# PlayVoice/whisper-vits-svc

Hardware: AMD Instinct MI355X
Metric: audio-seconds/sec end-to-end SVC @32kHz, 10s clips (Whisper-PPG -> flow -> NSF-BigVGAN) (higher is better)
Workload: dtype f32; 1 GPU; configs[1]: batch=1 x 10s clip per GPU, whisper-large-v2 dims (24 of 32 encoder blocks) + base.yaml prior/flow/NSF-BigVGAN; Whisper fp32, synthesizer fp32; clips_in_flight=4, gemm_ring2_mask=12, world_size=1, rccl_ranks_seen=1, whisper_weights_wire=f32, weights=packed on this rank

## Files before the change

### include/svcmi.h

```cpp
#ifndef SVCMI_H
#define SVCMI_H

#include <stddef.h>
#include <stdint.h>

#ifdef __cplusplus
extern "C" {
#endif

#define SVCMI_ABI_VERSION 22

enum svcmi_status { SVCMI_OK = 0, SVCMI_EINVAL = -1, SVCMI_EUNSUPPORTED = -2, SVCMI_EALIGN = -3 };

enum svcmi_act { SVCMI_ACT_NONE = 0, SVCMI_ACT_RELU = 1, SVCMI_ACT_GELU = 2, SVCMI_ACT_MISH = 3, SVCMI_ACT_TANH = 4, SVCMI_ACT_SIGMOID = 5 };

enum svcmi_conv_flags {
    SVCMI_CONV_ACCUMULATE = 1,
    SVCMI_CONV_MASK_IN = 2,
    SVCMI_CONV_MASK_OUT = 4,
    SVCMI_CONV_PARTIALS = 8,
    SVCMI_CONV_TILE_64x64 = 0x100,
    SVCMI_CONV_TILE_128x64 = 0x200,
    SVCMI_CONV_TILE_128x128 = 0x300,
    SVCMI_CONV_TILE_P16_64x48 = 0x400,
    SVCMI_CONV_TILE_P16_128x48 = 0x500,
    SVCMI_CONV_TILE_P16_64x80 = 0x600,
    SVCMI_CONV_TILE_P16_128x80 = 0x700,
    SVCMI_CONV_TILE_P16_64x160 = 0x800,
    SVCMI_CONV_TILE_64x128 = 0x900,
    SVCMI_CONV_TILE_P16W8_128x80 = 0xA00,
    SVCMI_CONV_TILE_MASK = 0xF00,
    SVCMI_CONV_RING2 = 0x1000
};

int svcmi_abi_version(void);
const char* svcmi_build_info(void);

typedef struct svcmi_conv_desc {
    const float* x;
    const float* w;
    const float* bias;
    const float* res;
    float* y;
    const int32_t* lengths;
    int64_t x_bstride, y_bstride, res_bstride;
    int32_t batch, t_in, t_out, c_in, ldx, n_out, ldw, ldy, ldr;
    int32_t ksize, stride, dilation, pad, x_row_shift;
    int32_t act;
    int32_t flags;
    float alpha;
    int32_t split_k;
    float* workspace;
    int64_t workspace_floats;
    int32_t* counters;
    int64_t counters_len;
    void* y16;
    int64_t y16_bstride;
    int32_t ldy16;
    int32_t y16_format;
} svcmi_conv_desc;

int svcmi_conv_gemm_f32(const svcmi_conv_desc* d, void* stream);

int svcmi_conv_gemm_group_f32(const svcmi_conv_desc* descs, int32_t count, void* stream);

enum svcmi_precision { SVCMI_PREC_F32 = 0, SVCMI_PREC_BF16X3 = 1, SVCMI_PREC_BF16 = 2, SVCMI_PREC_F16 = 3,
                       SVCMI_PREC_BF16_A16 = 4, SVCMI_PREC_F16_A16 = 5, SVCMI_PREC_BF16X3_A16 = 6,
                       SVCMI_PREC_MIXED = 7,
                       SVCMI_PREC_F16W2 = 8, SVCMI_PREC_F16W2_A16 = 9 };
int svcmi_pack_weights_lp(const float* w, int32_t n, int32_t ldw, int32_t precision, void* out, int32_t ldw16, void* stream);
int svcmi_conv_gemm_lp(const svcmi_conv_desc* d, int32_t precision, void* stream);
int svcmi_conv_gemm_group_lp(const svcmi_conv_desc* descs, int32_t count, int32_t precision, void* stream);

int svcmi_layernorm_f32(const float* x, const float* res, const float* gamma, const float* beta, float* y,
                        int32_t batch, int32_t rows_per_batch, int32_t c, int32_t ldx, int32_t ldr, int32_t ldy,
                        int32_t gb_bstride, float eps, void* y16, int32_t ldy16, int32_t y16_format, void* stream);

int svcmi_channel_norm_gelu_f32(const float* x, const float* gamma, const float* beta, float* y, double* scratch,
                                int32_t batch, int32_t t, int32_t c, int32_t ldx, int32_t ldy, float eps, void* stream);

int svcmi_splitk_layernorm_f32(const float* partials, int32_t split, const float* bias, float* x, const float* gamma,
                               const float* beta, float* y, int32_t batch, int32_t rows_per_batch, int32_t c,
                               int32_t ldx, int32_t ldy, float eps, void* y16, int32_t ldy16, int32_t y16_format, void* stream);

int svcmi_attention_f32(const float* q, const float* k, const float* v, float* o,
                        int32_t ldq, int32_t ldk, int32_t ldv, int32_t ldo,
                        int64_t q_bstride, int64_t k_bstride, int64_t v_bstride, int64_t o_bstride,
                        int32_t batch, int32_t t, int32_t heads, int32_t head_dim, float scale,
                        const float* rel_k, const float* rel_v, int32_t window,
                        const int32_t* lengths, void* o16, int32_t ldo16, int64_t o16_bstride, int32_t o16_format, void* stream);

int svcmi_attention16(const void* q, const void* k, const void* v, int32_t ld16, int64_t bstride16, float* o, int32_t ldo,
                      int64_t o_bstride, void* o16, int32_t ldo16, int64_t o16_bstride, int32_t batch, int32_t t, int32_t heads,
                      int32_t head_dim, float scale, const float* rel_k, const float* rel_v, int32_t window,
                      const int32_t* lengths, int32_t format, void* stream);

int svcmi_snake_alias_f32(const float* x, float* y, const float* alpha_log, const float* beta_log,
                          const float* filt, int32_t batch, int32_t len, int32_t c, int32_t ld, void* stream);
int svcmi_snake_alias_group_f32(const float* const* x, float* const* y, const float* const* alpha_log,
                                const float* const* beta_log, const float* filt, int32_t count, int32_t batch,
                                int32_t len, int32_t c, int32_t ld, void* const* y16, int32_t y16_format, void* stream);
int svcmi_block_mean_f32(const float* const* xs, int32_t count, float* y, int64_t n, void* stream);

int svcmi_snake_conv_supported(int32_t c, int32_t ld, int32_t ksize, int32_t dilation);
int svcmi_snake_conv_preferred(int32_t c, int32_t ld, int32_t ksize, int32_t dilation);
int svcmi_snake_conv_f32(const float* x, const float* w, const float* bias, const float* res, float* y,
                         const float* alpha_log, const float* beta_log, const float* filt,
                         int32_t batch, int32_t len, int32_t c, int32_t ld, int32_t ldw, int32_t ksize,
                         int32_t dilation, float alpha, int32_t accumulate, void* stream);

typedef struct svcmi_snake_conv_desc {
    const float* x; const float* w; const float* bias; const float* res; float* y;
    const float* alpha_log; const float* beta_log;
    int32_t ldw, ksize, dilation, accumulate;
    float alpha;
} svcmi_snake_conv_desc;
int svcmi_snake_conv_group_f32(const svcmi_snake_conv_desc* descs, int32_t count, const float* filt, int32_t batch,
                               int32_t len, int32_t c, int32_t ld, void* stream);

int svcmi_snake_conv_lp_supported(int32_t c, int32_t ld, int32_t ksize, int32_t dilation, int32_t precision);
int svcmi_snake_conv_group_lp(const svcmi_snake_conv_desc* descs, int32_t count, const float* filt, int32_t batch,
                              int32_t len, int32_t c, int32_t ld, int32_t precision, void* stream);

int svcmi_upsample_noise_supported(int32_t u, int32_t cp, int32_t c_in);
int svcmi_upsample_noise_f32(const float* x, const float* w_up, const float* b_up, const float* src, const float* w_nz,
                             const float* b_nz, float* y, int32_t batch, int32_t t_in, int32_t c_in, int32_t ldw_up,
                             int32_t taps, int32_t pad, int32_t u, int32_t cp, int64_t src_len, int32_t nz_k,
                             int32_t nz_stride, int32_t nz_pad, int32_t ldw_nz, void* stream);

int svcmi_snake_post_supported(int32_t c, int32_t ld, int32_t ksize);
int svcmi_snake_post_f32(const float* x, const float* w, float* y, const float* alpha_log, const float* beta_log,
                         const float* filt, int32_t batch, int32_t len, int32_t c, int32_t ld, int32_t ksize, void* stream);

int svcmi_tune_set(const char* name, int32_t value);
int svcmi_tune_get(const char* name, int32_t* value);

int svcmi_wn_gate_f32(const float* a, const float* bias, float* out, int32_t batch, int32_t t, int32_t h, int32_t lda,
                      int32_t ldo, int32_t splits, void* stream);

int svcmi_wn_update_f32(const float* rs, float* x, float* skip, const int32_t* lengths,
                        int32_t batch, int32_t t, int32_t h, int32_t ldrs, int32_t first, int32_t last, void* stream);

int svcmi_coupling_pre_f32(const float* x, int32_t ldx, int32_t x0_off, const float* ms_vs, float* out, int32_t ldo,
                           const int32_t* lengths, int32_t batch, int32_t t, int32_t half, void* stream);
int svcmi_coupling_post_f32(float* x, int32_t ldx, int32_t x1_off, const float* m, int32_t ldm, const float* ms_vs,
                            const int32_t* lengths, int32_t batch, int32_t t, int32_t half, void* stream);

int svcmi_embed_pitch_f32(float* x, int32_t ldx, const float* pit, const float* emb, const int32_t* lengths,
                          int32_t batch, int32_t t, int32_t c, void* stream);

int svcmi_sample_prior_f32(const float* stats, int32_t lds, const float* noise_ncl, const int32_t* lengths,
                           float* z, int32_t ldz, int32_t batch, int32_t t, int32_t i, void* stream);

int svcmi_ncl_to_nlc_f32(const float* x, const float* add, float add_scale, float* y,
                         int32_t batch, int32_t c, int32_t t, int32_t ldy, void* stream);
int svcmi_nlc_to_ncl_f32(const float* x, int32_t ldx, float* y, int32_t batch, int32_t c, int32_t t, void* stream);

int svcmi_pitch_prefix_f64(const float* f0, const float* rand_ini, double* prefix,
                           int32_t batch, int32_t t, int32_t hop, float sr, void* stream);
int svcmi_pitch_source_f32(const float* f0, const double* prefix, const float* noise, const float* merge_w,
                           float merge_b, float* out, int32_t batch, int32_t t, int32_t hop, float sr, void* stream);

int svcmi_reflect_pad_f32(const float* x, float* y, int32_t batch, int64_t n, int32_t pad, void* stream);
int svcmi_power_spectrum_f32(const float* ri, float* p, int64_t rows, int32_t nbins, int32_t half, int32_t ldri, int32_t ldp, void* stream);
int svcmi_logmel_finish_f32(float* mel_power, float* scratch, float* out, int32_t batch, int32_t t, int32_t c, void* stream);

int svcmi_pcm_resample_f32(const void* pcm, int32_t fmt, int32_t channels, int64_t frames, const float* taps, int32_t up, int32_t down,
                           int32_t taps_per_phase, int32_t half, float* out, int64_t n_out, void* stream);

int svcmi_lstm_step_f32(const float* gx, int64_t gx_bstride, const float* whh, float* hseq, int64_t h_bstride, int32_t ldh,
                        float* c, int32_t ldc, int32_t batch, int32_t hidden, int32_t t, int32_t t_total, void* stream);
int svcmi_preemph_pad_f32(const float* x, float* y, int32_t batch, int64_t n, int32_t pad, float coef, void* stream);
int svcmi_magnitude_spectrum_f32(const float* ri, float* p, int64_t rows, int32_t nbins, int32_t half, int32_t ldri, int32_t ldp, void* stream);
int svcmi_speaker_mel_finish_f32(float* mel, int64_t total, float ref_level_db, float min_level_db, float max_norm, void* stream);
int svcmi_l2norm_rows_f32(const float* x, int64_t ldx, int32_t rows, int32_t d, float* y, int64_t ldy, void* stream);
int svcmi_group_mean_f32(const float* x, int32_t rows_per_group, int32_t groups, int32_t d, float* y, void* stream);

int svcmi_linear_spectrogram_f32(const float* x, int64_t x_bstride, int32_t batch, int64_t n, const float* basis, int32_t n_fft, int32_t hop,
                                 int32_t pad, float eps, float* out, int64_t frames, void* stream);

int64_t svcmi_stft_distance_workspace_bytes(int32_t batch, int64_t n, int32_t n_fft, int32_t hop, int32_t pad);
int svcmi_stft_distance_f32(const float* x, int64_t x_bstride, const float* y, int64_t y_bstride, int32_t batch, int64_t n, const float* basis,
                            int32_t n_fft, int32_t hop, int32_t pad, float floor_, int64_t frames, float* partials, int64_t partials_bytes,
                            double* out, void* stream);
int svcmi_log_mel_f32(const float* spec, int32_t batch, int32_t bins, int64_t frames, const float* melT, int32_t ldm, int32_t n_mel, float clip,
                      float* out, void* stream);
int64_t svcmi_abs_diff_sum_workspace_bytes(int32_t batch, int64_t count);
int svcmi_abs_diff_sum_f32(const float* a, int64_t a_bstride, const float* b, int64_t b_bstride, int32_t batch, int64_t count, float* partials,
                           int64_t partials_bytes, double* out, void* stream);

int svcmi_crepe_frames_f32(const float* audio, int64_t n, int32_t hop, int32_t frame0, int32_t frames, float* out, int32_t ld, void* stream);
int svcmi_bn_maxpool2_f32(const float* x, const float* scale, const float* shift, float* y, int64_t rows_out, int32_t c,
                          int32_t ldx, int32_t ldy, void* y16, int32_t ldy16, int32_t y16_format, void* stream);
int svcmi_viterbi_decode(const float* prob, const double* log_trans, float* lp_scratch, int16_t* ptr_scratch, int32_t* path,
                         int32_t frames, int32_t batch_frames, int32_t minidx, int32_t maxidx, int32_t band, void* stream);

int svcmi_row_sqnorm_f32(const float* x, int32_t ldx, int64_t rows, int32_t d, float* out, void* stream);
int svcmi_knn_blend_f32(const float* x, int32_t ldx, const float* bank, int32_t ldb, const float* dots, int64_t ldd,
                        const float* bank_sq, float* out, int32_t ldo, int32_t t, int32_t n, int32_t d, int32_t k,
                        float ratio, void* stream);

int svcmi_ivf_assign_f32(const float* x, int32_t ldx, const float* dots, int64_t ldd, const float* cent_sq, int32_t t,
                         int32_t nlist, int32_t d, int32_t* assign, float* dist, void* stream);
int svcmi_ivf_blend_f32(const float* x, int32_t ldx, const int32_t* assign, const int32_t* list_off, const float* bank,
                        int32_t ldb, float* out, int32_t ldo, int32_t t, int32_t d, int32_t k, float ratio,
                        int32_t* out_idx, float* out_dist, void* stream);
int svcmi_segment_mean_f32(const float* x, int32_t ldx, const int32_t* order, const int32_t* seg_off, float* out, int32_t ldo,
                           int32_t segments, int32_t d, void* stream);

int svcmi_source2wav_i16(const float* x, int16_t* y, int64_t n, void* stream);


#define SVCMI_MAX_WHISPER_BLOCKS 32
#define SVCMI_MAX_ENC_LAYERS 8
#define SVCMI_MAX_FLOWS 8
#define SVCMI_MAX_WN_LAYERS 8
#define SVCMI_MAX_STAGES 6
#define SVCMI_MAX_AMP_BLOCKS 3
#define SVCMI_MAX_AMP_DILATIONS 3

typedef struct svcmi_weight {
    const float* w;
    const float* bias;
    const void* w16;
    const void* w16a;
    int32_t n, ldw, ldw16;
    int32_t prec16;
} svcmi_weight;

typedef struct svcmi_whisper_block {
    const float *ln1_g, *ln1_b, *ln2_g, *ln2_b;
    svcmi_weight qkv, o, m1, m2;
} svcmi_whisper_block;

typedef struct svcmi_whisper_model {
    int32_t n_state, n_heads, n_layers, n_mels, n_ctx;
    int32_t precision;
    svcmi_weight conv1, conv2;
    const float* pos;
    const float *lnp_g, *lnp_b;
    svcmi_whisper_block blocks[SVCMI_MAX_WHISPER_BLOCKS];
    int32_t split_o, split_mlp, tile_qkv, tile_o, tile_mlp1, tile_mlp2, small_m_rows, reserved;
    float lp_min_flops;
    int32_t reserved2;
} svcmi_whisper_model;

int64_t svcmi_whisper_workspace_bytes(const svcmi_whisper_model* m, int32_t batch, int32_t n_frames);
int svcmi_whisper_encoder_fwd(const svcmi_whisper_model* m, const float* mel, const float* noise, float noise_scale,
                              int32_t batch, int32_t n_frames, float* out, void* workspace, int64_t workspace_bytes, void* stream);

#define SVCMI_MAX_LSTM_LAYERS 8
typedef struct svcmi_lstm_layer {
    svcmi_weight ih;
    svcmi_weight lin;
    const float* whh;
    const void* reserved;
} svcmi_lstm_layer;
typedef struct svcmi_speaker_model {
    int32_t input_dim, lstm_dim, proj_dim, n_layers;
    svcmi_lstm_layer layers[SVCMI_MAX_LSTM_LAYERS];
} svcmi_speaker_model;

int64_t svcmi_speaker_encoder_workspace_bytes(const svcmi_speaker_model* m, int32_t batch, int32_t t);
int svcmi_speaker_encoder_fwd(const svcmi_speaker_model* m, const float* mel, int32_t batch, int32_t t, float* emb, void* workspace,
                              int64_t workspace_bytes, void* stream);

typedef struct svcmi_vad_conv_block {
    const float *dw_w, *dw_b;
    const float *pw_w, *pw_b;
    const float *proj_w, *proj_b;
    int32_t c_in, c_out;
// ... 247 lines not shown
```

### whisper-vits-svc_amd/csrc/amp_fused.hip

```cpp
#include "svcmi_rt.h"
#include "../../include/svcmi.h"

namespace {

constexpr int TPB = 256;
constexpr int RT = 8;
constexpr int CO = 10;
constexpr int DMAX = 5;

#include "snake_math.h"

template <int CP>
__device__ __forceinline__ int tile_row_offset(int t) {
    static_assert(CP == 12 || CP == 20 || CP == 40, "widths of the fused kernels");
    return CP == 12 ? (t << 3) + (t << 2) : CP == 20 ? (t << 4) + (t << 2) : (t << 5) + (t << 3);
}
__device__ __forceinline__ const float* tile_column(const float* xc) {
#ifndef SVCMI_EMU
    asm("" : "+v"(xc));
#endif
    return xc;
}
template <int CP>
__device__ __forceinline__ float tile_x(const float* xc, int t, int n, int ld) {
    (void)ld;
#ifndef SVCMI_EMU
    return ((const __attribute__((address_space(1))) float*)xc)[tile_row_offset<CP>(clampi(t, 0, n - 1))];
#else
    return xc[tile_row_offset<CP>(clampi(t, 0, n - 1))];
#endif
}
static inline bool tile_len_ok(int len, int ld) { return (long long)len * ld < (1LL << 31); }

struct AmpArgs {
    const float* x; const float* w; const float* bias; const float* res; float* y;
    const float* alpha_log; const float* beta_log; const float* filt;
    int n, ld, ldw, dil, accumulate, ks;
    float alpha;
};

template <bool H16, int LS>
__device__ __forceinline__ void tile_store(float* S, int row, int ch, float v) {
    if constexpr (H16) reinterpret_cast<unsigned short*>(S)[row * LS + ch] = (unsigned short)svcmi_cvt_pk_f16(v, 0.f);
    else S[row * LS + ch] = v;
}

template <int CP, int CR, int LS, bool H16 = false>
__device__ __forceinline__ void snake_tile(float* S, const float* xb, const float* alpha_log, const float* beta_log,
                                           const float* filt, int n, int ld, int t_blk, int halo, int rows, int tid) {
    struct { const float* alpha_log; const float* beta_log; const float* filt; } p = {alpha_log, beta_log, filt};
        float f[12];
#pragma unroll
        for (int k = 0; k < 12; ++k) f[k] = p.filt[k];
        const int runs = (rows + RT - 1) / RT;
        for (int item = tid; item < runs * CP; item += TPB) {
            const int ch = item % CP, run = item / CP;
            const int r0 = run * RT;
            const int t0 = t_blk - halo + r0;
            float out[RT];
            if (ch >= CR || t0 + RT <= 0 || t0 >= n) {
#pragma unroll
                for (int r = 0; r < RT; ++r) out[r] = 0.f;
            } else {
                const float a = expf(p.alpha_log[ch]);
                const float inv_b = 1.0f / (expf(p.beta_log[ch]) + 1e-9f);
                const float* xc = tile_column(xb + ch);
                SnakeWindow<RT + 10> xw;
#pragma unroll
                for (int i = 0; i < RT + 10; ++i) xw.set(i, tile_x<CP>(xc, t0 - 5 + i, n, ld));
                snake_run<RT>(xw, f, a, inv_b, xc, ld, n, t0, out);
#pragma unroll
                for (int r = 0; r < RT; ++r) {
                    const int t = t0 + r;
                    if (t < 0 || t >= n) out[r] = 0.f;
                }
            }
#pragma unroll
            for (int r = 0; r < RT; ++r)
                if (r0 + r < rows) tile_store<H16, LS>(S, r0 + r, ch, out[r]);
        }
}

template <int CP>
struct UTile {
    static constexpr int LU = 2 * CP + 2;
    __device__ __forceinline__ static int pos(int m) { return m * LU; }
    static constexpr int floats(int pair_rows) { return (pair_rows + 7) * LU; }
};

template <int CP, int CR, int LS, int MAXI, bool H16 = false>
__device__ __forceinline__ void snake_tile_u(float* smem, const float* xb, const float* alpha_log, const float* beta_log,
                                             const float* filt, int n, int ld, int t_blk, int halo, int rows, int tid) {
    constexpr int LU = UTile<CP>::LU;
    float f[12];
#pragma unroll
    for (int k = 0; k < 12; ++k) f[k] = filt[k];
    const int t_lo = t_blk - halo;
    const int pairs = rows + 5;
    const int mruns = (pairs + RT - 1) / RT;
    for (int item = tid; item < mruns * CP; item += TPB) {
        const int ch = item % CP, run = item / CP;
        if (ch >= CR) continue;
        const int m0 = run * RT, tq0 = t_lo + m0;
        svcmi_f32x2 s2[RT];
        if (2 * tq0 - 5 + 2 * RT - 1 < -12 || 2 * tq0 - 5 > 2 * n - 1 + 12) {
#pragma unroll
            for (int m = 0; m < RT; ++m) s2[m] = svcmi_splat2(0.f);
        } else {
            const float a = expf(alpha_log[ch]);
            const float inv_b = 1.0f / (expf(beta_log[ch]) + 1e-9f);
            const float* xc = tile_column(xb + ch);
            SnakeWindow<RT + 5> xw;
#pragma unroll
            for (int i = 0; i < RT + 5; ++i) xw.set(i, tile_x<CP>(xc, tq0 - 5 + i, n, ld));
            snake_pairs<RT>(xw, f, a, inv_b, xc, ld, n, tq0, s2);
        }
#pragma unroll
        for (int m = 0; m < RT; ++m)
            if (m0 + m < pairs) *reinterpret_cast<float2*>(smem + UTile<CP>::pos(m0 + m) + 2 * ch) = make_float2(s2[m][0], s2[m][1]);
    }
    __syncthreads();
    const int runs = (rows + RT - 1) / RT;
    float outs[MAXI][RT];
#pragma unroll
    for (int q = 0; q < MAXI; ++q) {
        const int item = tid + q * TPB;
        if (item < runs * CP) {
            const int ch = item % CP, run = item / CP, r0 = run * RT, t0 = t_lo + r0;
            if (ch >= CR || t0 + RT <= 0 || t0 >= n) {
#pragma unroll
                for (int r = 0; r < RT; ++r) outs[q][r] = 0.f;
            } else {
                svcmi_f32x2 P[RT + 5];
                const float* ub = smem + UTile<CP>::pos(r0) + 2 * ch;
#pragma unroll
                for (int i = 0; i < RT + 5; ++i) {
                    const float2 v = *reinterpret_cast<const float2*>(ub + i * LU);
                    P[i] = svcmi_f32x2{v.x, v.y};
                }
                snake_fir<RT>(P, f, outs[q]);
#pragma unroll
                for (int r = 0; r < RT; ++r) {
                    const int t = t0 + r;
                    if (t < 0 || t >= n) outs[q][r] = 0.f;
                }
            }
        }
    }
    __syncthreads();
#pragma unroll
    for (int q = 0; q < MAXI; ++q) {
        const int item = tid + q * TPB;
        if (item < runs * CP) {
            const int ch = item % CP, r0 = (item / CP) * RT;
#pragma unroll
            for (int r = 0; r < RT; ++r)
                if (r0 + r < rows) tile_store<H16, LS>(smem, r0 + r, ch, outs[q][r]);
        }
    }
}

template <int CP, int G, int TT, int KS>
struct AmpTile {
    static constexpr int TSUB = 4 / G;
    static constexpr int TB = TSUB * 64 * TT;
    static constexpr int LS = (CP / 4) % 2 ? CP : CP + 4;
    static constexpr int ROWS = TB + (KS - 1) * DMAX;
};

template <int CP, int CR, int KS_T, int G, int TT, bool UT = false>
__device__ __forceinline__ void snake_conv_body(const AmpArgs& p, float* S) {
    using TL = AmpTile<CP, G, TT, KS_T ? KS_T : 11>;
    const int KS = KS_T ? KS_T : p.ks;
    constexpr int TSUB = TL::TSUB, TB = TL::TB, LS = TL::LS;
    static_assert(G * CO >= CR && CP % 4 == 0 && CP >= CR, "channel split");

    const int tid = threadIdx.x, lane = tid & 63;
    const int wave = SVCMI_UNIFORM((int)(tid >> 6));
    const int b = blockIdx.y;
    const int n = p.n, ld = p.ld, d = p.dil;
    const int halo = (KS - 1) * d / 2;
    const int t_blk = blockIdx.x * TB;
    const int rows = TB + 2 * halo;
    const float* xb = p.x + (long long)b * n * ld;

    if constexpr (UT) snake_tile_u<CP, CR, LS, (((TL::ROWS + RT - 1) / RT) * CP + TPB - 1) / TPB>(S, xb, p.alpha_log, p.beta_log, p.filt, n, ld, t_blk, halo, rows, tid);
    else snake_tile<CP, CR, LS>(S, xb, p.alpha_log, p.beta_log, p.filt, n, ld, t_blk, halo, rows, tid);
    __syncthreads();

    const int g = wave % G, tsub = wave / G;
    const int co0 = g * CO;
    constexpr int NCO = CO;
    static_assert(NCO % 2 == 0 && CR % 2 == 0, "channel pairs");
    svcmi_f32x2 acc[TT][NCO / 2];
#pragma unroll
    for (int c = 0; c < NCO; c += 2) {
        const float b0 = (co0 + c < CR && p.bias) ? p.bias[co0 + c] : 0.f, b1 = (co0 + c < CR && p.bias) ? p.bias[co0 + c + 1] : 0.f;
#pragma unroll
        for (int j = 0; j < TT; ++j) acc[j][c / 2] = svcmi_f32x2{b0, b1};
    }
    const int tl0 = tsub * 64 * TT + lane;
    constexpr bool PRE = TT == 1;
    const float* rb = p.res ? p.res + (long long)b * n * ld : nullptr;
    float2 rpre[PRE ? TT : 1][NCO / 2];
    if constexpr (PRE) {
#pragma unroll
        for (int j = 0; j < TT; ++j) {
            const int t = t_blk + tl0 + 64 * j;
#pragma unroll
            for (int c = 0; c < NCO; c += 2) {
                rpre[j][c / 2] = make_float2(0.f, 0.f);
                if (rb && t < n && co0 + c < CR) rpre[j][c / 2] = *reinterpret_cast<const float2*>(rb + (long long)t * ld + co0 + c);
            }
        }
    }
    const float* wg = p.w + (long long)co0 * p.ldw;
    for (int tap = 0; tap < KS; ++tap) {
        const float* srow = S + (tl0 + tap * d) * LS;
        const float* wt = wg + tap * CP;
#pragma unroll
        for (int c4 = 0; c4 < (CR + 3) / 4; ++c4) {
            svcmi_f32x2 x01[TT], x23[TT];
#pragma unroll
            for (int j = 0; j < TT; ++j) {
                const float4 xin = *reinterpret_cast<const float4*>(srow + j * 64 * LS + 4 * c4);
                x01[j] = svcmi_f32x2{xin.x, xin.y}; x23[j] = svcmi_f32x2{xin.z, xin.w};
            }
#pragma unroll
            for (int c = 0; c < NCO; c += 2) {
                if (co0 + c < CR) {
                    const float* wr = wt + (long long)c * p.ldw + 4 * c4;
                    const float4 w0 = *reinterpret_cast<const float4*>(wr), w1 = *reinterpret_cast<const float4*>(wr + p.ldw);
#pragma unroll
                    for (int j = 0; j < TT; ++j) {
                        acc[j][c / 2] = svcmi_fma2(svcmi_splat_lo(x01[j]), svcmi_f32x2{w0.x, w1.x}, acc[j][c / 2]);
                        if (4 * c4 + 1 < CR) acc[j][c / 2] = svcmi_fma2(svcmi_splat_hi(x01[j]), svcmi_f32x2{w0.y, w1.y}, acc[j][c / 2]);
                        if (4 * c4 + 2 < CR) acc[j][c / 2] = svcmi_fma2(svcmi_splat_lo(x23[j]), svcmi_f32x2{w0.z, w1.z}, acc[j][c / 2]);
                        if (4 * c4 + 3 < CR) acc[j][c / 2] = svcmi_fma2(svcmi_splat_hi(x23[j]), svcmi_f32x2{w0.w, w1.w}, acc[j][c / 2]);
                    }
                }
            }
        }
    }

    float* yb = p.y + (long long)b * n * ld;
#pragma unroll
    for (int j = 0; j < TT; ++j) {
        const int t = t_blk + tl0 + 64 * j;
        if (t >= n) continue;
        float* yr = yb + (long long)t * ld + co0;
#pragma unroll
        for (int c = 0; c < NCO; c += 2) {
            float v0 = acc[j][c / 2][0], v1 = acc[j][c / 2][1];
            if (co0 + c >= CR) { v0 = 0.f; v1 = 0.f; }
            else {
                if (rb) {
                    float2 r2;
                    if constexpr (PRE) r2 = rpre[j][c / 2];
                    else r2 = *reinterpret_cast<const float2*>(rb + (long long)t * ld + co0 + c);
                    v0 += r2.x; v1 += r2.y;
                }
                v0 *= p.alpha; v1 *= p.alpha;
                if (p.accumulate) { const float2 o2 = *reinterpret_cast<const float2*>(yr + c); v0 += o2.x; v1 += o2.y; }
            }
            *reinterpret_cast<float2*>(yr + c) = make_float2(v0, v1);
        }
        if (g == G - 1) {
#pragma unroll
            for (int c = G * CO; c < CP; c += 2) *reinterpret_cast<float2*>(yb + (long long)t * ld + c) = make_float2(0.f, 0.f);
        }
    }
}

template <int CP, int CR, int KS, int G, int TT>
__global__ __launch_bounds__(TPB) void snake_conv_kernel(AmpArgs p) {
    using TL = AmpTile<CP, G, TT, KS>;
    __shared__ __attribute__((aligned(16))) float S[TL::ROWS * TL::LS];
    snake_conv_body<CP, CR, KS, G, TT>(p, S);
}

constexpr int AMP_GROUP = 3;
struct AmpGroupArgs {
    AmpArgs p[AMP_GROUP];
};

template <int CP, int CR, int G, int TT>
__global__ __launch_bounds__(TPB) void snake_conv_group_kernel(AmpGroupArgs g) {
    using TL = AmpTile<CP, G, TT, 11>;
    __shared__ __attribute__((aligned(16))) float S[TL::ROWS * TL::LS];
    snake_conv_body<CP, CR, 0, G, TT>(g.p[blockIdx.z], S);
}

template <int CP, int CR, int G, int TT>
__global__ __launch_bounds__(TPB) void snake_conv_group_u_kernel(AmpGroupArgs g) {
    using TL = AmpTile<CP, G, TT, 11>;
    constexpr int NU = UTile<CP>::floats(TL::ROWS + 5), NS = TL::ROWS * TL::LS;
    static_assert(((TL::ROWS + RT - 1) / RT) * CP <= 4 * TPB, "snake_tile_u keeps at most 4 work items per thread in registers");
    __shared__ __attribute__((aligned(16))) float S[NU > NS ? NU : NS];
    snake_conv_body<CP, CR, 0, G, TT, true>(g.p[blockIdx.z], S);
}

template <int CP, int CR, int TERMS>
struct Amp16 {
    static constexpr int CK = (CR + 7) / 8;
    static constexpr int LSH = 24;
    static constexpr int NCT = (CR + 15) / 16;
    static constexpr int TB = 256;
    static constexpr int ROWS = TB + 10 * DMAX;
    static constexpr int MAXSTEPS = (11 * CK + 3) / 4;
    static constexpr int S_FLOATS = (ROWS * LSH / 2 + 3) / 4 * 4;
    static constexpr int U_FLOATS = (UTile<CP>::floats(ROWS + 5) + 3) / 4 * 4;
    static constexpr int W_FLOATS = MAXSTEPS * NCT * TERMS * 64 * 4;
    static_assert(CK * 8 <= LSH && CP <= CK * 8 && CP + 4 >= CK * 8, "pad columns [CP, 8 CK) are one 8-byte store per row");
};

template <int CP, int CR, int TERMS, bool UT>
__device__ __forceinline__ void snake_conv16_body(const AmpArgs& p, float* smem, float* wl) {
    using TL = Amp16<CP, CR, TERMS>;
    constexpr int CK = TL::CK, LSH = TL::LSH, NCT = TL::NCT, TB = TL::TB;
    const int KS = p.ks;
    const int tid = threadIdx.x, lane = tid & 63;
    const int wave = SVCMI_UNIFORM((int)(tid >> 6));
    const int b = blockIdx.y;
    const int n = p.n, ld = p.ld, d = p.dil;
    const int halo = (KS - 1) * d / 2;
    const int t_blk = blockIdx.x * TB;
    const int rows = TB + 2 * halo;
    const float* xb = p.x + (long long)b * n * ld;
    const int nsteps = (KS * CK + 3) / 4;

    svcmi_u32x4* wf = reinterpret_cast<svcmi_u32x4*>(wl);
    auto pack_weights = [&] {
    for (int u = tid; u < nsteps * NCT * 64; u += TPB) {
        const int l = u & 63, f = u >> 6;
        const int ct = f % NCT, step = f / NCT;
        const int co = ct * 16 + (l & 15), s = 4 * step + (l >> 4);
        const int tap = s / CK, cb = s - tap * CK;
        float v[8];
#pragma unroll
        for (int h = 0; h < 2; ++h) {
            const int ci0 = cb * 8 + 4 * h;
            float4 q = make_float4(0.f, 0.f, 0.f, 0.f);
            if (co < CR && tap < KS && ci0 < CR) q = *reinterpret_cast<const float4*>(p.w + (long long)co * p.ldw + tap * CP + ci0);
            v[4 * h] = q.x;
            v[4 * h + 1] = ci0 + 1 < CR ? q.y : 0.f;
            v[4 * h + 2] = ci0 + 2 < CR ? q.z : 0.f;
            v[4 * h + 3] = ci0 + 3 < CR ? q.w : 0.f;
        }
        svcmi_u32x4 hi;
#pragma unroll
        for (int e = 0; e < 4; ++e) hi[e] = svcmi_cvt_pk_f16(v[2 * e], v[2 * e + 1]);
        wf[(f * TERMS) * 64 + l] = hi;
        if constexpr (TERMS == 2) {
            svcmi_u32x4 lo;
#pragma unroll
            for (int e = 0; e < 4; ++e)
                lo[e] = svcmi_cvt_pk_f16(v[2 * e] - svcmi_f16_bits_f32(hi[e]), v[2 * e + 1] - svcmi_f16_bits_f32(hi[e] >> 16));
            wf[(f * TERMS + 1) * 64 + l] = lo;
        }
    }
    };
    if constexpr (!UT) pack_weights();

    if constexpr (UT) snake_tile_u<CP, CR, LSH, (((TL::ROWS + RT - 1) / RT) * CP + TPB - 1) / TPB, true>(smem, xb, p.alpha_log, p.beta_log, p.filt, n, ld, t_blk, halo, rows, tid);
    else snake_tile<CP, CR, LSH, true>(smem, xb, p.alpha_log, p.beta_log, p.filt, n, ld, t_blk, halo, rows, tid);
    if constexpr (UT) pack_weights();
    unsigned short* S16 = reinterpret_cast<unsigned short*>(smem);
    if constexpr (CP < CK * 8)
        for (int r = tid; r < rows; r += TPB) *reinterpret_cast<svcmi_u32x2*>(S16 + r * LSH + CP) = svcmi_u32x2{0u, 0u};
    __syncthreads();

    constexpr int NT = 4;
    const int tq = lane & 15, kq = lane >> 4;
    svcmi_f32x4 acc[NT][NCT];
#pragma unroll
    for (int tt = 0; tt < NT; ++tt)
#pragma unroll
        for (int ct = 0; ct < NCT; ++ct) acc[tt][ct] = svcmi_f32x4{0.f, 0.f, 0.f, 0.f};
    const int row0 = wave * (16 * NT) + tq;
    const float* rb = p.res ? p.res + (long long)b * n * ld : nullptr;
    float4 rpre[NT][NCT];
#pragma unroll
    for (int tt = 0; tt < NT; ++tt) {
        const int t = t_blk + wave * (16 * NT) + tt * 16 + tq;
#pragma unroll
        for (int ct = 0; ct < NCT; ++ct) {
            const int co4 = ct * 16 + 4 * kq;
            rpre[tt][ct] = make_float4(0.f, 0.f, 0.f, 0.f);
            if (rb && t < n && co4 < CP) rpre[tt][ct] = *reinterpret_cast<const float4*>(rb + (long long)t * ld + co4);
        }
    }
    for (int step = 0; step < nsteps; ++step) {
        const int s = 4 * step + kq;
        int tap = s / CK;
        const int cb = s - tap * CK;
        tap = tap < KS ? tap : KS - 1;
        const unsigned short* sp = S16 + (row0 + tap * d) * LSH + cb * 8;
        svcmi_u32x4 bf[NT], af[NCT][TERMS];
#pragma unroll
        for (int ct = 0; ct < NCT; ++ct)
#pragma unroll
            for (int tm = 0; tm < TERMS; ++tm) af[ct][tm] = wf[((step * NCT + ct) * TERMS + tm) * 64 + lane];
#pragma unroll
        for (int tt = 0; tt < NT; ++tt) bf[tt] = *reinterpret_cast<const svcmi_u32x4*>(sp + tt * 16 * LSH);
#pragma unroll
        for (int tm = 0; tm < TERMS; ++tm)
#pragma unroll
            for (int ct = 0; ct < NCT; ++ct)
#pragma unroll
                for (int tt = 0; tt < NT; ++tt) acc[tt][ct] = svcmi_mfma16_16x16x32<true>(af[ct][tm], bf[tt], acc[tt][ct]);
    }

    float* yb = p.y + (long long)b * n * ld;
#pragma unroll
    for (int tt = 0; tt < NT; ++tt) {
        const int t = t_blk + wave * (16 * NT) + tt * 16 + tq;
        asm volatile("" ::: "memory");
        if (t >= n) continue;
#pragma unroll
        for (int ct = 0; ct < NCT; ++ct) {
            const int co4 = ct * 16 + 4 * kq;
            if (co4 >= CP) continue;
            float v[4] = {acc[tt][ct][0], acc[tt][ct][1], acc[tt][ct][2], acc[tt][ct][3]};
            float* yr = yb + (long long)t * ld + co4;
            float4 bq = make_float4(0.f, 0.f, 0.f, 0.f), oq = bq;
            const float4 rq = rpre[tt][ct];
            if (p.bias) bq = *reinterpret_cast<const float4*>(p.bias + co4);
            if (p.accumulate) oq = *reinterpret_cast<const float4*>(yr);
            const float bv[4] = {bq.x, bq.y, bq.z, bq.w}, rv[4] = {rq.x, rq.y, rq.z, rq.w}, ov[4] = {oq.x, oq.y, oq.z, oq.w};
#pragma unroll
            for (int e = 0; e < 4; ++e) v[e] = co4 + e < CR ? (v[e] + bv[e] + rv[e]) * p.alpha + ov[e] : 0.f;
            *reinterpret_cast<float4*>(yr) = make_float4(v[0], v[1], v[2], v[3]);
        }
    }
}

template <int CP, int CR, int TERMS, bool UT>
__global__ __launch_bounds__(TPB) void snake_conv16_group_kernel(AmpGroupArgs g) {
    using TL = Amp16<CP, CR, TERMS>;
    constexpr int NSW = TL::S_FLOATS + TL::W_FLOATS;
    __shared__ __attribute__((aligned(16))) float smem[UT && TL::U_FLOATS > NSW ? TL::U_FLOATS : NSW];
    snake_conv16_body<CP, CR, TERMS, UT>(g.p[blockIdx.z], smem, smem + TL::S_FLOATS);
}

template <int CP, int CR>
struct AmpM {
    static constexpr int NC4 = CP / 4;
    static constexpr int NCT = (CR + 15) / 16;
    static constexpr int TB = 256;
    static constexpr int ROWS = TB + 10 * DMAX;
    static constexpr int MAXQ = (11 * NC4 + 3) / 4;
    static constexpr int S_FLOATS = ROWS * CP;
// ... 99 lines not shown
}

template <int CP, int CR, bool UT>
__global__ __launch_bounds__(TPB) void snake_convm_group_kernel(AmpGroupArgs g) {
    using TL = AmpM<CP, CR>;
    constexpr int NSW = TL::S_FLOATS + TL::W_FLOATS;
    __shared__ __attribute__((aligned(16))) float smem[UT && TL::U_FLOATS > NSW ? TL::U_FLOATS : NSW];
    snake_convm_body<CP, CR, UT>(g.p[blockIdx.z], smem, smem + TL::S_FLOATS);
}

struct UpArgs {
    const float* x; const float* wu; const float* bu; const float* src; const float* wn; const float* bn; float* y;
    int t_in, cin, ldwu, taps, pad, u, cp, nz_k, nz_stride, nz_pad, ldwn;
    long long src_len;
};

template <int N>
__global__ __launch_bounds__(TPB) void upsample_noise_kernel(UpArgs p) {
    const int b = blockIdx.y;
    const int q = blockIdx.x * TPB + threadIdx.x;
    if (q >= p.t_in) return;
    const float* xb = p.x + (long long)b * p.t_in * p.cin;
    float acc[N];
    float* yr = p.y + ((long long)b * p.t_in + q) * N;
    if (!p.x) {
#pragma unroll
        for (int n = 0; n < N; n += 4) {
            const float4 v = *reinterpret_cast<const float4*>(yr + n);
            acc[n] = v.x; acc[n + 1] = v.y; acc[n + 2] = v.z; acc[n + 3] = v.w;
        }
    } else {
#pragma unroll
        for (int n = 0; n < N; ++n) acc[n] = p.bu[n];
    }
    for (int k = 0; p.x && k < p.taps; ++k) {
        const int row = q + k - p.pad;
        if (row < 0 || row >= p.t_in) continue;
        const float* xr = xb + (long long)row * p.cin;
        const float* wk = p.wu + k * p.cin;
        for (int c4 = 0; c4 < p.cin; c4 += 4) {
            const float4 xv = *reinterpret_cast<const float4*>(xr + c4);
            const svcmi_f32x2 x01 = {xv.x, xv.y}, x23 = {xv.z, xv.w};
#pragma unroll
            for (int n = 0; n < N; n += 2) {
                const float4 w0 = *reinterpret_cast<const float4*>(wk + (long long)n * p.ldwu + c4);
                const float4 w1 = *reinterpret_cast<const float4*>(wk + (long long)(n + 1) * p.ldwu + c4);
                svcmi_f32x2 a2 = {acc[n], acc[n + 1]};
                a2 = svcmi_fma2(svcmi_splat_lo(x01), svcmi_f32x2{w0.x, w1.x}, a2);
                a2 = svcmi_fma2(svcmi_splat_hi(x01), svcmi_f32x2{w0.y, w1.y}, a2);
                a2 = svcmi_fma2(svcmi_splat_lo(x23), svcmi_f32x2{w0.z, w1.z}, a2);
                a2 = svcmi_fma2(svcmi_splat_hi(x23), svcmi_f32x2{w0.w, w1.w}, a2);
                acc[n] = a2[0]; acc[n + 1] = a2[1];
            }
        }
    }
    const float* sb = p.src + (long long)b * p.src_len;
    const int cp = N / 2;
#pragma unroll
    for (int r = 0; r < 2; ++r) {
        const long long t = 2LL * q + r;
        for (int k = 0; k < p.nz_k; ++k) {
            const long long si = t * p.nz_stride - p.nz_pad + k;
            const float sv = (si >= 0 && si < p.src_len) ? sb[si] : 0.f;
#pragma unroll
            for (int co = 0; co < cp; ++co) acc[r * cp + co] = fmaf(p.wn[co * p.ldwn + k], sv, acc[r * cp + co]);
        }
#pragma unroll
        for (int co = 0; co < cp; ++co) acc[r * cp + co] += p.bn[co];
    }
#pragma unroll
    for (int n = 0; n < N; n += 4) *reinterpret_cast<float4*>(yr + n) = make_float4(acc[n], acc[n + 1], acc[n + 2], acc[n + 3]);
}

struct PostArgs {
    const float* x; const float* w; float* y; const float* alpha_log; const float* beta_log; const float* filt;
    int n, ld;
};

template <int CP, int CR, int KS, int TT>
__global__ __launch_bounds__(TPB) void snake_post_kernel(PostArgs p) {
    constexpr int TB = TPB * TT;
    constexpr int LS = (CP / 4) % 2 ? CP : CP + 4;
    constexpr int ROWS = TB + KS - 1;
    __shared__ __attribute__((aligned(16))) float S[ROWS * LS];
    const int tid = threadIdx.x, b = blockIdx.y;
    const int t_blk = blockIdx.x * TB;
    snake_tile<CP, CR, LS>(S, p.x + (long long)b * p.n * p.ld, p.alpha_log, p.beta_log, p.filt, p.n, p.ld, t_blk, (KS - 1) / 2,
                           ROWS, tid);
    __syncthreads();
    float acc[TT];
#pragma unroll
    for (int j = 0; j < TT; ++j) acc[j] = 0.f;
#pragma unroll
    for (int tap = 0; tap < KS; ++tap) {
#pragma unroll
        for (int c4 = 0; c4 < (CR + 3) / 4; ++c4) {
            const float4 wv = *reinterpret_cast<const float4*>(p.w + tap * CP + 4 * c4);
#pragma unroll
            for (int j = 0; j < TT; ++j) {
                const float4 xin = *reinterpret_cast<const float4*>(S + (tid + TPB * j + tap) * LS + 4 * c4);
                acc[j] = fmaf(wv.x, xin.x, acc[j]);
                if (4 * c4 + 1 < CR) acc[j] = fmaf(wv.y, xin.y, acc[j]);
                if (4 * c4 + 2 < CR) acc[j] = fmaf(wv.z, xin.z, acc[j]);
                if (4 * c4 + 3 < CR) acc[j] = fmaf(wv.w, xin.w, acc[j]);
            }
        }
    }
    float* yb = p.y + (long long)b * p.n;
#pragma unroll
    for (int j = 0; j < TT; ++j) {
        const int t = t_blk + tid + TPB * j;
        if (t < p.n) yb[t] = tanhf(acc[j]);
    }
}

template <int CP, int CR, int G, int TT>
int launch_amp(const AmpArgs& a, int batch, int ksize, void* stream) {
    constexpr int TB = (4 / G) * 64 * TT;
    dim3 grid((unsigned)((a.n + TB - 1) / TB), (unsigned)batch);
    switch (ksize) {
        case 3: SVCMI_LAUNCH((snake_conv_kernel<CP, CR, 3, G, TT>), grid, dim3(TPB), 0, stream, a); break;
        case 7: SVCMI_LAUNCH((snake_conv_kernel<CP, CR, 7, G, TT>), grid, dim3(TPB), 0, stream, a); break;
        case 11: SVCMI_LAUNCH((snake_conv_kernel<CP, CR, 11, G, TT>), grid, dim3(TPB), 0, stream, a); break;
        default: return SVCMI_EUNSUPPORTED;
    }
    return SVCMI_LAST_ERROR();
}

int g_amp_tt = 0;

}

extern "C" int svcmi_snake_conv_supported(int32_t c, int32_t ld, int32_t ksize, int32_t dilation) {
    const bool shape = (c == 10 && ld == 12) || (c == 20 && ld == 20) || (c == 40 && ld == 40);
    return shape && (ksize == 3 || ksize == 7 || ksize == 11) && dilation >= 1 && dilation <= DMAX;
}

extern "C" int svcmi_snake_conv_preferred(int32_t c, int32_t ld, int32_t ksize, int32_t dilation) {
    return svcmi_snake_conv_supported(c, ld, ksize, dilation) && c <= 20;
}

extern "C" int svcmi_snake_conv_f32(const float* x, const float* w, const float* bias, const float* res, float* y,
                                    const float* alpha_log, const float* beta_log, const float* filt,
                                    int32_t batch, int32_t len, int32_t c, int32_t ld, int32_t ldw, int32_t ksize,
                                    int32_t dilation, float alpha, int32_t accumulate, void* stream) {
    if (!x || !w || !y || !alpha_log || !beta_log || !filt || batch <= 0 || len <= 0) return SVCMI_EINVAL;
    if (x == y) return SVCMI_EINVAL;
    if (!svcmi_snake_conv_supported(c, ld, ksize, dilation)) return SVCMI_EUNSUPPORTED;
    if (ldw < ksize * ld || ldw % 4 != 0) return SVCMI_EINVAL;
    if (((uintptr_t)w & 15) || ((uintptr_t)x & 7) || ((uintptr_t)y & 7) || ((uintptr_t)res & 7)) return SVCMI_EALIGN;
    if (batch > 65535 || !tile_len_ok(len, ld)) return SVCMI_EUNSUPPORTED;
    AmpArgs a;
    a.x = x; a.w = w; a.bias = bias; a.res = res; a.y = y; a.alpha_log = alpha_log; a.beta_log = beta_log; a.filt = filt;
    a.n = len; a.ld = ld; a.ldw = ldw; a.dil = dilation; a.accumulate = accumulate; a.alpha = alpha; a.ks = ksize;
    const int tt = g_amp_tt ? g_amp_tt : 2;
    if (c == 10) return tt == 1 ? launch_amp<12, 10, 1, 1>(a, batch, ksize, stream) : tt == 2 ? launch_amp<12, 10, 1, 2>(a, batch, ksize, stream) : launch_amp<12, 10, 1, 4>(a, batch, ksize, stream);
    if (c == 20) return tt == 1 ? launch_amp<20, 20, 2, 1>(a, batch, ksize, stream) : tt == 2 ? launch_amp<20, 20, 2, 2>(a, batch, ksize, stream) : launch_amp<20, 20, 2, 4>(a, batch, ksize, stream);
    return tt == 1 ? launch_amp<40, 40, 4, 1>(a, batch, ksize, stream) : tt == 2 ? launch_amp<40, 40, 4, 2>(a, batch, ksize, stream) : launch_amp<40, 40, 4, 4>(a, batch, ksize, stream);
}

int g_amp_u = 0;
int g_amp_mfma = 1;

template <int TT>
static void launch_amp_group(const AmpGroupArgs& g, int count, int batch, int len, int c, void* stream) {
    if constexpr (TT == 1) {
        if (g_amp_u >= 0 && c == 10) {
            constexpr int TB = AmpTile<12, 1, 1, 3>::TB;
            SVCMI_LAUNCH((snake_conv_group_u_kernel<12, 10, 1, 1>), dim3((unsigned)((len + TB - 1) / TB), (unsigned)batch, (unsigned)count),
                         dim3(TPB), 0, stream, g);
            return;
        }
    }
    if constexpr (TT == 2) {
        if ((g_amp_u > 0 || (g_amp_u == 0 && (long long)batch * len >= 500000)) && c == 20) {
            constexpr int TB = AmpTile<20, 2, 2, 3>::TB;
            SVCMI_LAUNCH((snake_conv_group_u_kernel<20, 20, 2, 2>), dim3((unsigned)((len + TB - 1) / TB), (unsigned)batch, (unsigned)count),
                         dim3(TPB), 0, stream, g);
            return;
        }
    }
    if (c == 10) {
        constexpr int TB = AmpTile<12, 1, TT, 3>::TB;
        SVCMI_LAUNCH((snake_conv_group_kernel<12, 10, 1, TT>), dim3((unsigned)((len + TB - 1) / TB), (unsigned)batch, (unsigned)count),
                     dim3(TPB), 0, stream, g);
    } else if (c == 20) {
        constexpr int TB = AmpTile<20, 2, TT, 3>::TB;
        SVCMI_LAUNCH((snake_conv_group_kernel<20, 20, 2, TT>), dim3((unsigned)((len + TB - 1) / TB), (unsigned)batch, (unsigned)count),
                     dim3(TPB), 0, stream, g);
    } else {
        constexpr int TB = AmpTile<40, 4, TT, 3>::TB;
        SVCMI_LAUNCH((snake_conv_group_kernel<40, 40, 4, TT>), dim3((unsigned)((len + TB - 1) / TB), (unsigned)batch, (unsigned)count),
                     dim3(TPB), 0, stream, g);
    }
}

extern "C" int svcmi_snake_conv_group_f32(const svcmi_snake_conv_desc* descs, int32_t count, const float* filt, int32_t batch,
                                          int32_t len, int32_t c, int32_t ld, void* stream) {
    if (!descs || !filt || count < 1 || count > AMP_GROUP || batch <= 0 || len <= 0) return SVCMI_EINVAL;
    if (batch > 65535 || !tile_len_ok(len, ld)) return SVCMI_EUNSUPPORTED;
    int order[AMP_GROUP] = {0, 1, 2};
    for (int i = 0; i < count; ++i)
        for (int j = i + 1; j < count; ++j)
            if (descs[order[j]].ksize > descs[order[i]].ksize) { const int t = order[i]; order[i] = order[j]; order[j] = t; }
    AmpGroupArgs g;
    for (int i = 0; i < count; ++i) {
        const svcmi_snake_conv_desc& d = descs[order[i]];
        if (!d.x || !d.w || !d.y || !d.alpha_log || !d.beta_log || d.x == d.y) return SVCMI_EINVAL;
        if (!svcmi_snake_conv_supported(c, ld, d.ksize, d.dilation)) return SVCMI_EUNSUPPORTED;
        if (d.ldw < d.ksize * ld || d.ldw % 4 != 0) return SVCMI_EINVAL;
        if (((uintptr_t)d.w & 15) || ((uintptr_t)d.x & 7) || ((uintptr_t)d.y & 7) || ((uintptr_t)d.res & 7)) return SVCMI_EALIGN;
        AmpArgs& a = g.p[i];
        a.x = d.x; a.w = d.w; a.bias = d.bias; a.res = d.res; a.y = d.y; a.alpha_log = d.alpha_log; a.beta_log = d.beta_log;
        a.filt = filt; a.n = len; a.ld = ld; a.ldw = d.ldw; a.dil = d.dilation; a.accumulate = d.accumulate; a.alpha = d.alpha;
        a.ks = d.ksize;
    }
    for (int i = count; i < AMP_GROUP; ++i) g.p[i] = g.p[0];
    const bool mfma_auto = g_amp_mfma == 1 && c == 20 && batch <= 2;
    if ((mfma_auto || g_amp_mfma >= 2) && c <= 20 && !g_amp_tt) {
        bool al = true;
        for (int i = 0; i < count; ++i) al = al && !(((uintptr_t)g.p[i].y | (uintptr_t)g.p[i].res | (uintptr_t)g.p[i].bias) & 15);
        if (al) {
            const dim3 grid((unsigned)((len + 255) / 256), (unsigned)batch, (unsigned)count);
            const bool ut = g_amp_mfma == 3 ? false : g_amp_mfma == 2 ? true : g_amp_u >= 0;
            if (c == 10) { if (ut) SVCMI_LAUNCH((snake_convm_group_kernel<12, 10, true>), grid, dim3(TPB), 0, stream, g); else SVCMI_LAUNCH((snake_convm_group_kernel<12, 10, false>), grid, dim3(TPB), 0, stream, g); }
            else { if (ut) SVCMI_LAUNCH((snake_convm_group_kernel<20, 20, true>), grid, dim3(TPB), 0, stream, g); else SVCMI_LAUNCH((snake_convm_group_kernel<20, 20, false>), grid, dim3(TPB), 0, stream, g); }
            return SVCMI_LAST_ERROR();
        }
    }
    const int tt = g_amp_tt ? g_amp_tt : (c == 10 ? 1 : 2);
    if (tt == 4) launch_amp_group<4>(g, count, batch, len, c, stream);
    else if (tt == 1) launch_amp_group<1>(g, count, batch, len, c, stream);
    else launch_amp_group<2>(g, count, batch, len, c, stream);
    return SVCMI_LAST_ERROR();
}

extern "C" int svcmi_snake_conv_lp_supported(int32_t c, int32_t ld, int32_t ksize, int32_t dilation, int32_t precision) {
    return svcmi_snake_conv_supported(c, ld, ksize, dilation) && c <= 20 && (precision == SVCMI_PREC_F16 || precision == SVCMI_PREC_F16W2);
}

template <int CP, int CR, int TERMS>
static void launch_amp16_group(const AmpGroupArgs& g, int count, int batch, int len, bool ut, void* stream) {
    constexpr int TB = Amp16<CP, CR, TERMS>::TB;
    const dim3 grid((unsigned)((len + TB - 1) / TB), (unsigned)batch, (unsigned)count);
    if (ut) SVCMI_LAUNCH((snake_conv16_group_kernel<CP, CR, TERMS, true>), grid, dim3(TPB), 0, stream, g);
    else SVCMI_LAUNCH((snake_conv16_group_kernel<CP, CR, TERMS, false>), grid, dim3(TPB), 0, stream, g);
}

extern "C" int svcmi_snake_conv_group_lp(const svcmi_snake_conv_desc* descs, int32_t count, const float* filt, int32_t batch,
                                         int32_t len, int32_t c, int32_t ld, int32_t precision, void* stream) {
    if (!descs || !filt || count < 1 || count > AMP_GROUP || batch <= 0 || len <= 0) return SVCMI_EINVAL;
    if (batch > 65535 || !tile_len_ok(len, ld)) return SVCMI_EUNSUPPORTED;
    int order[AMP_GROUP] = {0, 1, 2};
    for (int i = 0; i < count; ++i)
        for (int j = i + 1; j < count; ++j)
            if (descs[order[j]].ksize > descs[order[i]].ksize) { const int t = order[i]; order[i] = order[j]; order[j] = t; }
    AmpGroupArgs g;
    for (int i = 0; i < count; ++i) {
        const svcmi_snake_conv_desc& d = descs[order[i]];
        if (!d.x || !d.w || !d.y || !d.alpha_log || !d.beta_log || d.x == d.y) return SVCMI_EINVAL;
        if (!svcmi_snake_conv_lp_supported(c, ld, d.ksize, d.dilation, precision)) return SVCMI_EUNSUPPORTED;
        if (d.ldw < d.ksize * ld || d.ldw % 4 != 0) return SVCMI_EINVAL;
        if (((uintptr_t)d.w & 15) || ((uintptr_t)d.x & 7) || ((uintptr_t)d.y & 15) || ((uintptr_t)d.res & 15) || ((uintptr_t)d.bias & 15)) return SVCMI_EALIGN;
        AmpArgs& a = g.p[i];
        a.x = d.x; a.w = d.w; a.bias = d.bias; a.res = d.res; a.y = d.y; a.alpha_log = d.alpha_log; a.beta_log = d.beta_log;
        a.filt = filt; a.n = len; a.ld = ld; a.ldw = d.ldw; a.dil = d.dilation; a.accumulate = d.accumulate; a.alpha = d.alpha;
        a.ks = d.ksize;
    }
    for (int i = count; i < AMP_GROUP; ++i) g.p[i] = g.p[0];
    const bool ut = g_amp_u >= 0;
    const bool w2 = precision == SVCMI_PREC_F16W2;
    if (c == 10) { if (w2) launch_amp16_group<12, 10, 2>(g, count, batch, len, ut, stream); else launch_amp16_group<12, 10, 1>(g, count, batch, len, ut, stream); }
    else { if (w2) launch_amp16_group<20, 20, 2>(g, count, batch, len, ut, stream); else launch_amp16_group<20, 20, 1>(g, count, batch, len, ut, stream); }
    return SVCMI_LAST_ERROR();
}

extern "C" int svcmi_snake_post_supported(int32_t c, int32_t ld, int32_t ksize) { return c == 10 && ld == 12 && ksize == 7; }

extern "C" int svcmi_snake_post_f32(const float* x, const float* w, float* y, const float* alpha_log, const float* beta_log,
                                    const float* filt, int32_t batch, int32_t len, int32_t c, int32_t ld, int32_t ksize, void* stream) {
    if (!x || !w || !y || !alpha_log || !beta_log || !filt || batch <= 0 || len <= 0) return SVCMI_EINVAL;
    if (!svcmi_snake_post_supported(c, ld, ksize)) return SVCMI_EUNSUPPORTED;
    if (((uintptr_t)w & 15) || ((uintptr_t)x & 7)) return SVCMI_EALIGN;
    if (batch > 65535 || !tile_len_ok(len, ld)) return SVCMI_EUNSUPPORTED;
    PostArgs a;
    a.x = x; a.w = w; a.y = y; a.alpha_log = alpha_log; a.beta_log = beta_log; a.filt = filt; a.n = len; a.ld = ld;
    constexpr int TT = 2;
    SVCMI_LAUNCH((snake_post_kernel<12, 10, 7, TT>), dim3((unsigned)((len + TPB * TT - 1) / (TPB * TT)), (unsigned)batch), dim3(TPB), 0,
                 stream, a);
    return SVCMI_LAST_ERROR();
}

extern "C" int svcmi_upsample_noise_supported(int32_t u, int32_t cp, int32_t cin) {
    return u == 2 && (cp == 12 || cp == 20) && cin % 4 == 0 && cin > 0;
}

extern "C" int svcmi_upsample_noise_f32(const float* x, const float* w_up, const float* b_up, const float* src, const float* w_nz,
                                        const float* b_nz, float* y, int32_t batch, int32_t t_in, int32_t c_in, int32_t ldw_up,
                                        int32_t taps, int32_t pad, int32_t u, int32_t cp, int64_t src_len, int32_t nz_k,
                                        int32_t nz_stride, int32_t nz_pad, int32_t ldw_nz, void* stream) {
    if (!src || !w_nz || !b_nz || !y || batch <= 0 || t_in <= 0 || nz_k <= 0) return SVCMI_EINVAL;
    if (x && (!w_up || !b_up || taps <= 0)) return SVCMI_EINVAL;
    if (!svcmi_upsample_noise_supported(u, cp, c_in)) return SVCMI_EUNSUPPORTED;
    if ((x && (ldw_up < taps * c_in || ldw_up % 4)) || ldw_nz < nz_k) return SVCMI_EINVAL;
    if (((uintptr_t)x & 15) || ((uintptr_t)w_up & 15) || ((uintptr_t)y & 15)) return SVCMI_EALIGN;
    if (batch > 65535) return SVCMI_EUNSUPPORTED;
    UpArgs a;
    a.x = x; a.wu = w_up; a.bu = b_up; a.src = src; a.wn = w_nz; a.bn = b_nz; a.y = y;
    a.t_in = t_in; a.cin = c_in; a.ldwu = ldw_up; a.taps = taps; a.pad = pad; a.u = u; a.cp = cp;
    a.nz_k = nz_k; a.nz_stride = nz_stride; a.nz_pad = nz_pad; a.ldwn = ldw_nz; a.src_len = src_len;
    dim3 grid((unsigned)((t_in + TPB - 1) / TPB), (unsigned)batch);
    if (cp == 12) SVCMI_LAUNCH((upsample_noise_kernel<24>), grid, dim3(TPB), 0, stream, a);
    else SVCMI_LAUNCH((upsample_noise_kernel<40>), grid, dim3(TPB), 0, stream, a);
    return SVCMI_LAST_ERROR();
}

extern "C" int svcmi_conv_tune_set(const char* name, int32_t value);
extern "C" int svcmi_attn_tune_set(const char* name, int32_t value);
extern "C" int svcmi_host_tune_set(const char* name, int32_t value);
extern "C" int svcmi_snake_tune_set(const char* name, int32_t value);

extern "C" int svcmi_tune_set(const char* name, int32_t value) {
    if (!name) return SVCMI_EINVAL;
    if (svcmi_conv_tune_set(name, value) == 0 || svcmi_attn_tune_set(name, value) == 0 || svcmi_host_tune_set(name, value) == 0 ||
        svcmi_snake_tune_set(name, value) == 0) return 0;
    const char* k = "amp_tt";
    int i = 0;
    while (k[i] && name[i] == k[i]) ++i;
    if (k[i] == 0 && name[i] == 0 && (value == 0 || value == 1 || value == 2 || value == 4)) { g_amp_tt = value; return 0; }
    const char* km = "amp_mfma";
    i = 0;
    while (km[i] && name[i] == km[i]) ++i;
    if (km[i] == 0 && name[i] == 0 && value >= 0 && value <= 3) { g_amp_mfma = value; return 0; }
    const char* ku = "amp_u";
    i = 0;
    while (ku[i] && name[i] == ku[i]) ++i;
    if (ku[i] == 0 && name[i] == 0 && value >= -1 && value <= 1) { g_amp_u = value; return 0; }
    return SVCMI_EINVAL;
}
```

### whisper-vits-svc_amd/csrc/host_stages.hip

```cpp
#include <math.h>
#include <string.h>

#include <vector>

#include "svcmi_rt.h"
#include "../../include/svcmi.h"

extern "C" int svcmi_pyin_plan_check_(const svcmi_pyin_plan* p);
extern "C" int svcmi_yin_plan_check_(const svcmi_yin_plan* p);

namespace {

int g_amp_grouped = 1;
int g_amp_lp = 1;

enum Op {
    OP_CONV_F32, OP_CONV_LP, OP_CONV_GROUP_F32, OP_CONV_GROUP_LP, OP_LAYERNORM, OP_SPLITK_LN, OP_ATTENTION, OP_SNAKE_ALIAS,
    OP_SNAKE_ALIAS_GROUP, OP_BLOCK_MEAN, OP_SNAKE_CONV, OP_SNAKE_CONV_GROUP, OP_UPSAMPLE_NOISE, OP_SNAKE_POST, OP_WN_GATE,
    OP_COUPLING_PRE, OP_COUPLING_POST, OP_EMBED_PITCH, OP_SAMPLE_PRIOR, OP_NCL_TO_NLC, OP_COPY2D, OP_PITCH_PREFIX, OP_PITCH_SOURCE,
    OP_ATTENTION16, OP_SNAKE_CONV_GROUP_LP, OP_LSTM_STEP, OP_L2NORM_ROWS, OP_VAD_FRONTEND, OP_VAD_LSTM_SCAN,
    OP_SALIENCE_STFT, OP_SALIENCE_MAP, OP_SALIENCE_DP, OP_PYIN_CMNDF, OP_PYIN_OBSERVE, OP_PYIN_VITERBI, OP_PYIN_FINISH,
    OP_YIN_CMNDF, OP_YIN_PICK, OP_YIN_APERIODICITY, OP_SWEEP_PITCH, OP_SWEEP_EMBED,
    OP_COUNT
};
// ... 421 lines not shown
    float* stats = qkv;
    {
        CV v; v.x = x; v.x_bs = (int64_t)T * H; v.B = B; v.t_in = T; v.c_in = v.ldx = H; v.w = &m.proj; v.lengths = io.lengths;
        v.mask_in = v.mask_out = true; v.y = stats; v.y_bs = (int64_t)T * 2 * I; v.ldy = 2 * I;
        conv(c, v);
    }
    run(c, OP_SAMPLE_PRIOR, 0.0, 16.0 * B * T * I,
        [&] { return svcmi_sample_prior_f32(stats, 2 * I, io.noise, io.lengths, z_p, I, B, T, I, c.stream); });
}

void prior_fwd(Ctx& c, const svcmi_synth_model& m, const svcmi_synth_io& io, float* z_p) {
    const int B = io.batch, T = io.t, H = m.hidden;
    const int64_t mark = c.ar.mark();
    c.prec = class_prec(m, SVCMI_CLASS_ENC);
    float* xa = c.ar.f((int64_t)B * T * H);
    float* xb = c.ar.f((int64_t)B * T * H);
    prior_front(c, m, io, xa);
    run(c, OP_EMBED_PITCH, 0.0, 8.0 * B * T * H,
        [&] { return svcmi_embed_pitch_f32(xa, H, io.pit, m.pit_emb, io.lengths, B, T, H, c.stream); });
    prior_tail(c, m, io, xa, xb, z_p);
    c.ar.release(mark);
}

void flow_fwd(Ctx& c, const svcmi_synth_model& m, const svcmi_synth_io& io, float* x) {
    const int B = io.batch, T = io.t, H = m.hidden, I = m.inter, half = I / 2, kf = m.flow_kernel;
    const int64_t mark = c.ar.mark();
    c.prec = class_prec(m, SVCMI_CLASS_FLOW);
    float* hs = c.ar.f((int64_t)B * T * 2 * H);
    float* skip = hs + H;
    const int nk = (kf * H + 31) / 32;
    const int blocks = B * ((T + 63) / 64) * ((2 * H + 63) / 64);
    int split = 1;
    if (blocks < 256) {
        const int a = nk / 8, b = (288 + blocks / 2) / blocks;
        split = a < b ? a : b;
        if (split < 1) split = 1;
    }
    float* msvs = c.ar.f((int64_t)B * 2 * half);
    float* x0n = c.ar.f((int64_t)B * T * half);
    float* acts = c.ar.f((int64_t)B * T * H);
    float* mpost = c.ar.f((int64_t)B * T * half);
    float* slabs = c.ar.f((int64_t)B * split * T * 2 * H);
    for (int fl = 0; fl < m.n_flow; ++fl) {
        const svcmi_flow_layer& L = m.flow[fl];
        {
            CV v; v.x = io.spk; v.x_bs = m.spk_dim; v.B = B; v.t_in = 1; v.c_in = v.ldx = m.spk_dim; v.w = &L.snac;
            v.y = msvs; v.y_bs = 2 * half; v.ldy = 2 * half;
            conv(c, v);
        }
        run(c, OP_COUPLING_PRE, 0.0, 8.0 * B * T * half,
            [&] { return svcmi_coupling_pre_f32(x, I, L.x0_off, msvs, x0n, half, io.lengths, B, T, half, c.stream); });
        {
            CV v; v.x = x0n; v.x_bs = (int64_t)T * half; v.B = B; v.t_in = T; v.c_in = v.ldx = half; v.w = &L.pre; v.lengths = io.lengths;
            v.mask_out = true; v.y = hs; v.y_bs = (int64_t)T * 2 * H; v.ldy = 2 * H;
            conv(c, v);
        }
        for (int l = 0; l < L.n_wn; ++l) {
            const svcmi_wn_layer& W = L.wn[l];
            {
                CV v; v.x = hs; v.x_bs = (int64_t)T * 2 * H; v.B = B; v.t_in = T; v.c_in = H; v.ldx = 2 * H; v.w = &W.in; v.bias = false;
                v.ksize = kf; v.pad = (kf - 1) / 2; v.slabs = slabs; v.split_k = split;
                conv(c, v);
            }
            run(c, OP_WN_GATE, 0.0, 4.0 * B * T * H * (2 * split + 1),
                [&] { return svcmi_wn_gate_f32(slabs, W.in.bias, acts, B, T, H, 2 * H, H, split, c.stream); });
            {
                CV v; v.x = acts; v.x_bs = (int64_t)T * H; v.B = B; v.t_in = T; v.c_in = v.ldx = H; v.w = &W.rs; v.lengths = io.lengths;
                v.mask_out = true; v.accumulate = true; v.y = l == L.n_wn - 1 ? skip : hs; v.y_bs = (int64_t)T * 2 * H; v.ldy = 2 * H;
                conv(c, v);
            }
        }
        {
            CV v; v.x = skip; v.x_bs = (int64_t)T * 2 * H; v.B = B; v.t_in = T; v.c_in = H; v.ldx = 2 * H; v.w = &L.post;
            v.lengths = io.lengths; v.mask_out = true; v.y = mpost; v.y_bs = (int64_t)T * half; v.ldy = half;
            conv(c, v);
        }
        run(c, OP_COUPLING_POST, 0.0, 12.0 * B * T * half,
            [&] { return svcmi_coupling_post_f32(x, I, L.x1_off, mpost, half, msvs, io.lengths, B, T, half, c.stream); });
    }
    c.ar.release(mark);
}

struct Snk { const float* a; const float* b; };

void snake_alias(Ctx& c, const svcmi_synth_model& m, const float* x, float* y, Snk s, int B, int64_t L, int C, int ld) {
    run(c, OP_SNAKE_ALIAS, 0.0, 8.0 * B * L * ld,
        [&] { return svcmi_snake_alias_f32(x, y, s.a, s.b, m.filt, B, (int32_t)L, C, ld, c.stream); });
}

void amp_block_seq(Ctx& c, const svcmi_synth_model& m, const svcmi_gen_stage& st, const svcmi_amp_block& blk, const float* y, float* acc,
                   float* xj, float* tmp, float* tmp2, int j, int nb, int B, int64_t L) {
    const int cp = st.cp, k = blk.k;
    const int64_t bs = L * cp;
    bool fused = true;
    for (int q = 0; q < blk.n_dil; ++q) fused = fused && svcmi_snake_conv_preferred(st.c, cp, k, blk.dil[q]);
    const float* xc = y;
    for (int q = 0; q < blk.n_dil; ++q) {
        const bool last = q == blk.n_dil - 1;
        const int d = blk.dil[q];
        float* outp = last ? acc : xj;
        const float alpha = last ? 1.0f / nb : 1.0f;
        const bool accum = last && j > 0;
        if (fused) {
            run(c, OP_SNAKE_CONV, 2.0 * B * L * st.c * st.c * k, 8.0 * B * L * st.c, [&] {
                return svcmi_snake_conv_f32(xc, blk.c1[q].w, blk.c1[q].bias, nullptr, tmp, blk.a1_alpha[q], blk.a1_beta[q], m.filt, B,
                                            (int32_t)L, st.c, cp, blk.c1[q].ldw, k, d, 1.0f, 0, c.stream);
            });
            run(c, OP_SNAKE_CONV, 2.0 * B * L * st.c * st.c * k, 8.0 * B * L * st.c, [&] {
                return svcmi_snake_conv_f32(tmp, blk.c2[q].w, blk.c2[q].bias, xc, outp, blk.a2_alpha[q], blk.a2_beta[q], m.filt, B,
                                            (int32_t)L, st.c, cp, blk.c2[q].ldw, k, 1, alpha, accum ? 1 : 0, c.stream);
            });
        } else {
            snake_alias(c, m, xc, tmp, Snk{blk.a1_alpha[q], blk.a1_beta[q]}, B, L, cp, cp);
            CV v; v.B = B; v.t_in = (int)L; v.c_in = v.ldx = cp; v.x_bs = bs; v.y_bs = bs; v.ldy = cp; v.ksize = k; v.tile = amp_tile(cp);
            { CV a = v; a.x = tmp; a.w = &blk.c1[q]; a.dil = d; a.pad = (k * d - d) / 2; a.y = tmp2; conv(c, a); }
            snake_alias(c, m, tmp2, tmp, Snk{blk.a2_alpha[q], blk.a2_beta[q]}, B, L, cp, cp);
            {
                CV a = v; a.x = tmp; a.w = &blk.c2[q]; a.pad = (k - 1) / 2; a.res = xc; a.res_bs = bs; a.ldr = cp; a.alpha = alpha;
                a.accumulate = accum; a.y = outp;
                conv(c, a);
            }
        }
        xc = xj;
    }
}

bool amp_stage_grouped(Ctx& c, const svcmi_synth_model& m, const svcmi_gen_stage& st, const float* y, float* acc, int B, int64_t L) {
    const int nb = st.n_blocks, cp = st.cp;
    if (!g_amp_grouped || nb < 2 || nb > 3 || cp % 4) return false;
    const int nd = st.blocks[0].n_dil;
    int nf = 0, nall = 0;
    for (int j = 0; j < nb; ++j) {
        if (st.blocks[j].n_dil != nd) return false;
        for (int q = 0; q < nd; ++q) { nf += svcmi_snake_conv_preferred(st.c, cp, st.blocks[j].k, st.blocks[j].dil[q]) ? 1 : 0; ++nall; }
    }
    if (nf != 0 && nf != nall) return false;
    const bool fused = nf == nall;
    const int64_t n = (int64_t)B * L * cp, bs = L * cp;
    float *xj[3], *t1[3], *t2[3];
    void* t1h[3] = {nullptr, nullptr, nullptr};
    for (int j = 0; j < nb; ++j) xj[j] = c.ar.f(n);
    for (int j = 0; j < nb; ++j) t1[j] = c.ar.f(n);
    for (int j = 0; j < nb; ++j) t2[j] = c.ar.f(n);
    if (!fused && mode16(c.prec) && cp % 8 == 0)
        for (int j = 0; j < nb; ++j) t1h[j] = c.ar.take(n * 2);
    const float* xc[3] = {y, y, y};
    bool lp = fused && g_amp_lp && (c.prec == SVCMI_PREC_F16 || c.prec == SVCMI_PREC_F16W2);
    for (int j = 0; lp && j < nb; ++j)
        for (int q = 0; q < nd; ++q) lp = lp && svcmi_snake_conv_lp_supported(st.c, cp, st.blocks[j].k, st.blocks[j].dil[q], SVCMI_PREC_F16W2);
    for (int q = 0; q < nd; ++q) {
        float** outs = q == nd - 1 ? t2 : xj;
        if (fused) {
            svcmi_snake_conv_desc d[3];
            double fl = 0.0;
            for (int j = 0; j < nb; ++j) {
                const svcmi_amp_block& b = st.blocks[j];
                d[j] = svcmi_snake_conv_desc{xc[j], b.c1[q].w, b.c1[q].bias, nullptr, t1[j], b.a1_alpha[q], b.a1_beta[q], b.c1[q].ldw, b.k,
                                             b.dil[q], 0, 1.0f};
                fl += 2.0 * B * L * st.c * st.c * b.k;
            }
            auto half_step = [&] {
                if (lp) run(c, OP_SNAKE_CONV_GROUP_LP, fl, 8.0 * nb * B * L * st.c,
                            [&] { return svcmi_snake_conv_group_lp(d, nb, m.filt, B, (int32_t)L, st.c, cp, SVCMI_PREC_F16W2, c.stream); });
                else run(c, OP_SNAKE_CONV_GROUP, fl, 8.0 * nb * B * L * st.c,
                         [&] { return svcmi_snake_conv_group_f32(d, nb, m.filt, B, (int32_t)L, st.c, cp, c.stream); });
            };
            half_step();
            for (int j = 0; j < nb; ++j) {
                const svcmi_amp_block& b = st.blocks[j];
                d[j] = svcmi_snake_conv_desc{t1[j], b.c2[q].w, b.c2[q].bias, xc[j], outs[j], b.a2_alpha[q], b.a2_beta[q], b.c2[q].ldw, b.k,
                                             1, 0, 1.0f};
            }
            half_step();
        } else {
            const float* px[3]; float* py[3]; const float *pa[3], *pb[3];
            CV vs[3];
            auto snake = [&](bool second) {
                const bool h16 = t1h[0] && conv_group(c, vs, nb, true) >= SVCMI_PREC_BF16_A16;
                for (int j = 0; j < nb; ++j) {
                    px[j] = second ? t2[j] : xc[j]; py[j] = t1[j];
                    pa[j] = second ? st.blocks[j].a2_alpha[q] : st.blocks[j].a1_alpha[q];
                    pb[j] = second ? st.blocks[j].a2_beta[q] : st.blocks[j].a1_beta[q];
                    if (!h16) vs[j].x16 = nullptr;
                }
                run(c, OP_SNAKE_ALIAS_GROUP, 0.0, (h16 ? 4.0 + 2.0 * w16(c.prec, 1) : 8.0) * nb * B * L * cp, [&] {
                    return svcmi_snake_alias_group_f32(px, h16 ? nullptr : py, pa, pb, m.filt, nb, B, (int32_t)L, cp, cp, h16 ? t1h : nullptr, fmt16_of(c.prec),
                                                       c.stream);
                });
            };
            for (int j = 0; j < nb; ++j) {
                const svcmi_amp_block& b = st.blocks[j];
                CV& v = vs[j]; v = CV();
                v.x = t1[j]; v.x16 = t1h[j]; v.x_bs = bs; v.B = B; v.t_in = (int)L; v.c_in = v.ldx = cp; v.w = &b.c1[q]; v.ksize = b.k; v.dil = b.dil[q];
                v.tile = amp_tile(cp);
                v.pad = (b.k * b.dil[q] - b.dil[q]) / 2; v.y = t2[j]; v.y_bs = bs; v.ldy = cp;
            }
            snake(false);
            conv_group(c, vs, nb);
            for (int j = 0; j < nb; ++j) {
                const svcmi_amp_block& b = st.blocks[j];
                CV& v = vs[j]; v = CV();
                v.x = t1[j]; v.x16 = t1h[j]; v.x_bs = bs; v.B = B; v.t_in = (int)L; v.c_in = v.ldx = cp; v.w = &b.c2[q]; v.ksize = b.k; v.pad = (b.k - 1) / 2;
                v.tile = amp_tile(cp);
                v.res = xc[j]; v.res_bs = bs; v.ldr = cp; v.y = outs[j]; v.y_bs = bs; v.ldy = cp;
            }
            snake(true);
            conv_group(c, vs, nb);
        }
        for (int j = 0; j < nb; ++j) xc[j] = outs[j];
    }
    run(c, OP_BLOCK_MEAN, 0.0, 4.0 * (nb + 1) * n, [&] { return svcmi_block_mean_f32(xc, nb, acc, n, c.stream); });
    return true;
}

void generator_tile(Ctx& c, const svcmi_synth_model& m, const float* z, const float* spk, const float* source, float* wave, int B, int T,
                    int split_k, int stop_after) {
    const int U = m.upsample_input;
    const int64_t mark = c.ar.mark();
    c.prec = class_prec(m, SVCMI_CLASS_UPS);
    float* sb = c.ar.f((int64_t)B * 2 * U);
    {
        CV v; v.x = spk; v.x_bs = m.spk_dim; v.B = B; v.t_in = 1; v.c_in = v.ldx = m.spk_dim; v.w = &m.adapter; v.y = sb; v.y_bs = 2 * U; v.ldy = 2 * U;
        conv(c, v);
    }
    float* xn = c.ar.f((int64_t)B * T * U);
    layernorm(c, z, nullptr, sb, sb + U, xn, B, T, U, U, 0, U, 2 * U);
    int cin = m.conv_pre.n;
    float* x = c.ar.f((int64_t)B * T * cin);
    {
        CV v; v.x = xn; v.x_bs = (int64_t)T * U; v.B = B; v.t_in = T; v.c_in = v.ldx = U; v.w = &m.conv_pre; v.ksize = 7; v.pad = 3;
        v.act = SVCMI_ACT_MISH; v.split_k = split_k; v.y = x; v.y_bs = (int64_t)T * cin; v.ldy = cin;
        conv(c, v);
    }
    const int64_t Lsrc = (int64_t)T * m.hop;
    if (stop_after == SVCMI_STOP_GEN_PRE) { c.ar.release(mark); return; }
    int64_t t_in = T;
    for (int i = 0; i < m.n_stages; ++i) {
        const svcmi_gen_stage& st = m.stages[i];
        const int cp = st.cp, u = st.u;
        const int64_t L = t_in * u;
        float* y = c.ar.f((int64_t)B * L * cp);
        float* acc = c.ar.f((int64_t)B * L * cp);
        const int64_t smark = c.ar.mark();
        c.prec = class_prec(m, SVCMI_CLASS_UPS);
        CV up; up.x = x; up.x_bs = t_in * cin; up.B = B; up.t_in = (int)t_in; up.t_out = (int)t_in; up.c_in = up.ldx = cin; up.w = &st.up;
        up.ksize = st.up_taps; up.pad = st.up_pad; up.split_k = split_k; up.y = y; up.y_bs = L * cp; up.ldy = u * cp;
        if (svcmi_upsample_noise_supported(u, cp, cin)) {
            const bool fuse_up = cp <= 12;
            if (!fuse_up) conv(c, up);
            run(c, OP_UPSAMPLE_NOISE, 0.0, 4.0 * B * t_in * (cin + u * cp), [&] {
                return svcmi_upsample_noise_f32(fuse_up ? x : nullptr, st.up.w, st.up.bias, source, st.nz.w, st.nz.bias, y, B, (int32_t)t_in,
                                                fuse_up ? cin : 4, st.up.ldw, st.up_taps, st.up_pad, u, cp, Lsrc, st.nz_k, st.nz_stride,
                                                st.nz_pad, st.nz.ldw, c.stream);
            });
        } else {
            conv(c, up);
            CV nz; nz.x = source; nz.x_bs = Lsrc; nz.B = B; nz.t_in = (int)Lsrc; nz.t_out = (int)L; nz.c_in = 1; nz.ldx = 1; nz.w = &st.nz;
            nz.ksize = st.nz_k; nz.stride = st.nz_stride; nz.pad = st.nz_pad; nz.accumulate = true; nz.split_k = split_k;
            nz.y = y; nz.y_bs = L * cp; nz.ldy = cp;
            conv(c, nz);
        }
        c.prec = class_prec(m, SVCMI_CLASS_AMP0 + (i < SVCMI_AMP_CLASSES ? i : SVCMI_AMP_CLASSES - 1));
        if (!amp_stage_grouped(c, m, st, y, acc, B, L)) {
            c.ar.release(smark);
            float* xj = c.ar.f((int64_t)B * L * cp);
            float* tmp = c.ar.f((int64_t)B * L * cp);
            float* tmp2 = c.ar.f((int64_t)B * L * cp);
            for (int j = 0; j < st.n_blocks; ++j) amp_block_seq(c, m, st, st.blocks[j], y, acc, xj, tmp, tmp2, j, st.n_blocks, B, L);
        }
        c.ar.release(smark);
        x = acc; cin = cp; t_in = L;
        if (stop_after == SVCMI_STOP_STAGE0 + i) { c.ar.release(mark); return; }
    }
    const svcmi_gen_stage& last = m.stages[m.n_stages - 1];
    c.prec = class_prec(m, SVCMI_CLASS_UPS);
    if (svcmi_snake_post_supported(last.c, cin, 7) && m.post.ldw >= 7 * cin) {
        run(c, OP_SNAKE_POST, 2.0 * B * t_in * last.c * 7, 4.0 * B * t_in * (last.c + 1), [&] {
            return svcmi_snake_post_f32(x, m.post.w, wave, m.post_alpha, m.post_beta, m.filt, B, (int32_t)t_in, last.c, cin, 7, c.stream);
        });
    } else {
        float* a = c.ar.f((int64_t)B * t_in * cin);
        snake_alias(c, m, x, a, Snk{m.post_alpha, m.post_beta}, B, t_in, cin, cin);
        CV v; v.x = a; v.x_bs = t_in * cin; v.B = B; v.t_in = (int)t_in; v.c_in = v.ldx = cin; v.w = &m.post; v.bias = false; v.n_out = 1;
        v.ksize = 7; v.pad = 3; v.act = SVCMI_ACT_TANH; v.y = wave; v.y_bs = t_in; v.ldy = 1;
        conv(c, v);
    }
    c.ar.release(mark);
}

constexpr int STREAM_HALO = 32;

void generator_fwd(Ctx& c, const svcmi_synth_model& m, const svcmi_synth_io& io, const float* z) {
    const int B = io.batch, T = io.t, S = io.stream_frames, U = m.upsample_input, hop = m.hop;
    if (S <= 0) { generator_tile(c, m, z, io.spk, io.source, io.wave, B, T, 0, io.stop_after); return; }
    const int64_t mark = c.ar.mark();
    const int tmax = S + 2 * STREAM_HALO < T ? S + 2 * STREAM_HALO : T;
    float* zt = c.ar.f((int64_t)B * tmax * U);
    float* st = c.ar.f((int64_t)B * tmax * hop);
    float* ot = c.ar.f((int64_t)B * tmax * hop);
    for (int t0 = 0; t0 < T; t0 += S) {
        const int a = t0 - STREAM_HALO > 0 ? t0 - STREAM_HALO : 0, b = t0 + S + STREAM_HALO < T ? t0 + S + STREAM_HALO : T;
        const int n = S < T - t0 ? S : T - t0, tt = b - a;
        copy2d(c, z + (int64_t)a * U, (int64_t)T * U, zt, (int64_t)tt * U, B, (int64_t)tt * U);
        copy2d(c, io.source + (int64_t)a * hop, (int64_t)T * hop, st, (int64_t)tt * hop, B, (int64_t)tt * hop);
        generator_tile(c, m, zt, io.spk, st, ot, B, tt, 1, SVCMI_STOP_NONE);
        copy2d(c, ot + (int64_t)(t0 - a) * hop, (int64_t)tt * hop, io.wave + (int64_t)t0 * hop, (int64_t)T * hop, B, (int64_t)n * hop);
    }
    c.ar.release(mark);
}

bool synth_shapes_ok(const svcmi_synth_model& m, const svcmi_synth_io& io) {
    if (m.precision < SVCMI_PREC_F32 || (m.precision > SVCMI_PREC_F16 && m.precision != SVCMI_PREC_MIXED && m.precision != SVCMI_PREC_F16W2)) return false;
    if (m.precision == SVCMI_PREC_MIXED)
        for (int i = 0; i < SVCMI_PREC_CLASSES; ++i)
            if ((m.class_prec[i] < SVCMI_PREC_F32 || m.class_prec[i] > SVCMI_PREC_F16) && m.class_prec[i] != SVCMI_PREC_F16W2) return false;
    return io.batch > 0 && io.t > 0 && m.n_enc >= 1 && m.n_enc <= SVCMI_MAX_ENC_LAYERS && m.n_flow >= 0 && m.n_flow <= SVCMI_MAX_FLOWS &&
           m.n_stages >= 1 && m.n_stages <= SVCMI_MAX_STAGES && m.hidden % 4 == 0 && m.inter % 8 == 0 && 2 * m.inter <= 3 * m.hidden &&
           m.upsample_input % 4 == 0 && (io.ppg_row_shift == 0 || io.ppg_row_shift == 1) && io.ppg_bstride % 4 == 0;
}

void synth_fwd(Ctx& c, const svcmi_synth_model& m, const svcmi_synth_io& io) {
    if (!synth_shapes_ok(m, io)) { c.rc = SVCMI_EINVAL; return; }
    const int B = io.batch, T = io.t, I = m.inter;
    c.lp_min_flops = m.lp_min_flops > 0.f ? m.lp_min_flops : 1.5e9f;
// ... 514 lines not shown
```

### whisper-vits-svc_amd/svcmi/_lib.py

```python
import ctypes
import os
from ctypes import POINTER, Structure, c_char_p, c_double, c_float, c_int, c_int32, c_int64, c_void_p

HERE = os.path.dirname(os.path.abspath(__file__))
DEFAULT_LIB = os.path.join(HERE, "libsvcmi.so")

ACT_NONE, ACT_RELU, ACT_GELU, ACT_MISH, ACT_TANH, ACT_SIGMOID = 0, 1, 2, 3, 4, 5
CONV_ACCUMULATE, CONV_MASK_IN, CONV_MASK_OUT, CONV_PARTIALS = 1, 2, 4, 8
ABI_VERSION = 22
PREC_F32, PREC_BF16X3, PREC_BF16, PREC_F16, PREC_BF16_A16, PREC_F16_A16, PREC_BF16X3_A16 = 0, 1, 2, 3, 4, 5, 6
PRECISIONS = {None: 0, "f32": 0, "fp32": 0, "bf16x3": 1, "bf16": 2, "f16": 3, "fp16": 3, "f16w2": 8}
PREC_F16W2, PREC_F16W2_A16 = 8, 9
PREC_MIXED = 7
PREC_CLASSES = 12
CLASS_ENC, CLASS_FLOW, CLASS_UPS, CLASS_AMP0 = 0, 1, 2, 3
AMP_CLASSES = 5
CLASS_NAMES = {"enc": 0, "flow": 1, "ups": 2, "amp0": 3, "amp1": 4, "amp2": 5, "amp3": 6, "amp4": 7, "encattn": 8}
MIXED_DEFAULT = {"enc": "bf16x3", "encattn": "f32", "ups": "bf16x3", "flow": "f16", "amp0": "bf16x3", "amp1": "f16", "amp2": "f16", "amp3": "f16w2", "amp4": "f16w2"}


def parse_precision(p):
    if isinstance(p, tuple):
        return p
    if isinstance(p, int) and not isinstance(p, bool):
        if p == PREC_MIXED:
            raise SvcmiError("precision code SVCMI_PREC_MIXED needs its per-class modes: pass \"mixed\", \"mixed:...\" or a dict")
        if p not in set(PRECISIONS.values()):
            raise SvcmiError(f"unknown precision code {p}")
        return (p, None)
    if (p is None or isinstance(p, str)) and p in PRECISIONS:
        return (PRECISIONS[p], None)
    pol = dict(MIXED_DEFAULT)
    if isinstance(p, dict):
        pol.update(p)
    elif isinstance(p, str) and (p == "mixed" or p.startswith("mixed:")):
        for item in filter(None, p[6:].split(",")):
            k, _, v = item.partition("=")
            pol[k.strip()] = v.strip()
    else:
        raise SvcmiError(f"unknown precision {p!r}")
    bad = [k for k in pol if k not in CLASS_NAMES] + [v for v in pol.values() if v not in PRECISIONS]
    if bad:
        raise SvcmiError(f"mixed precision policy: unknown class / mode {bad}; classes {sorted(CLASS_NAMES)}, modes f32 / bf16x3 / bf16 / f16 / f16w2")
    cls = [0] * PREC_CLASSES
    for k, v in pol.items():
        cls[CLASS_NAMES[k]] = PRECISIONS[v]
    return (PREC_MIXED, tuple(cls))
CONV_TILE_64x128 = 9


class SnakeConvDesc(Structure):
    _fields_ = [("x", c_void_p), ("w", c_void_p), ("bias", c_void_p), ("res", c_void_p), ("y", c_void_p),
                ("alpha_log", c_void_p), ("beta_log", c_void_p),
                ("ldw", c_int32), ("ksize", c_int32), ("dilation", c_int32), ("accumulate", c_int32), ("alpha", c_float)]


class ConvDesc(Structure):
    _fields_ = [
        ("x", c_void_p), ("w", c_void_p), ("bias", c_void_p), ("res", c_void_p), ("y", c_void_p), ("lengths", c_void_p),
        ("x_bstride", c_int64), ("y_bstride", c_int64), ("res_bstride", c_int64),
        ("batch", c_int32), ("t_in", c_int32), ("t_out", c_int32), ("c_in", c_int32), ("ldx", c_int32),
        ("n_out", c_int32), ("ldw", c_int32), ("ldy", c_int32), ("ldr", c_int32),
        ("ksize", c_int32), ("stride", c_int32), ("dilation", c_int32), ("pad", c_int32), ("x_row_shift", c_int32),
        ("act", c_int32), ("flags", c_int32), ("alpha", c_float), ("split_k", c_int32),
        ("workspace", c_void_p), ("workspace_floats", c_int64),
        ("counters", c_void_p), ("counters_len", c_int64),
        ("y16", c_void_p), ("y16_bstride", c_int64), ("ldy16", c_int32), ("y16_format", c_int32),
    ]


MAX_WHISPER_BLOCKS, MAX_ENC_LAYERS, MAX_FLOWS, MAX_WN_LAYERS, MAX_STAGES, MAX_AMP_BLOCKS, MAX_AMP_DILATIONS = 32, 8, 8, 8, 6, 3, 3
STOP_NONE, STOP_PRIOR, STOP_FLOW, STOP_GEN_PRE, STOP_STAGE0 = 0, 1, 2, 3, 4


class Weight(Structure):
    _fields_ = [("w", c_void_p), ("bias", c_void_p), ("w16", c_void_p), ("w16a", c_void_p), ("n", c_int32), ("ldw", c_int32),
                ("ldw16", c_int32), ("prec16", c_int32)]


class WhisperBlock(Structure):
    _fields_ = [("ln1_g", c_void_p), ("ln1_b", c_void_p), ("ln2_g", c_void_p), ("ln2_b", c_void_p),
                ("qkv", Weight), ("o", Weight), ("m1", Weight), ("m2", Weight)]


class WhisperModel(Structure):
    _fields_ = [("n_state", c_int32), ("n_heads", c_int32), ("n_layers", c_int32), ("n_mels", c_int32), ("n_ctx", c_int32),
                ("precision", c_int32), ("conv1", Weight), ("conv2", Weight), ("pos", c_void_p), ("lnp_g", c_void_p), ("lnp_b", c_void_p),
                ("blocks", WhisperBlock * MAX_WHISPER_BLOCKS),
                ("split_o", c_int32), ("split_mlp", c_int32), ("tile_qkv", c_int32), ("tile_o", c_int32), ("tile_mlp1", c_int32),
                ("tile_mlp2", c_int32), ("small_m_rows", c_int32), ("reserved", c_int32), ("lp_min_flops", c_float), ("reserved2", c_int32)]


class EncLayer(Structure):
    _fields_ = [("qkv", Weight), ("o", Weight), ("f1", Weight), ("f2", Weight), ("rel_k", c_void_p), ("rel_v", c_void_p),
                ("g1", c_void_p), ("b1", c_void_p), ("g2", c_void_p), ("b2", c_void_p)]


class WnLayer(Structure):
    _fields_ = [("in_", Weight), ("rs", Weight)]


class FlowLayer(Structure):
    _fields_ = [("x0_off", c_int32), ("x1_off", c_int32), ("n_wn", c_int32), ("reserved", c_int32),
                ("pre", Weight), ("post", Weight), ("snac", Weight), ("wn", WnLayer * MAX_WN_LAYERS)]


class AmpBlock(Structure):
    _fields_ = [("k", c_int32), ("n_dil", c_int32), ("dil", c_int32 * MAX_AMP_DILATIONS), ("reserved", c_int32),
                ("c1", Weight * MAX_AMP_DILATIONS), ("c2", Weight * MAX_AMP_DILATIONS),
                ("a1_alpha", c_void_p * MAX_AMP_DILATIONS), ("a1_beta", c_void_p * MAX_AMP_DILATIONS),
                ("a2_alpha", c_void_p * MAX_AMP_DILATIONS), ("a2_beta", c_void_p * MAX_AMP_DILATIONS)]


class GenStage(Structure):
    _fields_ = [("u", c_int32), ("c", c_int32), ("cp", c_int32), ("up_taps", c_int32), ("up_pad", c_int32), ("nz_k", c_int32),
                ("nz_stride", c_int32), ("nz_pad", c_int32), ("n_blocks", c_int32), ("reserved", c_int32),
                ("up", Weight), ("nz", Weight), ("blocks", AmpBlock * MAX_AMP_BLOCKS)]


class SynthModel(Structure):
    _fields_ = [("hidden", c_int32), ("inter", c_int32), ("n_heads", c_int32), ("enc_window", c_int32), ("enc_ffn_kernel", c_int32),
                ("flow_kernel", c_int32), ("n_enc", c_int32), ("n_flow", c_int32), ("n_stages", c_int32),
                ("ppg_dim", c_int32), ("vec_dim", c_int32), ("spk_dim", c_int32), ("upsample_input", c_int32), ("hop", c_int32),
                ("precision", c_int32), ("lp_min_flops", c_float), ("sampling_rate", c_float), ("merge_b", c_float),
                ("class_prec", c_int32 * PREC_CLASSES),
                ("pre", Weight), ("hub", Weight), ("proj", Weight), ("pit_emb", c_void_p),
                ("enc", EncLayer * MAX_ENC_LAYERS), ("flow", FlowLayer * MAX_FLOWS),
                ("adapter", Weight), ("conv_pre", Weight), ("post", Weight),
                ("merge_w", c_void_p), ("filt", c_void_p), ("post_alpha", c_void_p), ("post_beta", c_void_p),
                ("stages", GenStage * MAX_STAGES)]


class SynthIO(Structure):
    _fields_ = [("ppg", c_void_p), ("vec", c_void_p), ("pit", c_void_p), ("spk", c_void_p), ("lengths", c_void_p), ("source", c_void_p),
                ("noise", c_void_p), ("ppg_bstride", c_int64), ("ppg_row_shift", c_int32), ("batch", c_int32), ("t", c_int32),
                ("stream_frames", c_int32), ("stop_after", c_int32), ("reserved", c_int32),
                ("wave", c_void_p), ("z_p", c_void_p), ("z", c_void_p)]


SWEEP_MAX_KEYS = 32


class SweepIO(Structure):
    _fields_ = [("ppg", c_void_p), ("vec", c_void_p), ("pit", c_void_p), ("spk", c_void_p), ("length", c_void_p), ("source", c_void_p),
                ("noise", c_void_p), ("factors", c_double * SWEEP_MAX_KEYS), ("ppg_row_shift", c_int32), ("t", c_int32), ("n_keys", c_int32),
                ("stream_frames", c_int32), ("wave", c_void_p), ("pit_k", c_void_p)]


class LstmLayer(Structure):
    _fields_ = [("ih", Weight), ("lin", Weight), ("whh", c_void_p), ("reserved", c_void_p)]


MAX_LSTM_LAYERS = 8


class SpeakerModel(Structure):
    _fields_ = [("input_dim", c_int32), ("lstm_dim", c_int32), ("proj_dim", c_int32), ("n_layers", c_int32),
                ("layers", LstmLayer * MAX_LSTM_LAYERS)]


class VadConvBlock(Structure):
    _fields_ = [("dw_w", c_void_p), ("dw_b", c_void_p), ("pw_w", c_void_p), ("pw_b", c_void_p), ("proj_w", c_void_p), ("proj_b", c_void_p),
                ("c_in", c_int32), ("c_out", c_int32)]


class VadDown(Structure):
    _fields_ = [("w", c_void_p), ("b", c_void_p), ("scale", c_void_p), ("shift", c_void_p), ("c", c_int32), ("stride", c_int32)]


class VadModel(Structure):
    _fields_ = [("basis_t", c_void_p), ("filt", c_void_p), ("block", VadConvBlock * 4), ("down", VadDown * 4),
                ("gate0_w", c_void_p), ("gate0_b", c_void_p), ("whh0_t", c_void_p), ("wih1_t", c_void_p), ("whh1_t", c_void_p),
                ("gate1_b", c_void_p), ("dec_w", c_void_p), ("dec_b", c_float), ("reserved", c_int32)]


class SaliencePlan(Structure):
    _fields_ = [("basis", c_void_p), ("smooth", c_void_p), ("harm_off", c_void_p), ("harm_w", c_void_p),
                ("n_fft", c_int32), ("hop", c_int32), ("k_lo", c_int32), ("n_bins", c_int32),
                ("n_pitch", c_int32), ("smooth_len", c_int32), ("n_harm", c_int32), ("tol", c_int32),
                ("fs", c_float), ("f_min", c_float), ("f_max", c_float), ("bins_per_octave", c_float),
                ("thresh", c_double), ("log_hi", c_double), ("log_lo", c_double)]


SALIENCE_MAX_BINS = 1024


class PyinPlan(Structure):
    _fields_ = [("thresholds", c_void_p), ("beta", c_void_p), ("f_axis", c_void_p), ("band", c_void_p),
                ("n_fft", c_int32), ("hop", c_int32), ("p_min", c_int32), ("p_max", c_int32),
                ("n_pitch", c_int32), ("n_thr", c_int32), ("max_step", c_int32), ("reserved", c_int32),
                ("fs", c_double), ("tol_cents", c_double), ("absolute_min_prob", c_double), ("voicing_prob", c_double),
                ("log_tiny", c_double), ("log_cross", c_double), ("log_c", c_double), ("tiny", c_double)]


PYIN_MAX_BINS, PYIN_MAX_THRESHOLDS, PYIN_MAX_NFFT, PYIN_MAX_BAND = 1024, 128, 4096, 33


class YinPlan(Structure):
    _fields_ = [("n_fft", c_int32), ("hop", c_int32), ("lag_min", c_int32), ("lag_max", c_int32),
                ("fs", c_double), ("threshold", c_double), ("ratio_up", c_double), ("ratio_down", c_double)]


YIN_MAX_NFFT = 4096


class SwipeWindow(Structure):
    _fields_ = [("basis", c_void_p), ("resample", c_void_p), ("kernels", c_void_p), ("cand", c_void_p), ("mu", c_void_p),
                ("n_fft", c_int32), ("n_cand", c_int32)]


SWIPE_MAX_WINDOWS, SWIPE_MAX_NFFT, SWIPE_MAX_LOGBINS, SWIPE_MAX_CANDIDATES = 8, 4096, 1024, 1024


class SwipePlan(Structure):
    _fields_ = [("win", SwipeWindow * SWIPE_MAX_WINDOWS),
                ("n_win", c_int32), ("hop", c_int32), ("n_log", c_int32), ("n_pitch", c_int32),
                ("f_min", c_double), ("step", c_double), ("threshold", c_double)]


class TraceRecord(Structure):
    _fields_ = [("op", c_int32), ("ms", c_float), ("flops", c_double), ("bytes", c_double)]


_P, _I, _L, _F = c_void_p, c_int32, c_int64, c_float
SIGNATURES = {
    "svcmi_abi_version": (c_int, []),
    "svcmi_build_info": (c_char_p, []),
    "svcmi_conv_gemm_f32": (c_int, [POINTER(ConvDesc), _P]),
    "svcmi_pack_weights_lp": (c_int, [_P, _I, _I, _I, _P, _I, _P]),
    "svcmi_conv_gemm_lp": (c_int, [POINTER(ConvDesc), _I, _P]),
    "svcmi_conv_gemm_group_lp": (c_int, [_P, _I, _I, _P]),
    "svcmi_layernorm_f32": (c_int, [_P, _P, _P, _P, _P, _I, _I, _I, _I, _I, _I, _I, _F, _P, _I, _I, _P]),
    "svcmi_channel_norm_gelu_f32": (c_int, [_P, _P, _P, _P, _P, _I, _I, _I, _I, _I, _F, _P]),
    "svcmi_splitk_layernorm_f32": (c_int, [_P, _I, _P, _P, _P, _P, _P, _I, _I, _I, _I, _I, _F, _P, _I, _I, _P]),
    "svcmi_attention_f32": (c_int, [_P, _P, _P, _P, _I, _I, _I, _I, _L, _L, _L, _L, _I, _I, _I, _I, _F, _P, _P, _I, _P, _P, _I, _L, _I, _P]),
    "svcmi_attention16": (c_int, [_P, _P, _P, _I, _L, _P, _I, _L, _P, _I, _L, _I, _I, _I, _I, _F, _P, _P, _I, _P, _I, _P]),
    "svcmi_snake_alias_f32": (c_int, [_P, _P, _P, _P, _P, _I, _I, _I, _I, _P]),
    "svcmi_snake_conv_supported": (c_int, [_I, _I, _I, _I]),
    "svcmi_snake_conv_preferred": (c_int, [_I, _I, _I, _I]),
    "svcmi_snake_conv_f32": (c_int, [_P, _P, _P, _P, _P, _P, _P, _P, _I, _I, _I, _I, _I, _I, _I, _F, _I, _P]),
    "svcmi_upsample_noise_supported": (c_int, [_I, _I, _I]),
    "svcmi_upsample_noise_f32": (c_int, [_P, _P, _P, _P, _P, _P, _P, _I, _I, _I, _I, _I, _I, _I, _I, _L, _I, _I, _I, _I, _P]),
    "svcmi_tune_set": (c_int, [c_char_p, _I]),
    "svcmi_tune_get": (c_int, [c_char_p, POINTER(c_int32)]),
    "svcmi_wn_gate_f32": (c_int, [_P, _P, _P, _I, _I, _I, _I, _I, _I, _P]),
    "svcmi_wn_update_f32": (c_int, [_P, _P, _P, _P, _I, _I, _I, _I, _I, _I, _P]),
    "svcmi_coupling_pre_f32": (c_int, [_P, _I, _I, _P, _P, _I, _P, _I, _I, _I, _P]),
    "svcmi_coupling_post_f32": (c_int, [_P, _I, _I, _P, _I, _P, _P, _I, _I, _I, _P]),
    "svcmi_embed_pitch_f32": (c_int, [_P, _I, _P, _P, _P, _I, _I, _I, _P]),
    "svcmi_sample_prior_f32": (c_int, [_P, _I, _P, _P, _P, _I, _I, _I, _I, _P]),
    "svcmi_ncl_to_nlc_f32": (c_int, [_P, _P, _F, _P, _I, _I, _I, _I, _P]),
    "svcmi_nlc_to_ncl_f32": (c_int, [_P, _I, _P, _I, _I, _I, _P]),
    "svcmi_pitch_prefix_f64": (c_int, [_P, _P, _P, _I, _I, _I, _F, _P]),
    "svcmi_pitch_source_f32": (c_int, [_P, _P, _P, _P, _F, _P, _I, _I, _I, _F, _P]),
    "svcmi_reflect_pad_f32": (c_int, [_P, _P, _I, _L, _I, _P]),
    "svcmi_power_spectrum_f32": (c_int, [_P, _P, _L, _I, _I, _I, _I, _P]),
    "svcmi_logmel_finish_f32": (c_int, [_P, _P, _P, _I, _I, _I, _P]),
    "svcmi_pcm_resample_f32": (c_int, [_P, _I, _I, _L, _P, _I, _I, _I, _I, _P, _L, _P]),
    "svcmi_linear_spectrogram_f32": (c_int, [_P, _L, _I, _L, _P, _I, _I, _I, _F, _P, _L, _P]),
    "svcmi_stft_distance_workspace_bytes": (c_int64, [_I, _L, _I, _I, _I]),
    "svcmi_stft_distance_f32": (c_int, [_P, _L, _P, _L, _I, _L, _P, _I, _I, _I, _F, _L, _P, _L, _P, _P]),
    "svcmi_log_mel_f32": (c_int, [_P, _I, _I, _L, _P, _I, _I, _F, _P, _P]),
    "svcmi_abs_diff_sum_workspace_bytes": (c_int64, [_I, _L]),
    "svcmi_abs_diff_sum_f32": (c_int, [_P, _L, _P, _L, _I, _L, _P, _L, _P, _P]),
    "svcmi_lstm_step_f32": (c_int, [_P, _L, _P, _P, _L, _I, _P, _I, _I, _I, _I, _I, _P]),
    "svcmi_preemph_pad_f32": (c_int, [_P, _P, _I, _L, _I, _F, _P]),
    "svcmi_magnitude_spectrum_f32": (c_int, [_P, _P, _L, _I, _I, _I, _I, _P]),
    "svcmi_speaker_mel_finish_f32": (c_int, [_P, _L, _F, _F, _F, _P]),
    "svcmi_l2norm_rows_f32": (c_int, [_P, _L, _I, _I, _P, _L, _P]),
    "svcmi_group_mean_f32": (c_int, [_P, _I, _I, _I, _P, _P]),
    "svcmi_speaker_encoder_workspace_bytes": (c_int64, [POINTER(SpeakerModel), _I, _I]),
    "svcmi_speaker_encoder_fwd": (c_int, [POINTER(SpeakerModel), _P, _I, _I, _P, _P, _L, _P]),
    "svcmi_vad_model_bytes": (c_int64, []),
    "svcmi_vad_frontend_f32": (c_int, [POINTER(VadModel), _P, _P, _P, _I, _I, _P, _P, _P]),
    "svcmi_vad_lstm_scan_f32": (c_int, [POINTER(VadModel), _P, _P, _I, _I, _P, _P, _P]),
    "svcmi_mask_spans_f32": (c_int, [_P, _L, _P, _I, _L, _I, _P, _L, _P]),
    "svcmi_vad_workspace_bytes": (c_int64, [_I, _I]),
    "svcmi_vad_probs_fwd": (c_int, [POINTER(VadModel), _P, _P, _P, _I, _I, _P, _P, _P, _L, _P]),
    "svcmi_salience_plan_bytes": (c_int64, []),
    "svcmi_salience_stft_f32": (c_int, [POINTER(SaliencePlan), _P, _L, _P, _L, _P]),
    "svcmi_salience_map_f32": (c_int, [POINTER(SaliencePlan), _P, _L, _P, _P, _P, _P]),
    "svcmi_salience_dp_f64": (c_int, [_P, _L, _I, _I, c_double, c_double, _P, _P, _P]),
    "svcmi_salience_workspace_bytes": (c_int64, [POINTER(SaliencePlan), _L]),
    "svcmi_salience_f0_fwd": (c_int, [POINTER(SaliencePlan), _P, _L, _P, _P, _P, _L, _P]),
    "svcmi_pyin_plan_bytes": (c_int64, []),
    "svcmi_pyin_cmndf_f64": (c_int, [POINTER(PyinPlan), _P, _L, _P, _P, _L, _P]),
    "svcmi_pyin_observe_f64": (c_int, [POINTER(PyinPlan), _P, _L, _P, _P, _P, _P, _P]),
    "svcmi_pyin_viterbi_f64": (c_int, [_P, _L, _I, _I, _P, c_double, c_double, c_double, _P, _P, _P]),
    "svcmi_pyin_finish_f64": (c_int, [POINTER(PyinPlan), _P, _P, _P, _P, _P, _L, _P, _P, _P]),
    "svcmi_pyin_workspace_bytes": (c_int64, [POINTER(PyinPlan), _L]),
    "svcmi_pyin_f0_fwd": (c_int, [POINTER(PyinPlan), _P, _L, _P, _P, _P, _P, _P, _P, _P, _P, _L, _P]),
    "svcmi_yin_plan_bytes": (c_int64, []),
    "svcmi_yin_cmndf_f64": (c_int, [POINTER(YinPlan), _P, _L, _P, _P, _L, _P]),
    "svcmi_yin_pick_f64": (c_int, [POINTER(YinPlan), _P, _L, _P, _P, _P, _P, _P]),
    "svcmi_yin_aperiodicity_f64": (c_int, [POINTER(YinPlan), _P, _L, _P, _L, _P, _P]),
    "svcmi_yin_workspace_bytes": (c_int64, [POINTER(YinPlan), _L]),
    "svcmi_yin_f0_fwd": (c_int, [POINTER(YinPlan), _P, _L, _P, _P, _P, _P, _P, _P, _L, _P]),
    "svcmi_swipe_plan_bytes": (c_int64, []),
    "svcmi_swipe_frames": (c_int64, [POINTER(SwipePlan), _I, _L]),
    "svcmi_swipe_mag_f32": (c_int, [POINTER(SwipePlan), _I, _P, _L, _P, _P]),
    "svcmi_swipe_resample_f32": (c_int, [POINTER(SwipePlan), _I, _P, _L, _P, _P]),
    "svcmi_swipe_strength_f32": (c_int, [POINTER(SwipePlan), _I, _P, _L, _P, _P]),
    "svcmi_swipe_accum_f32": (c_int, [POINTER(SwipePlan), _P, _L, _P, _P]),
    "svcmi_swipe_finish_f64": (c_int, [_P, _L, _I, _I, c_double, c_double, c_double, _P, _P, _P, _P, _P]),
    "svcmi_swipe_workspace_bytes": (c_int64, [POINTER(SwipePlan), _L]),
    "svcmi_swipe_f0_fwd": (c_int, [POINTER(SwipePlan), _P, _L, _P, _P, _P, _P, _P, _L, _P]),
    "svcmi_crepe_frames_f32": (c_int, [_P, _L, _I, _I, _I, _P, _I, _P]),
    "svcmi_bn_maxpool2_f32": (c_int, [_P, _P, _P, _P, _L, _I, _I, _I, _P, _I, _I, _P]),
    "svcmi_viterbi_decode": (c_int, [_P, _P, _P, _P, _P, _I, _I, _I, _I, _I, _P]),
    "svcmi_row_sqnorm_f32": (c_int, [_P, _I, _L, _I, _P, _P]),
    "svcmi_knn_blend_f32": (c_int, [_P, _I, _P, _I, _P, _L, _P, _P, _I, _I, _I, _I, _I, _F, _P]),
    "svcmi_ivf_assign_f32": (c_int, [_P, _I, _P, _L, _P, _I, _I, _I, _P, _P, _P]),
    "svcmi_ivf_blend_f32": (c_int, [_P, _I, _P, _P, _P, _I, _P, _I, _I, _I, _I, _F, _P, _P, _P]),
    "svcmi_segment_mean_f32": (c_int, [_P, _I, _P, _P, _P, _I, _I, _I, _P]),
    "svcmi_snake_post_supported": (c_int, [_I, _I, _I]),
    "svcmi_snake_post_f32": (c_int, [_P, _P, _P, _P, _P, _P, _I, _I, _I, _I, _I, _P]),
    "svcmi_conv_gemm_group_f32": (c_int, [_P, _I, _P]),
    "svcmi_snake_conv_group_f32": (c_int, [_P, _I, _P, _I, _I, _I, _I, _P]),
    "svcmi_snake_conv_lp_supported": (c_int, [_I, _I, _I, _I, _I]),
    "svcmi_snake_conv_group_lp": (c_int, [_P, _I, _P, _I, _I, _I, _I, _I, _P]),
    "svcmi_snake_alias_group_f32": (c_int, [_P, _P, _P, _P, _P, _I, _I, _I, _I, _I, _P, _I, _P]),
    "svcmi_block_mean_f32": (c_int, [_P, _I, _P, _L, _P]),
    "svcmi_source2wav_i16": (c_int, [_P, _P, _L, _P]),
    "svcmi_whisper_workspace_bytes": (c_int64, [POINTER(WhisperModel), _I, _I]),
    "svcmi_whisper_encoder_fwd": (c_int, [POINTER(WhisperModel), _P, _P, _F, _I, _I, _P, _P, _L, _P]),
    "svcmi_synth_workspace_bytes": (c_int64, [POINTER(SynthModel), _I, _I, _I]),
    "svcmi_pitch2source_fwd": (c_int, [POINTER(SynthModel), _P, _P, _P, _I, _I, _P, _P, _L, _P]),
    "svcmi_text_encoder_fwd": (c_int, [POINTER(SynthModel), POINTER(SynthIO), _P, _P, _L, _P]),
    "svcmi_flow_reverse_fwd": (c_int, [POINTER(SynthModel), POINTER(SynthIO), _P, _P, _L, _P]),
    "svcmi_generator_fwd": (c_int, [POINTER(SynthModel), POINTER(SynthIO), _P, _P, _L, _P]),
    "svcmi_synth_infer_fwd": (c_int, [POINTER(SynthModel), POINTER(SynthIO), _P, _L, _P]),
    "svcmi_copy2d_f32": (c_int, [_P, _L, _P, _L, _L, _L, _P]),
    "svcmi_sweep_pitch_f32": (c_int, [_P, _P, _P, _I, _I, _P]),
    "svcmi_sweep_embed_f32": (c_int, [_P, _I, _P, _P, _P, _P, _I, _I, _I, _I, _P]),
    "svcmi_sweep_io_bytes": (c_int64, []),
    "svcmi_synth_sweep_workspace_bytes": (c_int64, [POINTER(SynthModel), _I, _I, _I]),
    "svcmi_synth_sweep_fwd": (c_int, [POINTER(SynthModel), POINTER(SweepIO), _P, _L, _P]),
    "svcmi_trace_begin": (c_int, [_I]),
    "svcmi_trace_end": (c_int, [POINTER(TraceRecord), _I]),
    "svcmi_trace_op_name": (c_char_p, [_I]),
    "svcmi_struct_sizes": (c_int, [POINTER(c_int64), _I]),
    "svcmi_packed_model_info": (c_int, [_P, _L, POINTER(c_int32), POINTER(c_int64), POINTER(c_int64)]),
    "svcmi_packed_model_bind": (c_int, [_P, _L, _P, _P, _L]),
}


class SvcmiError(RuntimeError):
    pass


def load_library(path=None):
    path = path or os.environ.get("SVCMI_LIB", DEFAULT_LIB)
    if not os.path.exists(path):
        raise SvcmiError(
            f"{path} not found: the HIP kernels are not built. Run `python whisper-vits-svc_amd/build.py` "
            "(hipcc --offload-arch=gfx950). svcmi has no CPU fallback.")
    lib = ctypes.CDLL(path)
    for name, (res, args) in SIGNATURES.items():
        try:
            fn = getattr(lib, name)
        except AttributeError as e:
            raise SvcmiError(f"{path} does not export {name}") from e
        fn.restype, fn.argtypes = res, args
    if lib.svcmi_abi_version() != ABI_VERSION:
        raise SvcmiError(f"ABI mismatch: library {lib.svcmi_abi_version()} vs binding {ABI_VERSION}")
    import ctypes as _c
    sizes = (c_int64 * 8)()
    n = lib.svcmi_struct_sizes(sizes, 8)
    mine = [_c.sizeof(t) for t in (Weight, WhisperModel, SynthModel, SynthIO, TraceRecord, ConvDesc, SnakeConvDesc)]
    if list(sizes[:n]) != mine:
        raise SvcmiError(f"struct layout mismatch: library {list(sizes[:n])} vs binding {mine}")
    if lib.svcmi_vad_model_bytes() != _c.sizeof(VadModel):
        raise SvcmiError(f"struct layout mismatch: svcmi_vad_model is {lib.svcmi_vad_model_bytes()} bytes in the library, {_c.sizeof(VadModel)} in the binding")
    if lib.svcmi_salience_plan_bytes() != _c.sizeof(SaliencePlan):
        raise SvcmiError(f"struct layout mismatch: svcmi_salience_plan is {lib.svcmi_salience_plan_bytes()} bytes in the library, {_c.sizeof(SaliencePlan)} in the binding")
    if lib.svcmi_pyin_plan_bytes() != _c.sizeof(PyinPlan):
        raise SvcmiError(f"struct layout mismatch: svcmi_pyin_plan is {lib.svcmi_pyin_plan_bytes()} bytes in the library, {_c.sizeof(PyinPlan)} in the binding")
    if lib.svcmi_yin_plan_bytes() != _c.sizeof(YinPlan):
        raise SvcmiError(f"struct layout mismatch: svcmi_yin_plan is {lib.svcmi_yin_plan_bytes()} bytes in the library, {_c.sizeof(YinPlan)} in the binding")
    if lib.svcmi_sweep_io_bytes() != _c.sizeof(SweepIO):
        raise SvcmiError(f"struct layout mismatch: svcmi_sweep_io is {lib.svcmi_sweep_io_bytes()} bytes in the library, {_c.sizeof(SweepIO)} in the binding")
    if lib.svcmi_swipe_plan_bytes() != _c.sizeof(SwipePlan):
        raise SvcmiError(f"struct layout mismatch: svcmi_swipe_plan is {lib.svcmi_swipe_plan_bytes()} bytes in the library, {_c.sizeof(SwipePlan)} in the binding")
    return lib
```

### whisper-vits-svc_amd/svcmi/cmodel.py

```python
from . import _lib
from ._lib import PREC_BF16, PREC_BF16X3, PREC_F16, PREC_F32
from .vits import consts as K


class CModel:

    def __init__(self, struct, keep):
        self.struct, self.keep = struct, keep


def _weight(cw, ops, w, bias, prec, keep, a16=False):
    cw.w, cw.bias = w.data_ptr(), (0 if bias is None else bias.data_ptr())
    cw.n, cw.ldw = int(w.shape[0]), int(w.shape[1])
    cw.w16, cw.w16a, cw.ldw16, cw.prec16 = 0, 0, 0, 0
    if prec != PREC_F32 and w.dim() == 2 and w.is_contiguous():
        base = PREC_F16 if prec == _lib.PREC_F16W2 else prec
        img = ops.lp_weight(w, base)
        cw.w16, cw.ldw16, cw.prec16 = img.data_ptr(), img.shape[1] // (2 if prec == PREC_BF16X3 else 1), prec
        keep.append(img)
        if a16:
            a16_code = {PREC_BF16X3: _lib.PREC_BF16X3_A16, _lib.PREC_F16W2: _lib.PREC_F16W2_A16}.get(prec, prec + 2)
            img_a = ops.lp_weight(w, a16_code)
            cw.w16a = img_a.data_ptr()
            keep.append(img_a)
    keep.append(w)
    keep.append(bias)


def whisper_cmodel(w, ops, prec=PREC_F32):
    m, keep = _lib.WhisperModel(), [w]
    if w.n_layers > _lib.MAX_WHISPER_BLOCKS:
        raise _lib.SvcmiError(f"{w.n_layers} encoder blocks > {_lib.MAX_WHISPER_BLOCKS}")
    m.n_state, m.n_heads, m.n_layers, m.n_mels = w.S, w.heads, w.n_layers, w.n_mels
    m.n_ctx, m.precision = int(w.pos.shape[0]), prec
    x3 = prec == PREC_BF16X3
    _weight(m.conv1, ops, w.conv1_w, w.conv1_b, prec, keep)
    _weight(m.conv2, ops, w.conv2_w, w.conv2_b, prec, keep)
    m.pos, m.lnp_g, m.lnp_b = w.pos.data_ptr(), w.lnp_g.data_ptr(), w.lnp_b.data_ptr()
    for i, b in enumerate(w.blocks):
        cb = m.blocks[i]
        cb.ln1_g, cb.ln1_b, cb.ln2_g, cb.ln2_b = (b[k].data_ptr() for k in ("ln1_g", "ln1_b", "ln2_g", "ln2_b"))
        _weight(cb.qkv, ops, b["qkv_w"], b["qkv_b"], prec, keep, a16=True)
        _weight(cb.o, ops, b["o_w"], b["o_b"], prec, keep, a16=not x3)
        _weight(cb.m1, ops, b["m1_w"], b["m1_b"], prec, keep, a16=not x3)
        _weight(cb.m2, ops, b["m2_w"], b["m2_b"], prec, keep, a16=not x3)
    return CModel(m, keep)


def speaker_cmodel(w, ops):
    m, keep = _lib.SpeakerModel(), [w]
    if len(w.layers) > _lib.MAX_LSTM_LAYERS:
        raise _lib.SvcmiError(f"{len(w.layers)} LSTM layers > {_lib.MAX_LSTM_LAYERS}")
    m.input_dim, m.lstm_dim, m.proj_dim, m.n_layers = w.input_dim, w.lstm_dim, w.proj_dim, len(w.layers)
    for i, ly in enumerate(w.layers):
        _weight(m.layers[i].ih, ops, ly["ih_w"], ly["bias"], PREC_F32, keep)
        _weight(m.layers[i].lin, ops, ly["lin_w"], None, PREC_F32, keep)
        m.layers[i].whh = ly["whh"].data_ptr()
        keep.append(ly["whh"])
    return CModel(m, keep)


def synth_cmodel(w, ops, prec=PREC_F32):
    code, classes = prec if isinstance(prec, tuple) else (prec, None)
    m, keep = _lib.SynthModel(), [w]
    hp = w.hp
    if len(w.enc) > _lib.MAX_ENC_LAYERS or len(w.flow) > _lib.MAX_FLOWS or len(w.stages) > _lib.MAX_STAGES:
        raise _lib.SvcmiError("model exceeds the fixed capacities of svcmi_synth_model")
    m.hidden, m.inter, m.n_heads = w.H, w.I, w.n_heads
    m.enc_window, m.enc_ffn_kernel, m.flow_kernel = K.ENC_WINDOW, K.ENC_FFN_KERNEL, K.FLOW_KERNEL
    m.n_enc, m.n_flow, m.n_stages = len(w.enc), len(w.flow), len(w.stages)
    m.ppg_dim, m.vec_dim, m.spk_dim = hp.vits.ppg_dim, hp.vits.vec_dim, hp.vits.spk_dim
    m.upsample_input, m.hop = w.U, w.hop
    m.precision, m.lp_min_flops = code, 0.0
    for i in range(_lib.PREC_CLASSES):
        m.class_prec[i] = classes[i] if classes else 0
    m.sampling_rate, m.merge_b = float(hp.data.sampling_rate), float(w.merge_b)
    state = {"cls": _lib.CLASS_ENC}

    def W(cw, wt, b=None, a16=False):
        p = classes[state["cls"]] if classes else code
        _weight(cw, ops, wt, b, p, keep, a16=a16 and p != PREC_BF16X3)
    W(m.pre, w.pre_w, w.pre_b)
    W(m.hub, w.hub_w, w.hub_b)
    W(m.proj, w.proj_w, w.proj_b)
    m.pit_emb = w.pit_emb.data_ptr()
    for i, L in enumerate(w.enc):
        e = m.enc[i]
        W(e.qkv, L["qkv_w"], L["qkv_b"], a16=True)
        W(e.o, L["o_w"], L["o_b"], a16=True)
        W(e.f1, L["f1_w"], L["f1_b"], a16=True)
        W(e.f2, L["f2_w"], L["f2_b"], a16=True)
        e.rel_k, e.rel_v = L["rel_k"].data_ptr(), L["rel_v"].data_ptr()
        e.g1, e.b1, e.g2, e.b2 = (L[k].data_ptr() for k in ("g1", "b1", "g2", "b2"))
    state["cls"] = _lib.CLASS_FLOW
    for i, L in enumerate(w.flow):
        f = m.flow[i]
        if len(L["wn"]) > _lib.MAX_WN_LAYERS:
            raise _lib.SvcmiError("too many WN layers")
        f.x0_off, f.x1_off, f.n_wn = L["x0_off"], L["x1_off"], len(L["wn"])
        W(f.pre, L["pre_w"], L["pre_b"])
        W(f.post, L["post_w"], L["post_b"])
        W(f.snac, L["snac_w"], L["snac_b"])
        for l, Wl in enumerate(L["wn"]):
            W(f.wn[l].in_, Wl["in_w"], Wl["in_b"])
            W(f.wn[l].rs, Wl["rs_w"], Wl["rs_b"])
    state["cls"] = _lib.CLASS_UPS
    W(m.adapter, w.ad_w, w.ad_b)
    W(m.conv_pre, w.pre_conv_w, w.pre_conv_b)
    W(m.post, w.post_w, None)
    m.merge_w, m.filt = w.merge_w.data_ptr(), w.filt.data_ptr()
    m.post_alpha, m.post_beta = w.post_a[0].data_ptr(), w.post_a[1].data_ptr()
    for i, st in enumerate(w.stages):
        s = m.stages[i]
        if len(st["blocks"]) > _lib.MAX_AMP_BLOCKS:
            raise _lib.SvcmiError("more AMP blocks per stage than svcmi_gen_stage holds")
        s.u, s.c, s.cp, s.up_taps, s.up_pad = st["u"], st["c"], st["cp"], st["up_taps"], st["up_pad"]
        s.nz_k, s.nz_stride, s.nz_pad, s.n_blocks = st["nz_k"], st["nz_stride"], st["nz_pad"], len(st["blocks"])
        state["cls"] = _lib.CLASS_UPS
        W(s.up, st["up_w"], st["up_b"])
        W(s.nz, st["nz_w"], st["nz_b"])
        state["cls"] = _lib.CLASS_AMP0 + min(i, _lib.AMP_CLASSES - 1)
        for j, blk in enumerate(st["blocks"]):
            b = s.blocks[j]
            if len(blk["d"]) > _lib.MAX_AMP_DILATIONS:
                raise _lib.SvcmiError("more dilations per AMP block than svcmi_amp_block holds")
            b.k, b.n_dil = blk["k"], len(blk["d"])
            for q, d in enumerate(blk["d"]):
                b.dil[q] = d
                W(b.c1[q], blk["c1"][q][0], blk["c1"][q][1], a16=st["cp"] % 8 == 0)
                W(b.c2[q], blk["c2"][q][0], blk["c2"][q][1], a16=st["cp"] % 8 == 0)
                b.a1_alpha[q], b.a1_beta[q] = blk["a1"][q][0].data_ptr(), blk["a1"][q][1].data_ptr()
                b.a2_alpha[q], b.a2_beta[q] = blk["a2"][q][0].data_ptr(), blk["a2"][q][1].data_ptr()
    return CModel(m, keep)


def vad_cmodel(w):
    m, keep = _lib.VadModel(), [w]
    m.basis_t, m.filt = w.basis_t.data_ptr(), w.filt.data_ptr()
    for i, blk in enumerate(w.blocks):
        b = m.block[i]
        b.c_in, b.c_out = blk["c_in"], blk["c_out"]
        for k in ("dw_w", "dw_b", "pw_w", "pw_b", "proj_w", "proj_b"):
            setattr(b, k, 0 if blk[k] is None else blk[k].data_ptr())
    for i, dn in enumerate(w.downs):
        d = m.down[i]
        d.c, d.stride = dn["c"], dn["stride"]
        for k in ("w", "b", "scale", "shift"):
            setattr(d, k, dn[k].data_ptr())
    for k in ("gate0_w", "gate0_b", "whh0_t", "wih1_t", "whh1_t", "gate1_b", "dec_w"):
        setattr(m, k, getattr(w, k).data_ptr())
    m.dec_b = w.dec_b
    return CModel(m, keep)
```

### whisper-vits-svc_amd/svcmi/ops.py

```python
import contextlib
import ctypes
import os
import threading

import torch

from . import _lib
from ._lib import (ACT_GELU, ACT_MISH, ACT_NONE, ACT_RELU, ACT_SIGMOID, ACT_TANH, CONV_ACCUMULATE, CONV_MASK_IN,
                   CONV_MASK_OUT, CONV_PARTIALS, PREC_BF16, PREC_BF16X3, PREC_F16, PREC_F32, PRECISIONS, ConvDesc, SnakeConvDesc, SvcmiError,
                   SynthIO, TraceRecord)


SPLIT16 = "bf16x3"


def _fmt16(dtype):
    return {torch.bfloat16: PREC_BF16, torch.float16: PREC_F16, SPLIT16: PREC_BF16X3}[dtype]


def _alloc16(lead, c, out16, device):
    if out16 == SPLIT16:
        cp = (c + 7) // 8 * 8
        return (torch.zeros if cp != c else torch.empty)(*lead, 2 * cp, dtype=torch.bfloat16, device=device)
    return torch.empty(*lead, c, dtype=out16, device=device)
# ... 399 lines not shown
    def layernorm(self, x, gamma=None, beta=None, *, res=None, eps=1e-5, per_batch_affine=False, out=None, out16=None):
        self._chk(x, gamma, beta, res, out)
        B, T, Cc = x.shape
        if out is None:
            out = torch.empty_like(x)
        y16 = _alloc16((B, T), Cc, out16, x.device) if out16 is not None else None
        self._call("svcmi_layernorm_f32", _ptr(x), _ptr(res), _ptr(gamma), _ptr(beta), _ptr(out), B, T, Cc,
                   x.stride(1), res.stride(1) if res is not None else 0, out.stride(1),
                   (gamma.stride(0) if gamma is not None else beta.stride(0)) if per_batch_affine else 0, eps,
                   _ptr(y16), y16.stride(1) if y16 is not None else 0, _fmt16(out16) if out16 is not None else 0, self._stream())
        return out if out16 is None else (out, y16)

    def channel_norm_gelu(self, x, gamma, beta, eps=1e-5, out=None):
        self._chk(x, gamma, beta, out)
        B, T, Cc = x.shape
        if out is None:
            out = torch.empty_like(x)
        scratch = torch.empty(B * 129 * Cc, dtype=torch.float64, device=x.device)
        self._call("svcmi_channel_norm_gelu_f32", _ptr(x), _ptr(gamma), _ptr(beta), _ptr(out), _ptr(scratch), B, T, Cc,
                   x.stride(1), out.stride(1), eps, self._stream())
        return out

    def splitk_layernorm(self, partials, bias, x, gamma, beta, *, eps=1e-5, out=None, out16=None):
        self._chk(partials, bias, x, gamma, beta, out)
        B, S, T, Cc = partials.shape
        if out is None:
            out = torch.empty_like(x)
        y16 = _alloc16((B, T), Cc, out16, x.device) if out16 is not None else None
        self._call("svcmi_splitk_layernorm_f32", _ptr(partials), S, _ptr(bias), _ptr(x), _ptr(gamma), _ptr(beta), _ptr(out),
                   B, T, Cc, x.stride(1), out.stride(1), eps, _ptr(y16), y16.stride(1) if y16 is not None else 0,
                   _fmt16(out16) if out16 is not None else 0, self._stream())
        return out if out16 is None else (out, y16)

    def attention(self, qkv, heads, scale, *, rel_k=None, rel_v=None, window=0, lengths=None, out=None, out16=None):
        self._chk(qkv, rel_k, rel_v, lengths, out)
        B, T, C3 = qkv.shape
        Cc = C3 // 3
        if out is None:
            out = torch.empty(B, T, Cc, dtype=torch.float32, device=qkv.device)
        base = qkv.data_ptr()
        bs = qkv.stride(0)
        o16 = _alloc16((B, T), Cc, out16, qkv.device) if out16 is not None else None
        self._call("svcmi_attention_f32", base, base + 4 * Cc, base + 8 * Cc, _ptr(out), C3, C3, C3, out.stride(1),
                   bs, bs, bs, out.stride(0), B, T, heads, Cc // heads, scale, _ptr(rel_k), _ptr(rel_v), window,
                   _ptr(lengths), _ptr(o16), o16.stride(1) if o16 is not None else 0, o16.stride(0) if o16 is not None else 0,
                   _fmt16(out16) if out16 is not None else 0, self._stream(),
                   work={"flops": 4.0 * B * T * T * Cc})
        return out if out16 is None else (out, o16)

    def attention16(self, qkv16, heads, scale, *, rel_k=None, rel_v=None, window=0, lengths=None, want_f32=True):
        self._chk(qkv16, lengths, rel_k, rel_v)
        B, T, C3 = qkv16.shape
        Cc = C3 // 3
        o = torch.empty(B, T, Cc, dtype=torch.float32, device=qkv16.device) if want_f32 else None
        o16 = torch.empty(B, T, Cc, dtype=qkv16.dtype, device=qkv16.device)
        base, esz = qkv16.data_ptr(), 2
        self._call("svcmi_attention16", base, base + esz * Cc, base + 2 * esz * Cc, C3, qkv16.stride(0), _ptr(o), Cc, T * Cc, _ptr(o16), Cc, T * Cc,
                   B, T, heads, Cc // heads, scale, _ptr(rel_k), _ptr(rel_v), window, _ptr(lengths), _fmt16(qkv16.dtype), self._stream(),
                   work={"flops": 4.0 * B * T * T * Cc})
        return o, o16

    def snake_alias(self, x, alpha_log, beta_log, filt, out=None):
        self._chk(x, alpha_log, beta_log, filt, out)
        B, L, Cc = x.shape
        if out is None:
            out = torch.empty_like(x)
        self._call("svcmi_snake_alias_f32", _ptr(x), _ptr(out), _ptr(alpha_log), _ptr(beta_log), _ptr(filt),
                   B, L, Cc, x.stride(1), self._stream(), work={"bytes": 8.0 * B * L * Cc})
        return out

    def snake_alias_group(self, xs, alpha_logs, beta_logs, filt, outs):
        self._chk(*xs, *alpha_logs, *beta_logs, filt, *outs)
        n = len(xs)
        B, L, Cc = xs[0].shape
        arr = lambda ts: (ctypes.c_void_p * n)(*[t.data_ptr() for t in ts])
        if outs[0].dtype != torch.float32:
            split = outs[0].dtype == torch.bfloat16 and outs[0].shape[-1] == 2 * xs[0].stride(1)
            self._call("svcmi_snake_alias_group_f32", arr(xs), None, arr(alpha_logs), arr(beta_logs), _ptr(filt), n,
                       B, L, Cc, xs[0].stride(1), arr(outs), _fmt16(SPLIT16 if split else outs[0].dtype), self._stream(),
                       work={"bytes": (8.0 if split else 6.0) * n * B * L * Cc})
            return outs
        self._call("svcmi_snake_alias_group_f32", arr(xs), arr(outs), arr(alpha_logs), arr(beta_logs), _ptr(filt), n,
                   B, L, Cc, xs[0].stride(1), None, 0, self._stream(), work={"bytes": 8.0 * n * B * L * Cc})
        return outs

    def block_mean(self, xs, out=None):
        self._chk(*xs, out)
        if out is None:
            out = torch.empty_like(xs[0])
        arr = (ctypes.c_void_p * len(xs))(*[t.data_ptr() for t in xs])
        self._call("svcmi_block_mean_f32", arr, len(xs), _ptr(out), xs[0].numel(), self._stream(),
                   work={"bytes": 4.0 * (len(xs) + 1) * xs[0].numel()})
        return out

    def upsample_noise_supported(self, u, cp, cin):
        return bool(self.lib.svcmi_upsample_noise_supported(u, cp, cin))

    def upsample_noise(self, x, up_w, up_b, taps, pad, u, cp, src, nz_w, nz_b, nz_k, nz_stride, nz_pad, y=None):
        self._chk(x, up_w, up_b, src, nz_w, nz_b, y)
        noise_only = y is not None
        if noise_only:
            B, t_in, cin = y.shape[0], y.shape[1] // u, 4
        else:
            B, t_in, cin = x.shape
            y = torch.empty(B, t_in * u, cp, dtype=torch.float32, device=x.device)
        self._call("svcmi_upsample_noise_f32", 0 if noise_only else _ptr(x), _ptr(up_w), _ptr(up_b), _ptr(src), _ptr(nz_w),
                   _ptr(nz_b), _ptr(y), B, t_in, cin, up_w.shape[1] if up_w is not None else 0, taps, pad, u, cp, src.shape[1],
                   nz_k, nz_stride, nz_pad, nz_w.shape[1], self._stream(), work={"bytes": 4.0 * B * t_in * (cin + u * cp)})
        return y

    def snake_conv_supported(self, c, ld, ksize, dilation):
        return bool(self.lib.svcmi_snake_conv_supported(c, ld, ksize, dilation))

    def snake_conv_preferred(self, c, ld, ksize, dilation):
        return bool(self.lib.svcmi_snake_conv_preferred(c, ld, ksize, dilation))

    def snake_conv(self, x, alpha_log, beta_log, filt, w, bias, *, c, ksize, dilation=1, res=None, alpha=1.0,
                   accumulate=False, out=None):
        self._chk(x, alpha_log, beta_log, filt, w, bias, res, out)
        B, L, ld = x.shape
        if out is None:
            out = torch.empty_like(x)
        self._call("svcmi_snake_conv_f32", _ptr(x), _ptr(w), _ptr(bias), _ptr(res), _ptr(out), _ptr(alpha_log),
                   _ptr(beta_log), _ptr(filt), B, L, c, ld, w.shape[1], ksize, dilation, float(alpha), int(accumulate),
                   self._stream(), work={"flops": 2.0 * B * L * c * c * ksize, "bytes": 8.0 * B * L * c})
        return out

    def snake_post_supported(self, c, ld, ksize):
        return bool(self.lib.svcmi_snake_post_supported(c, ld, ksize))

    def snake_post(self, x, alpha_log, beta_log, filt, w, *, c, ksize):
        self._chk(x, alpha_log, beta_log, filt, w)
        B, L, ld = x.shape
        out = torch.empty(B, L, dtype=torch.float32, device=x.device)
        self._call("svcmi_snake_post_f32", _ptr(x), _ptr(w), _ptr(out), _ptr(alpha_log), _ptr(beta_log), _ptr(filt), B, L, c, ld,
                   ksize, self._stream(), work={"flops": 2.0 * B * L * c * ksize, "bytes": 4.0 * B * L * (c + 1)})
        return out

    def snake_conv_group(self, problems, filt, *, c, precision=None):
        descs = (SnakeConvDesc * len(problems))()
        B, L, ld = problems[0]["x"].shape
        flops = 0.0
        for i, pr in enumerate(problems):
            self._chk(pr["x"], pr["alpha_log"], pr["beta_log"], pr["w"], pr.get("bias"), pr.get("res"), pr["out"])
            d = descs[i]
            d.x, d.w, d.bias, d.res, d.y = _ptr(pr["x"]), _ptr(pr["w"]), _ptr(pr.get("bias")), _ptr(pr.get("res")), _ptr(pr["out"])
            d.alpha_log, d.beta_log = _ptr(pr["alpha_log"]), _ptr(pr["beta_log"])
            d.ldw, d.ksize, d.dilation = pr["w"].shape[1], pr["ksize"], pr.get("dilation", 1)
            d.accumulate, d.alpha = int(pr.get("accumulate", False)), float(pr.get("alpha", 1.0))
            flops += 2.0 * B * L * c * c * pr["ksize"]
        if precision is not None:
            self._call("svcmi_snake_conv_group_lp", descs, len(problems), _ptr(filt), B, L, c, ld, PRECISIONS[precision], self._stream(),
                       work={"flops": flops, "bytes": 8.0 * len(problems) * B * L * c})
        else:
            self._call("svcmi_snake_conv_group_f32", descs, len(problems), _ptr(filt), B, L, c, ld, self._stream(),
                       work={"flops": flops, "bytes": 8.0 * len(problems) * B * L * c})
        return [pr["out"] for pr in problems]

    def pitch2source(self, f0, rand_ini, noise, merge_w, merge_b, hop, sr):
        self._chk(f0, rand_ini, noise, merge_w)
        B, T = f0.shape
        prefix = torch.empty(B, T, 11, dtype=torch.float64, device=f0.device)
        self._call("svcmi_pitch_prefix_f64", _ptr(f0), _ptr(rand_ini), _ptr(prefix), B, T, hop, float(sr), self._stream())
        out = torch.empty(B, T * hop, dtype=torch.float32, device=f0.device)
        self._call("svcmi_pitch_source_f32", _ptr(f0), _ptr(prefix), _ptr(noise), _ptr(merge_w), float(merge_b),
                   _ptr(out), B, T, hop, float(sr), self._stream())
        return out

    def reflect_pad(self, x, pad):
        self._chk(x)
        B, n = x.shape
        y = torch.empty(B, n + 2 * pad, dtype=torch.float32, device=x.device)
        self._call("svcmi_reflect_pad_f32", _ptr(x), _ptr(y), B, n, pad, self._stream())
        return y

    def power_spectrum(self, ri, nbins, half):
        self._chk(ri)
        B, T, ld = ri.shape
        p = torch.empty(B, T, half, dtype=torch.float32, device=ri.device)
        self._call("svcmi_power_spectrum_f32", _ptr(ri), _ptr(p), B * T, nbins, half, ld, half, self._stream())
        return p

    def logmel_finish(self, mel_power):
        self._chk(mel_power)
        B, T, Cc = mel_power.shape
        scratch = torch.empty(B * 64, dtype=torch.float32, device=mel_power.device)
        out = torch.empty(B, Cc, T, dtype=torch.float32, device=mel_power.device)
        self._call("svcmi_logmel_finish_f32", _ptr(mel_power), _ptr(scratch), _ptr(out), B, T, Cc, self._stream())
        return out

    def pcm_resample(self, pcm, fmt, channels, taps, up, down, half):
        self._chk(pcm, taps)
        pcm = pcm.contiguous()
        if 0 <= fmt <= 3 and pcm.element_size() != (4, 2, 4, 1)[fmt]:
            raise SvcmiError(f"pcm_resample: fmt {fmt} does not describe a {pcm.dtype} tensor")
        if taps is not None and not (taps.dtype == torch.float32 and taps.is_contiguous() and taps.dim() == 2 and taps.shape[0] == up):
            raise SvcmiError("pcm_resample: taps must be a contiguous float32 [up, K] image")
        frames = pcm.numel() // max(int(channels), 1)
        n_out = -(-frames * up // down) if up >= 1 and down >= 1 else 0
        out = torch.empty(max(n_out, 0), dtype=torch.float32, device=pcm.device)
        self._call("svcmi_pcm_resample_f32", _ptr(pcm), fmt, channels, frames, _ptr(taps), up, down,
                   taps.shape[1] if taps is not None else 0, half, _ptr(out), n_out, self._stream(),
                   work={"bytes": float(pcm.numel() * pcm.element_size() + 4 * n_out)})
        return out

    def linear_spectrogram(self, x, basis, n_fft, hop, pad, eps=1e-6, out=None):
        self._chk(x, basis, out)
        if not (x.dim() == 2 and x.dtype == torch.float32 and (x.shape[1] <= 1 or x.stride(1) == 1)):
            raise SvcmiError("linear_spectrogram: x must be float32 [B, n] with unit stride along n")
        bins = n_fft // 2 + 1
        if not (basis.dtype == torch.float32 and basis.is_contiguous() and tuple(basis.shape) == (n_fft, 2 * bins)):
            raise SvcmiError("linear_spectrogram: basis must be a contiguous float32 [n_fft, n_fft + 2] table")
        B, n = x.shape
        frames = 1 + (n + 2 * pad - n_fft) // hop if hop >= 1 and n + 2 * pad >= n_fft else 0
        if out is None:
            out = torch.empty(B, bins, max(frames, 0), dtype=torch.float32, device=x.device)
        elif not (out.dtype == torch.float32 and out.is_contiguous() and tuple(out.shape) == (B, bins, frames)):
            raise SvcmiError("linear_spectrogram: out must be a contiguous float32 [B, bins, frames] tensor")
        self._call("svcmi_linear_spectrogram_f32", _ptr(x), x.stride(0), B, n, _ptr(basis), n_fft, hop, pad, float(eps), _ptr(out), frames,
                   self._stream(), work={"flops": 4.0 * B * frames * bins * n_fft, "bytes": 4.0 * (B * n + basis.numel() + out.numel())})
        return out

    def stft_distance(self, x, y, basis, n_fft, hop, pad=None, floor=1e-7, out=None, workspace=None):
        self._chk(x, y, basis, out, workspace)
        for name, t in (("x", x), ("y", y)):
            if not (t.dim() == 2 and t.dtype == torch.float32 and (t.shape[1] <= 1 or t.stride(1) == 1)):
                raise SvcmiError(f"stft_distance: {name} must be float32 [B, n] with unit stride along n")
        if x.shape != y.shape or x.device != y.device:
            raise SvcmiError(f"stft_distance: x {tuple(x.shape)} on {x.device} and y {tuple(y.shape)} on {y.device} differ")
        bins = n_fft // 2 + 1
        if not (basis.dtype == torch.float32 and basis.is_contiguous() and tuple(basis.shape) == (n_fft, 2 * bins)):
            raise SvcmiError("stft_distance: basis must be a contiguous float32 [n_fft, n_fft + 2] table")
        B, n = x.shape
        pad = n_fft // 2 if pad is None else pad
        frames = 1 + (n + 2 * pad - n_fft) // hop if hop >= 1 and n + 2 * pad >= n_fft else 0
        need = self.stft_distance_workspace(B, n, n_fft, hop, pad)
        if workspace is None:
            workspace = torch.empty(max(need, 1), dtype=torch.float32, device=x.device)
        elif not (workspace.dtype == torch.float32 and workspace.is_contiguous() and workspace.numel() >= need):
            raise SvcmiError(f"stft_distance: workspace must be a contiguous float32 tensor of at least {need} elements")
        if out is None:
            out = torch.empty(B, 3, dtype=torch.float64, device=x.device)
        elif not (out.dtype == torch.float64 and out.is_contiguous() and tuple(out.shape) == (B, 3)):
            raise SvcmiError("stft_distance: out must be a contiguous float64 [B, 3] tensor")
        self._call("svcmi_stft_distance_f32", _ptr(x), x.stride(0), _ptr(y), y.stride(0), B, n, _ptr(basis), n_fft, hop, pad, float(floor), frames,
                   _ptr(workspace), 4 * workspace.numel(), _ptr(out), self._stream(),
                   work={"flops": 8.0 * B * frames * bins * n_fft, "bytes": 4.0 * (2 * B * n + basis.numel())})
        return out

    def stft_distance_workspace(self, batch, n, n_fft, hop, pad=None):
        nbytes = self.lib.svcmi_stft_distance_workspace_bytes(batch, n, n_fft, hop, n_fft // 2 if pad is None else pad)
        if nbytes < 0:
            raise SvcmiError(f"stft_distance: batch {batch}, n {n}, n_fft {n_fft}, hop {hop}, pad {pad} is not a valid geometry (code {nbytes})")
        return nbytes // 4

    def log_mel(self, spec, melT, n_mel, clip=1e-5, out=None):
        self._chk(spec, melT, out)
        if not (spec.dim() == 3 and spec.dtype == torch.float32 and spec.is_contiguous()):
            raise SvcmiError("log_mel: spec must be a contiguous float32 [B, bins, frames] tensor")
        B, bins, frames = spec.shape
        if not (melT.dim() == 2 and melT.dtype == torch.float32 and melT.is_contiguous() and melT.shape[0] == bins
                and melT.shape[1] >= (n_mel + 31) // 32 * 32):
            raise SvcmiError("log_mel: melT must be a contiguous float32 [bins, ldm] table, ldm >= n_mel rounded up to 32")
        if out is None:
            out = torch.empty(B, n_mel, frames, dtype=torch.float32, device=spec.device)
        elif not (out.dtype == torch.float32 and out.is_contiguous() and tuple(out.shape) == (B, n_mel, frames)):
            raise SvcmiError("log_mel: out must be a contiguous float32 [B, n_mel, frames] tensor")
        self._call("svcmi_log_mel_f32", _ptr(spec), B, bins, frames, _ptr(melT), melT.shape[1], n_mel, float(clip), _ptr(out), self._stream(),
                   work={"flops": 2.0 * B * frames * bins * n_mel, "bytes": 4.0 * (spec.numel() + melT.numel() + out.numel())})
        return out

    def abs_diff_sum(self, a, b, out=None):
        self._chk(a, b, out)
        if a.shape != b.shape or a.dim() < 2 or a.dtype != torch.float32 or b.dtype != torch.float32 or a.device != b.device:
            raise SvcmiError("abs_diff_sum: a and b must be float32 tensors [B, ...] of one shape on one device")
        if not (a[0].is_contiguous() and b[0].is_contiguous()):
            raise SvcmiError("abs_diff_sum: every batch item must be contiguous")
        B, count = a.shape[0], a[0].numel()
        nbytes = self.lib.svcmi_abs_diff_sum_workspace_bytes(B, count)
        if nbytes < 0:
            raise SvcmiError(f"abs_diff_sum: batch {B} x {count} elements is not a valid shape")
        workspace = torch.empty(nbytes // 4, dtype=torch.float32, device=a.device)
        if out is None:
            out = torch.empty(B, dtype=torch.float64, device=a.device)
        elif not (out.dtype == torch.float64 and out.is_contiguous() and tuple(out.shape) == (B,)):
            raise SvcmiError("abs_diff_sum: out must be a contiguous float64 [B] tensor")
        self._call("svcmi_abs_diff_sum_f32", _ptr(a), a.stride(0), _ptr(b), b.stride(0), B, count, _ptr(workspace), nbytes, _ptr(out), self._stream(),
                   work={"bytes": 8.0 * B * count})
        return out

    def lstm_step(self, gx, whh, hseq, c, t):
        self._chk(gx, whh, hseq, c)
        B, T, H = hseq.shape
        self._call("svcmi_lstm_step_f32", _ptr(gx), gx.stride(0), _ptr(whh), _ptr(hseq), hseq.stride(0), hseq.stride(1), _ptr(c), c.stride(0),
                   B, H, t, T, self._stream(), work={"flops": 8.0 * B * H * H if t else 0.0, "bytes": 16.0 * H * H if t else 0.0})
        return hseq

    def preemph_pad(self, x, pad, coef):
        self._chk(x)
        B, n = x.shape
        y = torch.empty(B, n + 2 * pad, dtype=torch.float32, device=x.device)
        self._call("svcmi_preemph_pad_f32", _ptr(x), _ptr(y), B, n, pad, float(coef), self._stream())
        return y

    def magnitude_spectrum(self, ri, nbins, half):
        self._chk(ri)
# ... 476 lines not shown
```

### whisper-vits-svc_amd/svcmi/weights.py

```python
import math

import torch


def _round4(n):
    return (n + 3) // 4 * 4


def fold_weight_norm(sd, name):
    v, g = sd[name + ".weight_v"].float(), sd[name + ".weight_g"].float()
    n = v.flatten(1).norm(dim=1).view(-1, *([1] * (v.dim() - 1)))
    return g * v / n


def pack_conv(w, cin_pad=None, n_pad=None):
    N, Cin, Kk = w.shape
    cin_pad = cin_pad or Cin
    n_pad = n_pad or N
    p = torch.zeros(n_pad, Kk, cin_pad, dtype=torch.float32, device=w.device)
    p[:N, :, :Cin] = w.float().permute(0, 2, 1)
    p = p.reshape(n_pad, Kk * cin_pad)
    ldw = _round4(p.shape[1])
    if ldw != p.shape[1]:
        p = torch.cat([p, torch.zeros(n_pad, ldw - p.shape[1], dtype=torch.float32, device=w.device)], dim=1)
    return p.contiguous()


def pad_vec(v, n_pad):
    out = torch.zeros(n_pad, dtype=torch.float32, device=v.device)
    out[:v.shape[0]] = v.float()
    return out


def pack_conv_transpose(w, bias, u, p, cin_pad=None, cout_pad=None):
    Cin, Cout, Kk = w.shape
    cin_pad = cin_pad or Cin
    cout_pad = cout_pad or Cout
    js = [j for r in range(u) for j in range(-Kk, Kk + 1) if 0 <= u * j + r + p < Kk]
    jmin, jmax = min(js), max(js)
    taps = jmax - jmin + 1
    W = torch.zeros(u, cout_pad, taps, cin_pad, dtype=torch.float32, device=w.device)
    for r in range(u):
        for j in range(jmin, jmax + 1):
            kk = u * j + r + p
            if 0 <= kk < Kk:
                W[r, :Cout, jmax - j, :Cin] = w[:, :, kk].float().t()
    b = torch.zeros(u, cout_pad, dtype=torch.float32, device=w.device)
    b[:, :Cout] = bias.float()[None, :]
    return W.reshape(u * cout_pad, taps * cin_pad).contiguous(), b.reshape(-1).contiguous(), taps, jmax


class VitsWeights:

    def __init__(self, sd, hp, device):
        from .vits import consts as K
        f = lambda t: t.float().to(device).contiguous()
        H, I = hp.vits.hidden_channels, hp.vits.inter_channels
        self.hp = hp
        self.H, self.I, self.half = H, I, I // 2
        self.n_heads = K.ENC_HEADS
        self.pre_w, self.pre_b = f(pack_conv(sd["enc_p.pre.weight"])), f(sd["enc_p.pre.bias"])
        self.hub_w, self.hub_b = f(pack_conv(sd["enc_p.hub.weight"])), f(sd["enc_p.hub.bias"])
        self.pit_emb = f(sd["enc_p.pit.weight"])
        self.enc = []
        for i in range(K.ENC_LAYERS):
            a = f"enc_p.enc.attn_layers.{i}"
            qkv_w = torch.cat([sd[a + ".conv_q.weight"], sd[a + ".conv_k.weight"], sd[a + ".conv_v.weight"]], 0)
            qkv_b = torch.cat([sd[a + ".conv_q.bias"], sd[a + ".conv_k.bias"], sd[a + ".conv_v.bias"]], 0)
            self.enc.append(dict(
                qkv_w=f(pack_conv(qkv_w)), qkv_b=f(qkv_b),
                o_w=f(pack_conv(sd[a + ".conv_o.weight"])), o_b=f(sd[a + ".conv_o.bias"]),
                rel_k=f(sd[a + ".emb_rel_k"][0]), rel_v=f(sd[a + ".emb_rel_v"][0]),
                g1=f(sd[f"enc_p.enc.norm_layers_1.{i}.gamma"]), b1=f(sd[f"enc_p.enc.norm_layers_1.{i}.beta"]),
                f1_w=f(pack_conv(sd[f"enc_p.enc.ffn_layers.{i}.conv_1.weight"])), f1_b=f(sd[f"enc_p.enc.ffn_layers.{i}.conv_1.bias"]),
                f2_w=f(pack_conv(sd[f"enc_p.enc.ffn_layers.{i}.conv_2.weight"])), f2_b=f(sd[f"enc_p.enc.ffn_layers.{i}.conv_2.bias"]),
                g2=f(sd[f"enc_p.enc.norm_layers_2.{i}.gamma"]), b2=f(sd[f"enc_p.enc.norm_layers_2.{i}.beta"])))
        self.proj_w, self.proj_b = f(pack_conv(sd["enc_p.proj.weight"])), f(sd["enc_p.proj.bias"])
        half = self.half
        self.flow = []
        flipped = False
        for fl in reversed(range(K.FLOW_N)):
            flipped = not flipped
            p = f"flow.flows.{2 * fl}"
            pre_w, post_w, post_b = sd[p + ".pre.weight"].float(), sd[p + ".post.weight"].float(), sd[p + ".post.bias"].float()
            snac_w, snac_b = sd[p + ".snac.weight"].float()[:, :, 0], sd[p + ".snac.bias"].float()
            m_w, v_w, m_b, v_b = snac_w[:half], snac_w[half:], snac_b[:half], snac_b[half:]
            if flipped:
                pre_w = pre_w.flip(1)
                post_w, post_b = post_w.flip(0), post_b.flip(0)
                m_w, v_w, m_b, v_b = m_w.flip(0), v_w.flip(0), m_b.flip(0), v_b.flip(0)
            layer = dict(x0_off=half if flipped else 0, x1_off=0 if flipped else half,
                         pre_w=f(pack_conv(pre_w, n_pad=2 * H)), pre_b=f(pad_vec(sd[p + ".pre.bias"], 2 * H)),
                         post_w=f(pack_conv(post_w)), post_b=f(post_b),
                         snac_w=f(pack_conv(torch.cat([m_w, v_w], 0).unsqueeze(-1))), snac_b=f(torch.cat([m_b, v_b], 0)),
                         wn=[])
            for l in range(K.FLOW_WN_LAYERS):
                layer["wn"].append(dict(
                    in_w=f(pack_conv(fold_weight_norm(sd, f"{p}.enc.in_layers.{l}"))), in_b=f(sd[f"{p}.enc.in_layers.{l}.bias"]),
                    rs_w=f(pack_conv(fold_weight_norm(sd, f"{p}.enc.res_skip_layers.{l}"))), rs_b=f(sd[f"{p}.enc.res_skip_layers.{l}.bias"])))
            self.flow.append(layer)
        assert not flipped, "an even number of Flip modules leaves the tensor un-permuted"
        g = hp.gen
        self.rates, self.up_k = list(g.upsample_rates), list(g.upsample_kernel_sizes)
        self.rk = list(g.resblock_kernel_sizes)
        self.rd = [list(d) for d in g.resblock_dilation_sizes]
        self.hop = int(math.prod(self.rates))
        self.ad_w = f(pack_conv(torch.cat([sd["dec.adapter.W_scale.weight"], sd["dec.adapter.W_bias.weight"]], 0).unsqueeze(-1)))
        self.ad_b = f(torch.cat([sd["dec.adapter.W_scale.bias"], sd["dec.adapter.W_bias.bias"]], 0))
        self.U = g.upsample_input
        self.pre_conv_w, self.pre_conv_b = f(pack_conv(sd["dec.conv_pre.weight"])), f(sd["dec.conv_pre.bias"])
        self.merge_w = f(sd["dec.m_source.merge_w"].view(-1))
        self.merge_b = float(sd["dec.m_source.merge_b"].view(-1)[0])
        self.filt = f(sd["dec.activation_post.upsample.filter"].view(-1))
        C0 = g.upsample_initial_channel
        self.stages = []
        for i, (u, k) in enumerate(zip(self.rates, self.up_k)):
            cin, cout = C0 // (2 ** i), C0 // (2 ** (i + 1))
            cin_p, cout_p = _round4(cin), _round4(cout)
            up_w, up_b, taps, upad = pack_conv_transpose(fold_weight_norm(sd, f"dec.ups.{i}"), sd[f"dec.ups.{i}.bias"],
                                                         u, (k - u) // 2, cin_p, cout_p)
            nw = sd[f"dec.noise_convs.{i}.weight"]
            s = int(math.prod(self.rates[i + 1:])) if i + 1 < len(self.rates) else 1
            st = dict(u=u, c=cout, cp=cout_p, up_w=f(up_w), up_b=f(up_b), up_taps=taps, up_pad=upad,
                      nz_w=f(pack_conv(nw, n_pad=cout_p)), nz_b=f(pad_vec(sd[f"dec.noise_convs.{i}.bias"], cout_p)),
                      nz_k=nw.shape[2], nz_stride=s, nz_pad=(s // 2 if i + 1 < len(self.rates) else 0), blocks=[])
            for j, kk in enumerate(self.rk):
                b = f"dec.resblocks.{i * len(self.rk) + j}"
                blk = dict(k=kk, d=self.rd[j], c1=[], c2=[], a1=[], a2=[])
                for q in range(3):
                    blk["c1"].append((f(pack_conv(fold_weight_norm(sd, f"{b}.convs1.{q}"), cout_p, cout_p)), f(pad_vec(sd[f"{b}.convs1.{q}.bias"], cout_p))))
                    blk["c2"].append((f(pack_conv(fold_weight_norm(sd, f"{b}.convs2.{q}"), cout_p, cout_p)), f(pad_vec(sd[f"{b}.convs2.{q}.bias"], cout_p))))
                    blk["a1"].append((f(pad_vec(sd[f"{b}.activations.{2 * q}.act.alpha"], cout_p)), f(pad_vec(sd[f"{b}.activations.{2 * q}.act.beta"], cout_p))))
                    blk["a2"].append((f(pad_vec(sd[f"{b}.activations.{2 * q + 1}.act.alpha"], cout_p)), f(pad_vec(sd[f"{b}.activations.{2 * q + 1}.act.beta"], cout_p))))
                st["blocks"].append(blk)
            self.stages.append(st)
        cl = self.stages[-1]["cp"]
        self.post_a = (f(pad_vec(sd["dec.activation_post.act.alpha"], cl)), f(pad_vec(sd["dec.activation_post.act.beta"], cl)))
        self.post_w = f(pack_conv(sd["dec.conv_post.weight"], cin_pad=cl))


class WhisperWeights:

    def __init__(self, ckpt, device):
        dims, sd = ckpt["dims"], ckpt["model_state_dict"]
        f = lambda t: t.float().to(device).contiguous()
        self.dims = dict(dims) if isinstance(dims, dict) else dict(vars(dims))
        S, L = self.dims["n_audio_state"], self.dims["n_audio_layer"]
        self.S, self.heads = S, self.dims["n_audio_head"]
        self.n_layers = L - L // 4
        self.n_mels = self.dims["n_mels"]
        self.conv1_w, self.conv1_b = f(pack_conv(sd["encoder.conv1.weight"])), f(sd["encoder.conv1.bias"])
        self.conv2_w, self.conv2_b = f(pack_conv(sd["encoder.conv2.weight"])), f(sd["encoder.conv2.bias"])
        self.pos = f(sd["encoder.positional_embedding"]) if "encoder.positional_embedding" in sd else None
        self.blocks = []
        zeros = torch.zeros(S)
        for i in range(self.n_layers):
            b = f"encoder.blocks.{i}"
            qkv_w = torch.cat([sd[b + ".attn.query.weight"], sd[b + ".attn.key.weight"], sd[b + ".attn.value.weight"]], 0)
            qkv_b = torch.cat([sd[b + ".attn.query.bias"].float().cpu(), zeros, sd[b + ".attn.value.bias"].float().cpu()], 0)
            self.blocks.append(dict(
                ln1_g=f(sd[b + ".attn_ln.weight"]), ln1_b=f(sd[b + ".attn_ln.bias"]),
                qkv_w=f(qkv_w), qkv_b=f(qkv_b),
                o_w=f(sd[b + ".attn.out.weight"]), o_b=f(sd[b + ".attn.out.bias"]),
                ln2_g=f(sd[b + ".mlp_ln.weight"]), ln2_b=f(sd[b + ".mlp_ln.bias"]),
                m1_w=f(sd[b + ".mlp.0.weight"]), m1_b=f(sd[b + ".mlp.0.bias"]),
                m2_w=f(sd[b + ".mlp.2.weight"]), m2_b=f(sd[b + ".mlp.2.bias"])))
        self.lnp_g, self.lnp_b = f(sd["encoder.ln_post.weight"]), f(sd["encoder.ln_post.bias"])


class HubertWeights:

    def __init__(self, sd, device):
        f = lambda t: t.float().to(device).contiguous()
        self.conv0_w = f(pack_conv(sd["feature_extractor.conv0.weight"]))
        self.norm0_g, self.norm0_b = f(sd["feature_extractor.norm0.weight"]), f(sd["feature_extractor.norm0.bias"])
        self.convs = []
        i = 1
        while f"feature_extractor.conv{i}.weight" in sd:
            w = sd[f"feature_extractor.conv{i}.weight"]
            self.convs.append((f(pack_conv(w)), int(w.shape[2])))
            i += 1
        self.fp_g, self.fp_b = f(sd["feature_projection.norm.weight"]), f(sd["feature_projection.norm.bias"])
        self.fp_w = f(pack_conv(sd["feature_projection.projection.weight"].unsqueeze(-1)))
        self.fp_b2 = f(sd["feature_projection.projection.bias"])
        v, g = sd["positional_embedding.conv.weight_v"].float(), sd["positional_embedding.conv.weight_g"].float()
        w = g * v / v.pow(2).sum(dim=(0, 1), keepdim=True).sqrt()
        self.E, self.pos_k = int(v.shape[0]), int(v.shape[2])
        self.G = self.E // int(v.shape[1])
        cg = self.E // self.G
        pb = sd["positional_embedding.conv.bias"].float()
        self.pos_w = [f(pack_conv(w[gi * cg:(gi + 1) * cg])) for gi in range(self.G)]
        self.pos_b = [f(pb[gi * cg:(gi + 1) * cg]) for gi in range(self.G)]
        self.norm_g, self.norm_b = f(sd["norm.weight"]), f(sd["norm.bias"])
        self.layers = []
        i = 0
        while f"encoder.layers.{i}.norm1.weight" in sd:
            p = f"encoder.layers.{i}."
            self.layers.append(dict(
                in_w=f(pack_conv(sd[p + "self_attn.in_proj_weight"].unsqueeze(-1))), in_b=f(sd[p + "self_attn.in_proj_bias"]),
                out_w=f(pack_conv(sd[p + "self_attn.out_proj.weight"].unsqueeze(-1))), out_b=f(sd[p + "self_attn.out_proj.bias"]),
                l1_w=f(pack_conv(sd[p + "linear1.weight"].unsqueeze(-1))), l1_b=f(sd[p + "linear1.bias"]),
                l2_w=f(pack_conv(sd[p + "linear2.weight"].unsqueeze(-1))), l2_b=f(sd[p + "linear2.bias"]),
                n1_g=f(sd[p + "norm1.weight"]), n1_b=f(sd[p + "norm1.bias"]),
                n2_g=f(sd[p + "norm2.weight"]), n2_b=f(sd[p + "norm2.bias"])))
            i += 1
        self.heads = 12 if self.E == 768 else self.E // 16
        self.proj_w, self.proj_b = f(pack_conv(sd["proj.weight"].unsqueeze(-1))), f(sd["proj.bias"])


CREPE_FRAME_ROWS = 256
CREPE_DENSE_MAX_ROWS = 32


class CrepeWeights:

    def __init__(self, sd, device, eps=0.0010000000474974513):
        f = lambda t: t.float().to(device).contiguous()
        self.layers = []
        i = 1
        while f"conv{i}.weight" in sd:
            w = sd[f"conv{i}.weight"].float()[:, :, :, 0]
            if i == 1:
                packed = w[:, 0, :].contiguous()
            else:
                packed = pack_conv(w)
            g, b = sd[f"conv{i}_BN.weight"].float(), sd[f"conv{i}_BN.bias"].float()
            mu, var = sd[f"conv{i}_BN.running_mean"].float(), sd[f"conv{i}_BN.running_var"].float()
            scale = g / torch.sqrt(var + eps)
            layer = dict(w=f(packed), b=f(sd[f"conv{i}.bias"]), scale=f(scale), shift=f(b - mu * scale))
            t_in = CREPE_FRAME_ROWS >> (i - 1)
            if i > 1 and t_in <= CREPE_DENSE_MAX_ROWS:
                n_out, c_in, taps = w.shape
                ti = torch.arange(t_in)
                k = ti[None, :] - ti[:, None] + (taps // 2 - 1)
                assert int(k.min()) >= 0 and int(k.max()) < taps
                dense = w[:, :, k].permute(2, 0, 3, 1).reshape(t_in * n_out, t_in * c_in)
                layer.update(dense_w=f(dense), dense_b=f(sd[f"conv{i}.bias"].float().repeat(t_in)), t_in=t_in)
            self.layers.append(layer)
            i += 1
        self.fc_w = f(pack_conv(sd["classifier.weight"].float().unsqueeze(-1)))
        self.fc_b = f(sd["classifier.bias"])


LSTM_UNIT_TILE = 4


def lstm_tile_order(hidden, unit_tile=LSTM_UNIT_TILE):
    if hidden % unit_tile:
        raise ValueError(f"lstm_dim {hidden} is not a multiple of the kernel's unit tile {unit_tile}")
    j = torch.arange(hidden).view(hidden // unit_tile, 1, unit_tile)
    q = torch.arange(4).view(1, 4, 1)
    return (q * hidden + j).reshape(-1)


class SpeakerWeights:

    def __init__(self, sd, device):
        f = lambda t: t.detach().float().to(device).contiguous()
        n = 0
        while f"layers.{n}.lstm.weight_ih_l0" in sd:
            n += 1
        if n == 0:
            raise KeyError("no layers.N.lstm.weight_ih_l0 in the state dict: not an LSTMSpeakerEncoder with projection layers")
        self.layers = []
        for i in range(n):
            p = f"layers.{i}"
            w_ih, w_hh = sd[p + ".lstm.weight_ih_l0"].float(), sd[p + ".lstm.weight_hh_l0"].float()
            H = w_hh.shape[1]
            perm = lstm_tile_order(H).to(w_ih.device)
            bias = sd[p + ".lstm.bias_ih_l0"].float() + sd[p + ".lstm.bias_hh_l0"].float()
            self.layers.append(dict(ih_w=f(pack_conv(w_ih[perm].unsqueeze(-1))), whh=f(w_hh[perm]), bias=f(bias[perm]),
                                    lin_w=f(pack_conv(sd[p + ".linear.weight"].float().unsqueeze(-1)))))
        self.input_dim = int(sd["layers.0.lstm.weight_ih_l0"].shape[1])
        self.lstm_dim = int(sd["layers.0.lstm.weight_hh_l0"].shape[1])
        self.proj_dim = int(sd["layers.0.linear.weight"].shape[0])
        for d in (self.input_dim, self.lstm_dim, self.proj_dim):
            if d % 4:
                raise ValueError(f"speaker encoder dimension {d} is not a multiple of 4")


VAD_BLOCKS = (("first_layer.0", 258, 16), ("encoder.3.0", 16, 32), ("encoder.7.0", 32, 32), ("encoder.11.0", 32, 64))
VAD_DOWNS = (("encoder.0", "encoder.1", 16, 2), ("encoder.4", "encoder.5", 32, 2), ("encoder.8", "encoder.9", 32, 2), ("encoder.12", "encoder.13", 64, 1))
VAD_HIDDEN = 64
VAD_BASIS_LD = 260


# ... 40 lines not shown
```

Baseline: 1500 audio-seconds/sec.

## Add pair-ordered f32 weight image for small-channel fused snake-conv kernels

Adds a new weight layout for the c=10 and c=20 AMP resblock convolutions. The weights are repacked so each group's output-channel pairs sit contiguously, which lets the kernel fetch them as wide uniform (scalar) loads and apply them with packed 2-wide FMAs. The goal is to cut per-element weight indexing and scalar FMA issue in the last upsample stages. The new path is enabled by default for the f32 fused group path. It adds extra packed weight copies and more kernel template instantiations, and it changes the dispatch branches for the u-kernel versus the plain kernel.

```diff
diff --git a/include/svcmi.h b/include/svcmi.h
--- a/include/svcmi.h
+++ b/include/svcmi.h
@@ -67,7 +67,8 @@
 enum svcmi_precision { SVCMI_PREC_F32 = 0, SVCMI_PREC_BF16X3 = 1, SVCMI_PREC_BF16 = 2, SVCMI_PREC_F16 = 3,
                        SVCMI_PREC_BF16_A16 = 4, SVCMI_PREC_F16_A16 = 5, SVCMI_PREC_BF16X3_A16 = 6,
                        SVCMI_PREC_MIXED = 7,
-                       SVCMI_PREC_F16W2 = 8, SVCMI_PREC_F16W2_A16 = 9 };
+                       SVCMI_PREC_F16W2 = 8, SVCMI_PREC_F16W2_A16 = 9,
+                       SVCMI_PREC_F32_PAIRS = 10 };
 int svcmi_pack_weights_lp(const float* w, int32_t n, int32_t ldw, int32_t precision, void* out, int32_t ldw16, void* stream);
 int svcmi_conv_gemm_lp(const svcmi_conv_desc* d, int32_t precision, void* stream);
 int svcmi_conv_gemm_group_lp(const svcmi_conv_desc* descs, int32_t count, int32_t precision, void* stream);
@@ -117,6 +118,8 @@
 } svcmi_snake_conv_desc;
 int svcmi_snake_conv_group_f32(const svcmi_snake_conv_desc* descs, int32_t count, const float* filt, int32_t batch,
                                int32_t len, int32_t c, int32_t ld, void* stream);
+int svcmi_snake_conv_group_pairs_f32(const svcmi_snake_conv_desc* descs, const float* const* wpairs, int32_t count, const float* filt,
+                                     int32_t batch, int32_t len, int32_t c, int32_t ld, void* stream);
 
 int svcmi_snake_conv_lp_supported(int32_t c, int32_t ld, int32_t ksize, int32_t dilation, int32_t precision);
 int svcmi_snake_conv_group_lp(const svcmi_snake_conv_desc* descs, int32_t count, const float* filt, int32_t batch,
diff --git a/whisper-vits-svc_amd/csrc/amp_fused.hip b/whisper-vits-svc_amd/csrc/amp_fused.hip
--- a/whisper-vits-svc_amd/csrc/amp_fused.hip
+++ b/whisper-vits-svc_amd/csrc/amp_fused.hip
@@ -37,6 +37,41 @@
     const float* alpha_log; const float* beta_log; const float* filt;
     int n, ld, ldw, dil, accumulate, ks;
     float alpha;
+    const float* wp;
+};
+
+template <int CR>
+struct PairImage {
+    static constexpr int NC4 = (CR + 3) / 4, NG = CR / CO, SLICE = 4 * CO;
+    static constexpr int TAP = NC4 * NG * SLICE;
+    static_assert(CR % CO == 0, "whole groups of CO output channels");
+};
+template <int NCI>
+struct PairSlice {
+#ifndef SVCMI_EMU
+    typedef float f32x8 __attribute__((ext_vector_type(8)));
+    svcmi_f32x16 a, b;
+    f32x8 c;
+    __device__ __forceinline__ void load(const float* q) {
+        if constexpr (NCI == 4) {
+            a = *(const __attribute__((address_space(4))) svcmi_f32x16*)(q);
+            b = *(const __attribute__((address_space(4))) svcmi_f32x16*)(q + 16);
+            c = *(const __attribute__((address_space(4))) f32x8*)(q + 32);
+        } else {
+            static_assert(NCI == 2, "10 channels: the last slice holds two");
+            a = *(const __attribute__((address_space(4))) svcmi_f32x16*)(q);
+            const svcmi_f32x4 t = svcmi_load_uniform4(q + 16);
+            b[0] = t[0]; b[1] = t[1]; b[2] = t[2]; b[3] = t[3];
+        }
+    }
+    __device__ __forceinline__ svcmi_f32x2 pair(int k) const {
+        return k < 8 ? svcmi_f32x2{a[2 * k], a[2 * k + 1]} : k < 16 ? svcmi_f32x2{b[2 * k - 16], b[2 * k - 15]} : svcmi_f32x2{c[2 * k - 32], c[2 * k - 31]};
+    }
+#else
+    const float* q_;
+    void load(const float* q) { q_ = q; }
+    svcmi_f32x2 pair(int k) const { return svcmi_f32x2{q_[2 * k], q_[2 * k + 1]}; }
+#endif
 };
 
 template <bool H16, int LS>
@@ -168,7 +203,7 @@
     static constexpr int ROWS = TB + (KS - 1) * DMAX;
 };
 
-template <int CP, int CR, int KS_T, int G, int TT, bool UT = false>
+template <int CP, int CR, int KS_T, int G, int TT, bool UT = false, bool PW = false>
 __device__ __forceinline__ void snake_conv_body(const AmpArgs& p, float* S) {
     using TL = AmpTile<CP, G, TT, KS_T ? KS_T : 11>;
     const int KS = KS_T ? KS_T : p.ks;
@@ -214,6 +249,40 @@
             }
         }
     }
+    if constexpr (PW) {
+        using PI = PairImage<CR>;
+        static_assert(G * CO == CR, "every group owns CO real output channels");
+        const float* wpg = p.wp + g * PI::SLICE;
+        for (int tap = 0; tap < KS; ++tap) {
+            const float* srow = S + (tl0 + tap * d) * LS;
+            const float* wt = wpg + tap * PI::TAP;
+#pragma unroll
+            for (int c4 = 0; c4 < PI::NC4; ++c4) {
+                constexpr int LAST = CR - 4 * (PI::NC4 - 1);
+                svcmi_f32x2 x01[TT], x23[TT];
+#pragma unroll
+                for (int j = 0; j < TT; ++j) {
+                    const float4 xin = *reinterpret_cast<const float4*>(srow + j * 64 * LS + 4 * c4);
+                    x01[j] = svcmi_f32x2{xin.x, xin.y}; x23[j] = svcmi_f32x2{xin.z, xin.w};
+                }
+                auto slice = [&](auto& ws) {
+                    ws.load(wt + c4 * (PI::NG * PI::SLICE));
+#pragma unroll
+                    for (int c = 0; c < NCO; c += 2) {
+#pragma unroll
+                        for (int j = 0; j < TT; ++j) {
+                            acc[j][c / 2] = svcmi_fma2(svcmi_splat_lo(x01[j]), ws.pair(c / 2), acc[j][c / 2]);
+                            if (4 * c4 + 1 < CR) acc[j][c / 2] = svcmi_fma2(svcmi_splat_hi(x01[j]), ws.pair(NCO / 2 + c / 2), acc[j][c / 2]);
+                            if (4 * c4 + 2 < CR) acc[j][c / 2] = svcmi_fma2(svcmi_splat_lo(x23[j]), ws.pair(NCO + c / 2), acc[j][c / 2]);
+                            if (4 * c4 + 3 < CR) acc[j][c / 2] = svcmi_fma2(svcmi_splat_hi(x23[j]), ws.pair(3 * NCO / 2 + c / 2), acc[j][c / 2]);
+                        }
+                    }
+                };
+                if (LAST == 4 || c4 + 1 < PI::NC4) { PairSlice<4> ws; slice(ws); }
+                else { PairSlice<LAST == 4 ? 4 : 2> ws; slice(ws); }
+            }
+        }
+    } else {
     const float* wg = p.w + (long long)co0 * p.ldw;
     for (int tap = 0; tap < KS; ++tap) {
         const float* srow = S + (tl0 + tap * d) * LS;
@@ -241,6 +310,7 @@
                 }
             }
         }
+    }
     }
 
     float* yb = p.y + (long long)b * n * ld;
@@ -284,20 +354,20 @@
     AmpArgs p[AMP_GROUP];
 };
 
-template <int CP, int CR, int G, int TT>
+template <int CP, int CR, int G, int TT, bool PW = false>
 __global__ __launch_bounds__(TPB) void snake_conv_group_kernel(AmpGroupArgs g) {
     using TL = AmpTile<CP, G, TT, 11>;
     __shared__ __attribute__((aligned(16))) float S[TL::ROWS * TL::LS];
-    snake_conv_body<CP, CR, 0, G, TT>(g.p[blockIdx.z], S);
-}
-
-template <int CP, int CR, int G, int TT>
+    snake_conv_body<CP, CR, 0, G, TT, false, PW>(g.p[blockIdx.z], S);
+}
+
+template <int CP, int CR, int G, int TT, bool PW = false>
 __global__ __launch_bounds__(TPB) void snake_conv_group_u_kernel(AmpGroupArgs g) {
     using TL = AmpTile<CP, G, TT, 11>;
     constexpr int NU = UTile<CP>::floats(TL::ROWS + 5), NS = TL::ROWS * TL::LS;
     static_assert(((TL::ROWS + RT - 1) / RT) * CP <= 4 * TPB, "snake_tile_u keeps at most 4 work items per thread in registers");
     __shared__ __attribute__((aligned(16))) float S[NU > NS ? NU : NS];
-    snake_conv_body<CP, CR, 0, G, TT, true>(g.p[blockIdx.z], S);
+    snake_conv_body<CP, CR, 0, G, TT, true, PW>(g.p[blockIdx.z], S);
 }
 
 template <int CP, int CR, int TERMS>
@@ -703,7 +773,7 @@
     if (batch > 65535 || !tile_len_ok(len, ld)) return SVCMI_EUNSUPPORTED;
     AmpArgs a;
     a.x = x; a.w = w; a.bias = bias; a.res = res; a.y = y; a.alpha_log = alpha_log; a.beta_log = beta_log; a.filt = filt;
-    a.n = len; a.ld = ld; a.ldw = ldw; a.dil = dilation; a.accumulate = accumulate; a.alpha = alpha; a.ks = ksize;
+    a.n = len; a.ld = ld; a.ldw = ldw; a.dil = dilation; a.accumulate = accumulate; a.alpha = alpha; a.ks = ksize; a.wp = nullptr;
     const int tt = g_amp_tt ? g_amp_tt : 2;
     if (c == 10) return tt == 1 ? launch_amp<12, 10, 1, 1>(a, batch, ksize, stream) : tt == 2 ? launch_amp<12, 10, 1, 2>(a, batch, ksize, stream) : launch_amp<12, 10, 1, 4>(a, batch, ksize, stream);
     if (c == 20) return tt == 1 ? launch_amp<20, 20, 2, 1>(a, batch, ksize, stream) : tt == 2 ? launch_amp<20, 20, 2, 2>(a, batch, ksize, stream) : launch_amp<20, 20, 2, 4>(a, batch, ksize, stream);
@@ -713,22 +783,32 @@
 int g_amp_u = 0;
 int g_amp_mfma = 1;
 
+int g_amp_pairs = 1;
+
 template <int TT>
-static void launch_amp_group(const AmpGroupArgs& g, int count, int batch, int len, int c, void* stream) {
+static void launch_amp_group(const AmpGroupArgs& g, int count, int batch, int len, int c, bool pw, void* stream) {
     if constexpr (TT == 1) {
-        if (g_amp_u >= 0 && c == 10) {
+        if (c == 10) {
             constexpr int TB = AmpTile<12, 1, 1, 3>::TB;
-            SVCMI_LAUNCH((snake_conv_group_u_kernel<12, 10, 1, 1>), dim3((unsigned)((len + TB - 1) / TB), (unsigned)batch, (unsigned)count),
-                         dim3(TPB), 0, stream, g);
-            return;
+            const dim3 grid((unsigned)((len + TB - 1) / TB), (unsigned)batch, (unsigned)count);
+            if (g_amp_u >= 0) {
+                if (pw) SVCMI_LAUNCH((snake_conv_group_u_kernel<12, 10, 1, 1, true>), grid, dim3(TPB), 0, stream, g);
+                else SVCMI_LAUNCH((snake_conv_group_u_kernel<12, 10, 1, 1>), grid, dim3(TPB), 0, stream, g);
+                return;
+            }
+            if (pw) { SVCMI_LAUNCH((snake_conv_group_kernel<12, 10, 1, 1, true>), grid, dim3(TPB), 0, stream, g); return; }
         }
     }
     if constexpr (TT == 2) {
-        if ((g_amp_u > 0 || (g_amp_u == 0 && (long long)batch * len >= 500000)) && c == 20) {
+        if (c == 20) {
             constexpr int TB = AmpTile<20, 2, 2, 3>::TB;
-            SVCMI_LAUNCH((snake_conv_group_u_kernel<20, 20, 2, 2>), dim3((unsigned)((len + TB - 1) / TB), (unsigned)batch, (unsigned)count),
-                         dim3(TPB), 0, stream, g);
-            return;
+            const dim3 grid((unsigned)((len + TB - 1) / TB), (unsigned)batch, (unsigned)count);
+            if (g_amp_u > 0 || (g_amp_u == 0 && (long long)batch * len >= 500000)) {
+                if (pw) SVCMI_LAUNCH((snake_conv_group_u_kernel<20, 20, 2, 2, true>), grid, dim3(TPB), 0, stream, g);
+                else SVCMI_LAUNCH((snake_conv_group_u_kernel<20, 20, 2, 2>), grid, dim3(TPB), 0, stream, g);
+                return;
+            }
+            if (pw) { SVCMI_LAUNCH((snake_conv_group_kernel<20, 20, 2, 2, true>), grid, dim3(TPB), 0, stream, g); return; }
         }
     }
     if (c == 10) {
@@ -746,8 +826,8 @@
     }
 }
 
-extern "C" int svcmi_snake_conv_group_f32(const svcmi_snake_conv_desc* descs, int32_t count, const float* filt, int32_t batch,
-                                          int32_t len, int32_t c, int32_t ld, void* stream) {
+static int amp_group_f32(const svcmi_snake_conv_desc* descs, const float* const* wpairs, int32_t count, const float* filt, int32_t batch,
+                         int32_t len, int32_t c, int32_t ld, void* stream) {
     if (!descs || !filt || count < 1 || count > AMP_GROUP || batch <= 0 || len <= 0) return SVCMI_EINVAL;
     if (batch > 65535 || !tile_len_ok(len, ld)) return SVCMI_EUNSUPPORTED;
     int order[AMP_GROUP] = {0, 1, 2};
@@ -755,6 +835,7 @@
         for (int j = i + 1; j < count; ++j)
             if (descs[order[j]].ksize > descs[order[i]].ksize) { const int t = order[i]; order[i] = order[j]; order[j] = t; }
     AmpGroupArgs g;
+    bool pw = wpairs && g_amp_pairs && c <= 20 && !g_amp_tt;
     for (int i = 0; i < count; ++i) {
         const svcmi_snake_conv_desc& d = descs[order[i]];
         if (!d.x || !d.w || !d.y || !d.alpha_log || !d.beta_log || d.x == d.y) return SVCMI_EINVAL;
@@ -765,6 +846,9 @@
         a.x = d.x; a.w = d.w; a.bias = d.bias; a.res = d.res; a.y = d.y; a.alpha_log = d.alpha_log; a.beta_log = d.beta_log;
         a.filt = filt; a.n = len; a.ld = ld; a.ldw = d.ldw; a.dil = d.dilation; a.accumulate = d.accumulate; a.alpha = d.alpha;
         a.ks = d.ksize;
+        a.wp = wpairs ? wpairs[order[i]] : nullptr;
+        if ((uintptr_t)a.wp & 63) return SVCMI_EALIGN;
+        pw = pw && a.wp;
     }
     for (int i = count; i < AMP_GROUP; ++i) g.p[i] = g.p[0];
     const bool mfma_auto = g_amp_mfma == 1 && c == 20 && batch <= 2;
@@ -780,11 +864,22 @@
         }
     }
     const int tt = g_amp_tt ? g_amp_tt : (c == 10 ? 1 : 2);
-    if (tt == 4) launch_amp_group<4>(g, count, batch, len, c, stream);
-    else if (tt == 1) launch_amp_group<1>(g, count, batch, len, c, stream);
-    else launch_amp_group<2>(g, count, batch, len, c, stream);
+    if (tt == 4) launch_amp_group<4>(g, count, batch, len, c, pw, stream);
+    else if (tt == 1) launch_amp_group<1>(g, count, batch, len, c, pw, stream);
+    else launch_amp_group<2>(g, count, batch, len, c, pw, stream);
     return SVCMI_LAST_ERROR();
 }
+
+extern "C" int svcmi_snake_conv_group_f32(const svcmi_snake_conv_desc* descs, int32_t count, const float* filt, int32_t batch,
+                                          int32_t len, int32_t c, int32_t ld, void* stream) {
+    return amp_group_f32(descs, nullptr, count, filt, batch, len, c, ld, stream);
+}
+
+extern "C" int svcmi_snake_conv_group_pairs_f32(const svcmi_snake_conv_desc* descs, const float* const* wpairs, int32_t count,
+                                                const float* filt, int32_t batch, int32_t len, int32_t c, int32_t ld, void* stream) {
+    return amp_group_f32(descs, wpairs, count, filt, batch, len, c, ld, stream);
+}
+
 
 extern "C" int svcmi_snake_conv_lp_supported(int32_t c, int32_t ld, int32_t ksize, int32_t dilation, int32_t precision) {
     return svcmi_snake_conv_supported(c, ld, ksize, dilation) && c <= 20 && (precision == SVCMI_PREC_F16 || precision == SVCMI_PREC_F16W2);
@@ -816,7 +911,7 @@
         AmpArgs& a = g.p[i];
         a.x = d.x; a.w = d.w; a.bias = d.bias; a.res = d.res; a.y = d.y; a.alpha_log = d.alpha_log; a.beta_log = d.beta_log;
         a.filt = filt; a.n = len; a.ld = ld; a.ldw = d.ldw; a.dil = d.dilation; a.accumulate = d.accumulate; a.alpha = d.alpha;
-        a.ks = d.ksize;
+        a.ks = d.ksize; a.wp = nullptr;
     }
     for (int i = count; i < AMP_GROUP; ++i) g.p[i] = g.p[0];
     const bool ut = g_amp_u >= 0;
@@ -883,6 +978,10 @@
     i = 0;
     while (km[i] && name[i] == km[i]) ++i;
     if (km[i] == 0 && name[i] == 0 && value >= 0 && value <= 3) { g_amp_mfma = value; return 0; }
+    const char* kp = "amp_pairs";
+    i = 0;
+    while (kp[i] && name[i] == kp[i]) ++i;
+    if (kp[i] == 0 && name[i] == 0 && (value == 0 || value == 1)) { g_amp_pairs = value; return 0; }
     const char* ku = "amp_u";
     i = 0;
     while (ku[i] && name[i] == ku[i]) ++i;
diff --git a/whisper-vits-svc_amd/csrc/host_stages.hip b/whisper-vits-svc_amd/csrc/host_stages.hip
--- a/whisper-vits-svc_amd/csrc/host_stages.hip
+++ b/whisper-vits-svc_amd/csrc/host_stages.hip
@@ -597,24 +597,28 @@
         float** outs = q == nd - 1 ? t2 : xj;
         if (fused) {
             svcmi_snake_conv_desc d[3];
+            const float* wp[3];
+            auto pairs_of = [](const svcmi_weight& w) { return w.prec16 == SVCMI_PREC_F32_PAIRS ? static_cast<const float*>(w.w16a) : nullptr; };
             double fl = 0.0;
             for (int j = 0; j < nb; ++j) {
                 const svcmi_amp_block& b = st.blocks[j];
                 d[j] = svcmi_snake_conv_desc{xc[j], b.c1[q].w, b.c1[q].bias, nullptr, t1[j], b.a1_alpha[q], b.a1_beta[q], b.c1[q].ldw, b.k,
                                              b.dil[q], 0, 1.0f};
+                wp[j] = pairs_of(b.c1[q]);
                 fl += 2.0 * B * L * st.c * st.c * b.k;
             }
             auto half_step = [&] {
                 if (lp) run(c, OP_SNAKE_CONV_GROUP_LP, fl, 8.0 * nb * B * L * st.c,
                             [&] { return svcmi_snake_conv_group_lp(d, nb, m.filt, B, (int32_t)L, st.c, cp, SVCMI_PREC_F16W2, c.stream); });
                 else run(c, OP_SNAKE_CONV_GROUP, fl, 8.0 * nb * B * L * st.c,
-                         [&] { return svcmi_snake_conv_group_f32(d, nb, m.filt, B, (int32_t)L, st.c, cp, c.stream); });
+                         [&] { return svcmi_snake_conv_group_pairs_f32(d, wp, nb, m.filt, B, (int32_t)L, st.c, cp, c.stream); });
             };
             half_step();
             for (int j = 0; j < nb; ++j) {
                 const svcmi_amp_block& b = st.blocks[j];
                 d[j] = svcmi_snake_conv_desc{t1[j], b.c2[q].w, b.c2[q].bias, xc[j], outs[j], b.a2_alpha[q], b.a2_beta[q], b.c2[q].ldw, b.k,
                                              1, 0, 1.0f};
+                wp[j] = pairs_of(b.c2[q]);
             }
             half_step();
         } else {
diff --git a/whisper-vits-svc_amd/svcmi/_lib.py b/whisper-vits-svc_amd/svcmi/_lib.py
--- a/whisper-vits-svc_amd/svcmi/_lib.py
+++ b/whisper-vits-svc_amd/svcmi/_lib.py
@@ -11,6 +11,7 @@
 PREC_F32, PREC_BF16X3, PREC_BF16, PREC_F16, PREC_BF16_A16, PREC_F16_A16, PREC_BF16X3_A16 = 0, 1, 2, 3, 4, 5, 6
 PRECISIONS = {None: 0, "f32": 0, "fp32": 0, "bf16x3": 1, "bf16": 2, "f16": 3, "fp16": 3, "f16w2": 8}
 PREC_F16W2, PREC_F16W2_A16 = 8, 9
+PREC_F32_PAIRS = 10
 PREC_MIXED = 7
 PREC_CLASSES = 12
 CLASS_ENC, CLASS_FLOW, CLASS_UPS, CLASS_AMP0 = 0, 1, 2, 3
@@ -317,6 +318,7 @@
     "svcmi_snake_post_f32": (c_int, [_P, _P, _P, _P, _P, _P, _I, _I, _I, _I, _I, _P]),
     "svcmi_conv_gemm_group_f32": (c_int, [_P, _I, _P]),
     "svcmi_snake_conv_group_f32": (c_int, [_P, _I, _P, _I, _I, _I, _I, _P]),
+    "svcmi_snake_conv_group_pairs_f32": (c_int, [_P, _P, _I, _P, _I, _I, _I, _I, _P]),
     "svcmi_snake_conv_lp_supported": (c_int, [_I, _I, _I, _I, _I]),
     "svcmi_snake_conv_group_lp": (c_int, [_P, _I, _P, _I, _I, _I, _I, _I, _P]),
     "svcmi_snake_alias_group_f32": (c_int, [_P, _P, _P, _P, _P, _I, _I, _I, _I, _I, _P, _I, _P]),
diff --git a/whisper-vits-svc_amd/svcmi/cmodel.py b/whisper-vits-svc_amd/svcmi/cmodel.py
--- a/whisper-vits-svc_amd/svcmi/cmodel.py
+++ b/whisper-vits-svc_amd/svcmi/cmodel.py
@@ -9,7 +9,7 @@
         self.struct, self.keep = struct, keep
 
 
-def _weight(cw, ops, w, bias, prec, keep, a16=False):
+def _weight(cw, ops, w, bias, prec, keep, a16=False, pairs=None):
     cw.w, cw.bias = w.data_ptr(), (0 if bias is None else bias.data_ptr())
     cw.n, cw.ldw = int(w.shape[0]), int(w.shape[1])
     cw.w16, cw.w16a, cw.ldw16, cw.prec16 = 0, 0, 0, 0
@@ -23,6 +23,9 @@
             img_a = ops.lp_weight(w, a16_code)
             cw.w16a = img_a.data_ptr()
             keep.append(img_a)
+    elif pairs is not None:
+        cw.w16a, cw.prec16 = pairs.data_ptr(), _lib.PREC_F32_PAIRS
+        keep.append(pairs)
     keep.append(w)
     keep.append(bias)
 
@@ -77,9 +80,9 @@
     m.sampling_rate, m.merge_b = float(hp.data.sampling_rate), float(w.merge_b)
     state = {"cls": _lib.CLASS_ENC}
 
-    def W(cw, wt, b=None, a16=False):
+    def W(cw, wt, b=None, a16=False, pairs=None):
         p = classes[state["cls"]] if classes else code
-        _weight(cw, ops, wt, b, p, keep, a16=a16 and p != PREC_BF16X3)
+        _weight(cw, ops, wt, b, p, keep, a16=a16 and p != PREC_BF16X3, pairs=pairs)
     W(m.pre, w.pre_w, w.pre_b)
     W(m.hub, w.hub_w, w.hub_b)
     W(m.proj, w.proj_w, w.proj_b)
@@ -127,8 +130,9 @@
             b.k, b.n_dil = blk["k"], len(blk["d"])
             for q, d in enumerate(blk["d"]):
                 b.dil[q] = d
-                W(b.c1[q], blk["c1"][q][0], blk["c1"][q][1], a16=st["cp"] % 8 == 0)
-                W(b.c2[q], blk["c2"][q][0], blk["c2"][q][1], a16=st["cp"] % 8 == 0)
+                W(b.c1[q], blk["c1"][q][0], blk["c1"][q][1], a16=st["cp"] % 8 == 0,
+                  pairs=blk["c1p"][q] if "c1p" in blk else None)
+                W(b.c2[q], blk["c2"][q][0], blk["c2"][q][1], a16=st["cp"] % 8 == 0, pairs=blk["c2p"][q] if "c2p" in blk else None)
                 b.a1_alpha[q], b.a1_beta[q] = blk["a1"][q][0].data_ptr(), blk["a1"][q][1].data_ptr()
                 b.a2_alpha[q], b.a2_beta[q] = blk["a2"][q][0].data_ptr(), blk["a2"][q][1].data_ptr()
     return CModel(m, keep)
diff --git a/whisper-vits-svc_amd/svcmi/ops.py b/whisper-vits-svc_amd/svcmi/ops.py
--- a/whisper-vits-svc_amd/svcmi/ops.py
+++ b/whisper-vits-svc_amd/svcmi/ops.py
@@ -575,6 +575,11 @@
         if precision is not None:
             self._call("svcmi_snake_conv_group_lp", descs, len(problems), _ptr(filt), B, L, c, ld, PRECISIONS[precision], self._stream(),
                        work={"flops": flops, "bytes": 8.0 * len(problems) * B * L * c})
+        elif any(pr.get("wp") is not None for pr in problems):
+            self._chk(*[pr.get("wp") for pr in problems])
+            wps = (ctypes.c_void_p * len(problems))(*[_ptr(pr.get("wp")) for pr in problems])
+            self._call("svcmi_snake_conv_group_pairs_f32", descs, wps, len(problems), _ptr(filt), B, L, c, ld, self._stream(),
+                       work={"flops": flops, "bytes": 8.0 * len(problems) * B * L * c})
         else:
             self._call("svcmi_snake_conv_group_f32", descs, len(problems), _ptr(filt), B, L, c, ld, self._stream(),
                        work={"flops": flops, "bytes": 8.0 * len(problems) * B * L * c})
diff --git a/whisper-vits-svc_amd/svcmi/weights.py b/whisper-vits-svc_amd/svcmi/weights.py
--- a/whisper-vits-svc_amd/svcmi/weights.py
+++ b/whisper-vits-svc_amd/svcmi/weights.py
@@ -24,6 +24,24 @@
     if ldw != p.shape[1]:
         p = torch.cat([p, torch.zeros(n_pad, ldw - p.shape[1], dtype=torch.float32, device=w.device)], dim=1)
     return p.contiguous()
+
+
+PAIR_GROUP = 10
+
+
+def conv_pairs_supported(c, ld, ksize):
+    return (c, ld) in ((10, 12), (20, 20)) and ksize in (3, 7, 11)
+
+
+def pack_conv_pairs(rows, c, ld, ksize):
+    if not conv_pairs_supported(c, ld, ksize):
+        raise ValueError(f"no pair-ordered image for c={c} ld={ld} ksize={ksize}")
+    nc4, ng = (c + 3) // 4, c // PAIR_GROUP
+    w = rows[:c, :ksize * ld].reshape(c, ksize, ld)[:, :, :c]
+    p = torch.zeros(ksize, nc4 * 4, c, dtype=torch.float32, device=rows.device)
+    p[:, :c, :] = w.permute(1, 2, 0)
+    p = p.reshape(ksize, nc4, 4, ng, PAIR_GROUP).permute(0, 1, 3, 2, 4)
+    return p.contiguous().reshape(-1)
 
 
 def pad_vec(v, n_pad):
@@ -132,6 +150,9 @@
                     blk["c2"].append((f(pack_conv(fold_weight_norm(sd, f"{b}.convs2.{q}"), cout_p, cout_p)), f(pad_vec(sd[f"{b}.convs2.{q}.bias"], cout_p))))
                     blk["a1"].append((f(pad_vec(sd[f"{b}.activations.{2 * q}.act.alpha"], cout_p)), f(pad_vec(sd[f"{b}.activations.{2 * q}.act.beta"], cout_p))))
                     blk["a2"].append((f(pad_vec(sd[f"{b}.activations.{2 * q + 1}.act.alpha"], cout_p)), f(pad_vec(sd[f"{b}.activations.{2 * q + 1}.act.beta"], cout_p))))
+                if conv_pairs_supported(cout, cout_p, kk):
+                    blk["c1p"] = [f(pack_conv_pairs(w, cout, cout_p, kk)) for w, _ in blk["c1"]]
+                    blk["c2p"] = [f(pack_conv_pairs(w, cout, cout_p, kk)) for w, _ in blk["c2"]]
                 st["blocks"].append(blk)
             self.stages.append(st)
         cl = self.stages[-1]["cp"]
```

Result: no change. 1508 audio-seconds/sec, median of 6 (+0.6%).
